# lucas-t-t/FACT-CLIP

Measured on AMD Instinct MI355X. Metric: frames/sec FACT_CLIP fwd+bwd, T=4096 D=2048 Nact=32, at 1/2/4/8 GPUs, higher is better.
Workload: dtype fp32; 1 GPU; FACT_CLIP HAViD-holdout dims, seg10 synthetic, T=4096; model=FACT_CLIP, T=4096, D=2048, Nact=32, C=75, videos_per_rank=2, global_batch=2, seq_len=4096, parallelism=dp1, weights=fixed (no optimizer update in the timed steps)

## Files before the change

### fact-clip_amd/csrc/decoder.cpp

```cpp
#include <algorithm>
#include <cmath>
#include <vector>

#include "fx_common.h"
#include "ops.h"
#include "tokdec.h"

namespace fx {
namespace {

constexpr int MAXL = 16;
constexpr int kSmallTok = 64;

struct PackKV {
  const float* src[2 * MAXL];
  const float* bsrc[2 * MAXL];
  float* dst;
  float* bdst;
  int A, Hm, L;
};

__global__ void pack_kv_kernel(PackKV p) {
  const int blk = blockIdx.y;
  const long long n = (long long)p.A * p.Hm;
// ... 6 lines not shown
}

struct UnpackKV {
  float* dst[2 * MAXL];
  float* bdst[2 * MAXL];
  const float* src;
  const float* bsrc;
  int A, Hm, L;
};

__global__ void unpack_kv_acc_kernel(UnpackKV p) {
  const int blk = blockIdx.y;
  const long long n = (long long)p.A * p.Hm;
  const float* src = p.src + (long long)blk * n;
  float* dst = p.dst[blk];
  for (long long i = (long long)blockIdx.x * blockDim.x + threadIdx.x; i < n; i += (long long)gridDim.x * blockDim.x)
    dst[i] += src[i];
  if (blockIdx.x == 0 && p.bdst[blk])
    for (int i = threadIdx.x; i < p.A; i += blockDim.x) p.bdst[blk][i] += p.bsrc[blk * p.A + i];
}

int linear_fwd_res(const float* x, long long ldx, int M, int K, const float* w, long long ldw, const float* b,
                   const float* resid, long long ldr, float* y, long long ldy, int N, hipStream_t s) {
  fx_gemm_desc d = gemm_desc(M, N, K, op_rows(x, ldx), op_rows(w, ldw), y, ldy);
  d.bias = b;
  d.resid = resid;
  d.ld_resid = ldr;
  return launch_gemm(d, s);
}

fx_gemm_desc dx_res_desc(const float* dy, long long lddy, const float* w, long long ldw, int M, int K, int N,
                         const float* resid, long long ldr, float* dx, long long lddx, float* ws) {
  fx_gemm_desc d = gemm_desc(M, K, N, op_rows(dy, lddy), op_cols(w, ldw), dx, lddx);
  d.resid = resid;
  d.ld_resid = ldr;
  d.split_k = pick_split(M, K, N);
  d.workspace = ws;
  return d;
}

int linear_dx_res(const float* dy, long long lddy, const float* w, long long ldw, int M, int K, int N,
                  const float* resid, long long ldr, float* dx, long long lddx, float* ws, hipStream_t s) {
  fx_gemm_desc d = gemm_desc(M, K, N, op_rows(dy, lddy), op_cols(w, ldw), dx, lddx);
  d.resid = resid;
  d.ld_resid = ldr;
  d.split_k = pick_split(M, K, N);
  d.workspace = ws;
  return launch_gemm(d, s);
}

struct DecLayout {
  long long xq, qkv, psa, osa, xh1, rs1, t1, t1q, qc, pca, oca, xh2, rs2, t2, f1, xh3, rs3, t3, per_layer;
  long long layers, fxh, frs, fo, kv, mpos, total_saved;
  long long wkv, bkv, wsp, total_ws_fwd;
  long long dkv, dwkv, dbkv, dT, dS, dU, dF, dQKV, dO, dq, lnws, core, dmask, split, gdu, gdf, gdq, gdqkv,
      gdy, total_ws_bwd;
};

long long dec_split_ws(const fx_decoder_params* p, int R, int T) {
  const int A = p->A, FF = p->FF;
  long long sp = 0;
  sp = std::max(sp, dwdb_ws(R, A, 3 * A));
  sp = std::max(sp, dwdb_ws(R, A, 2 * A));
  sp = std::max(sp, dwdb_ws(R, A, A));
  sp = std::max(sp, dwdb_ws(R, A, FF));
  sp = std::max(sp, dwdb_ws(R, FF, A));
  sp = std::max(sp, split_ws(R, A, 3 * A));
  sp = std::max(sp, split_ws(R, A, FF));
  sp = std::max(sp, split_ws(R, FF, A));
  sp = std::max(sp, dwdb_ws(R, A, p->out_dim));
  sp = std::max(sp, split_ws(R, A, p->out_dim));
  if (p->cross) {
    const long long AL2 = 2LL * A * p->num_layers;
    sp = std::max(sp, split_ws(T, (int)AL2, p->Hm));
    sp = std::max(sp, dwdb_ws(T, p->Hm, (int)AL2));
    sp = std::max(sp, split_ws(T, p->Hm, (int)AL2));
    sp = std::max(sp, dwdb_ws(T, p->Hm, (int)(AL2 / 2)));
    sp = std::max(sp, (long long)defer_split(T) * AL2 * (p->Hm + 1));
    sp = std::max(sp, split_ws(T, p->Hm, (int)(AL2 / 2)));
  }
  return sp;
}

int dec_tmax(const fx_decoder_params* p, int T, int nvid) {
  if (!p->cross) return 0;
  if (!p->mem_off) return T / nvid;
  int m = 0;
  for (int v = 0; v < nvid; ++v) m = std::max(m, p->mem_off[v + 1] - p->mem_off[v]);
  return m;
}

int dec_qmax(const fx_decoder_params* p, int R, int nvid) {
  if (!p->tok_off) return R / nvid;
  int m = 0;
  for (int v = 0; v < nvid; ++v) m = std::max(m, p->tok_off[v + 1] - p->tok_off[v]);
  return m;
}

long long dec_attn_ws(const fx_decoder_params* p, int nvid, int Qv, int Tv) {
  const int hd = p->A / p->nhead;
  long long w = p->cross ? tattn_ws_floats(nvid, Qv, Tv, hd, p->nhead) : 0;
  if (Qv > kSmallTok) w = std::max(w, tattn_ws_floats(nvid, Qv, Qv, hd, p->nhead));
  return w;
}

DecLayout dec_layout(const fx_decoder_params* p, int R, int T, int has_qpos, int has_mpos, int nvid) {
  DecLayout L{};
  const long long A = p->A, FF = p->FF, h = p->nhead, RA = (long long)R * A;
  const long long Qv = dec_qmax(p, R, nvid), Tv = dec_tmax(p, T, nvid);
  long long o = 0;
  L.xq = o; o += al64(has_qpos ? RA : 0);
  L.qkv = o; o += al64(3 * RA);
  L.psa = o; o += al64(nvid * h * Qv * Qv);
  L.osa = o; o += al64(RA);
  L.xh1 = o; o += al64(RA);
  L.rs1 = o; o += al64(R);
  L.t1 = o; o += al64(RA);
  if (p->cross) {
    L.t1q = o; o += al64(has_qpos ? RA : 0);
    L.qc = o; o += al64(RA);
    L.pca = o; o += al64(nvid * h * Qv);
    L.oca = o; o += al64(RA);
    L.xh2 = o; o += al64(RA);
    L.rs2 = o; o += al64(R);
    L.t2 = o; o += al64(RA);
  }
  L.f1 = o; o += al64((long long)R * FF);
  L.xh3 = o; o += al64(RA);
  L.rs3 = o; o += al64(R);
  L.t3 = o; o += al64(RA);
  L.per_layer = o;
  L.layers = 0;
  o = L.layers + L.per_layer * p->num_layers;
  L.fxh = o; o += al64(p->final_norm ? RA : 0);
  L.frs = o; o += al64(p->final_norm ? R : 0);
  L.fo = o; o += al64(p->final_norm ? RA : 0);
  const long long AL2 = 2 * A * p->num_layers;
  L.kv = o; o += al64(p->cross ? (long long)T * AL2 : 0);
  L.mpos = o; o += al64((p->cross && has_mpos) ? (long long)T * p->Hm : 0);
  L.total_saved = o;
  const long long sp = dec_split_ws(p, R, T);
  o = 0;
  L.wkv = o; o += al64(p->cross ? AL2 * p->Hm : 0);
  L.bkv = o; o += al64(p->cross ? AL2 : 0);
  const long long att = dec_attn_ws(p, nvid, (int)Qv, (int)Tv);
  L.wsp = o; o += al64(std::max(sp, att) + RA);
  L.total_ws_fwd = o;
  o = 0;
  L.dkv = o; o += al64(p->cross ? (long long)T * AL2 : 0);
  L.dwkv = o; o += al64(p->cross ? AL2 * p->Hm : 0);
  L.dbkv = o; o += al64(p->cross ? AL2 : 0);
  L.dT = o; o += al64(RA);
  L.dS = o; o += al64(RA);
  L.dU = o; o += al64(RA);
  L.dF = o; o += al64((long long)R * FF);
  L.dQKV = o; o += al64(3 * RA);
  L.dO = o; o += al64(RA);
  L.dq = o; o += al64(RA);
  L.lnws = o; o += al64(layernorm_bwd_ws_floats(R, (int)A));
  L.core = o; o += al64(att);
  L.dmask = o; o += al64((p->dropout > 0.f) ? RA : 0);
  L.split = o; o += al64(sp);
  L.gdu = o; o += al64(3LL * p->num_layers * RA);
  L.gdf = o; o += al64((long long)p->num_layers * R * FF);
  L.gdq = o; o += al64((long long)p->num_layers * RA);
  L.gdqkv = o; o += al64(3LL * p->num_layers * RA);
  L.gdy = o; o += al64(3LL * p->num_layers * RA);
  L.total_ws_bwd = o;
  (void)FF;
  return L;
}

int dec_check(const fx_decoder_params* p, int R, int T, int nvid) {
  FX_REQUIRE(p && p->num_layers >= 1 && p->num_layers <= MAXL, "decoder: 1..16 layers");
  FX_REQUIRE(nvid >= 1 && nvid <= 32, "decoder: 1..32 videos");
  if (p->tok_off) {
    FX_REQUIRE(p->tok_off[0] == 0 && p->tok_off[nvid] == R, "decoder: token offsets must span [0, R]");
    for (int v = 0; v < nvid; ++v) FX_REQUIRE(p->tok_off[v + 1] > p->tok_off[v], "decoder: >= 1 token per video, offsets increasing");
  } else {
    FX_REQUIRE(R % nvid == 0, "decoder: token rows split evenly (or tok_off)");
  }
  if (p->cross) {
    if (p->mem_off) {
      FX_REQUIRE(p->mem_off[0] == 0 && p->mem_off[nvid] == T, "decoder: memory offsets must span [0, T]");
      for (int v = 0; v < nvid; ++v) FX_REQUIRE(p->mem_off[v + 1] > p->mem_off[v], "decoder: empty video memory");
    } else {
      FX_REQUIRE(T % nvid == 0 && T >= nvid, "decoder: memory rows must split evenly over the videos");
    }
    FX_REQUIRE(p->Hm > 0, "decoder: cross attention needs memory rows");
  }
  R /= nvid;
  FX_REQUIRE(p->nhead > 0 && p->A % p->nhead == 0, "decoder: A must be divisible by nhead");
  FX_REQUIRE(R >= 1, "decoder: >= 1 token per video");
  FX_REQUIRE(p->A / p->nhead <= 64, "decoder: head dim must be <= 64");
  FX_REQUIRE(p->A <= 1024, "decoder: A <= 1024 (LayerNorm row kernel)");
  FX_REQUIRE(p->dropout >= 0.f && p->dropout < 1.f && p->attn_dropout >= 0.f && p->attn_dropout < 1.f,
             "decoder: dropout p in [0, 1)");
// ... 385 lines not shown
  if (amode == TOK_A_LN) {
    P->ln.w = ln_w;
    P->ln.b = ln_b;
    P->ln.eps = 1e-5f;
  }
  return tb.flush();
}

long long fx_decoder_saved_floats(const fx_decoder_params* p, int R, int T, int nvid, int has_qpos, int has_mpos) {
  return dec_layout(p, R, T, has_qpos, has_mpos, std::max(nvid, 1)).total_saved;
}

long long fx_decoder_workspace_floats(const fx_decoder_params* p, int R, int T, int nvid, int has_qpos,
                                      int has_mpos) {
  const DecLayout L = dec_layout(p, R, T, has_qpos, has_mpos, std::max(nvid, 1));
  return std::max(L.total_ws_fwd, L.total_ws_bwd);
}

int fx_decoder_fwd(const fx_decoder_params* p, const float* tgt, long long ldt, int R, const float* qpos,
                   long long ldqp, const float* mem, long long ldm, int T, int nvid, const float* mpos, long long ldmp,
                   float* out, long long ldo, float* saved, float* workspace, void* stream) {
  FX_TRY(dec_check(p, R, T, nvid));
  const int Qv = dec_qmax(p, R, nvid), Tv = dec_tmax(p, T, nvid);
  hipStream_t s = (hipStream_t)stream;
  const int A = p->A, FF = p->FF, h = p->nhead, hd = A / h, NL = p->num_layers;
  const long long RA = (long long)R * A;
  const float eps = p->eps > 0.f ? p->eps : 1e-5f;
  const float pd = p->dropout, pa = p->attn_dropout;
  const float scale = 1.0f / std::sqrt((float)hd);
  const DecLayout L = dec_layout(p, R, T, qpos != nullptr, mpos != nullptr, nvid);
  FX_REQUIRE(!qpos || ldqp == A, "decoder: query_pos must be dense (R, A)");
  float* spl = workspace + L.wsp;
  WsBound wb(spl, L.total_ws_fwd - L.wsp);
  const int AL2 = 2 * A * NL;
  float* kv = saved + L.kv;
  if (p->cross) {
    PackKV pk{};
    for (int l = 0; l < NL; ++l) {
      pk.src[l] = p->ca_k_w[l];
      pk.src[NL + l] = p->ca_v_w[l];
      pk.bsrc[l] = p->ca_in_b[l] + A;
      pk.bsrc[NL + l] = p->ca_in_b[l] + 2 * A;
    }
    pk.dst = workspace + L.wkv;
    pk.bdst = workspace + L.bkv;
    pk.A = A;
    pk.Hm = p->Hm;
    pk.L = NL;
    fx_launch(pack_kv_kernel, dim3(std::min(cdiv((long long)A * p->Hm, 256), 256), 2 * NL), dim3(256), 0, s,
                       pk);
    FX_CHECK_HIP(hipGetLastError());
    prof_begin(9, s);
    if (!mpos) {
      FX_TRY(linear_fwd(mem, ldm, T, p->Hm, workspace + L.wkv, workspace + L.bkv, kv, AL2, AL2, 0, s));
      prof_end(9, s, 2.0 * T * AL2 * p->Hm, 4.0 * ((double)T * p->Hm + (double)AL2 * p->Hm + (double)T * AL2));
    } else {
      const int AL = A * NL;
      FX_TRY(linear_fwd(mem, ldm, T, p->Hm, workspace + L.wkv, workspace + L.bkv, kv, AL2, AL, 0, s, -1, mpos, ldmp,
                        p->Hm));
      FX_TRY(linear_fwd(mem, ldm, T, p->Hm, workspace + L.wkv + (long long)AL * p->Hm, workspace + L.bkv + AL,
                        kv + AL, AL2, AL, 0, s));
      prof_end(9, s, 2.0 * T * AL2 * p->Hm, 4.0 * (2.0 * T * p->Hm + (double)AL2 * p->Hm + (double)T * AL2), 2);
      FX_TRY(add2(mem, ldm, mpos, ldmp, T, p->Hm, saved + L.mpos, p->Hm, 0, s));
    }
  }
  {
    const void* ptrs[3] = {tgt, qpos, out};
    const long long lds_[2] = {ldt, ldo};
    if (dec_tok_ok(p, R, nvid, ptrs, 3, lds_, 2)) {
      float* u = spl + (std::max(L.total_ws_fwd - L.wsp, RA) - RA);
      return dec_fwd_tok(p, tgt, ldt, R, qpos, nvid, Qv, Tv, kv, out, ldo, saved, L, u, spl, s);
    }
  }
  const float* x = tgt;
  long long ldx = ldt;
  for (int l = 0; l < NL; ++l) {
    float* b = saved + L.layers + l * L.per_layer;
    const float* xq = x;
    long long ldxq = ldx;
    if (qpos) {
      if (l == 0) FX_TRY(add2(x, ldx, qpos, A, R, A, b + L.xq, A, 0, s));
      xq = b + L.xq;
      ldxq = A;
    }
    float* qkv = b + L.qkv;
    if (!qpos) {
      FX_TRY(linear_fwd(x, ldx, R, A, p->sa_in_w[l], p->sa_in_b[l], qkv, 3 * A, 3 * A, 0, s));
    } else {
      fx_gemm_desc d2[2];
      d2[0] = gemm_desc(R, 2 * A, A, op_rows(xq, ldxq), op_rows(p->sa_in_w[l], A), qkv, 3 * A);
      d2[0].bias = p->sa_in_b[l];
      d2[1] = gemm_desc(R, A, A, op_rows(x, ldx), op_rows(p->sa_in_w[l] + 2LL * A * A, A), qkv + 2 * A, 3 * A);
      d2[1].bias = p->sa_in_b[l] + 2 * A;
      FX_TRY(launch_gemm_group(d2, 2, s));
    }
    if (Qv <= kSmallTok) {
      FX_TRY(launch_mha_small_fwd(qkv, 3 * A, qkv + A, 3 * A, qkv + 2 * A, 3 * A, Qv, Qv, hd, h, scale, b + L.psa,
                                  b + L.osa, A, s, nvid, pa, dec_seed(p, l, 0), p->tok_off));
    } else {
      TAttnOpts o;
      o.koff = o.qoff = p->tok_off;
      o.drop_p = pa;
      o.drop_seed = dec_seed(p, l, 0);
      FX_TRY(launch_tattn_fwd(qkv, 3 * A, qkv + A, 3 * A, qkv + 2 * A, 3 * A, nvid, Qv, Qv, hd, h, scale, b + L.osa, A,
                              b + L.psa, spl, s, &o));
    }
    float* u = spl + (std::max(L.total_ws_fwd - L.wsp, RA) - RA);
// ... 302 lines not shown
```

### fact-clip_amd/csrc/fx_common.h

```cpp
#pragma once
#include <hip/hip_runtime.h>
#include <hip/hip_ext.h>
#include <cstdint>
#include <cstdio>
#include <string>

#include "../../include/factmx.h"

namespace fx {

void set_error(const std::string& msg);

#define FX_CHECK_HIP(expr)                                                        \
  do {                                                                            \
    hipError_t _e = (expr);                                                       \
    if (_e != hipSuccess) {                                                       \
      ::fx::set_error(std::string("HIP error ") + hipGetErrorString(_e) + " at " + \
                      __FILE__ + ":" + std::to_string(__LINE__));                 \
      return FX_ERR_HIP;                                                          \
    }                                                                             \
  } while (0)

#define FX_REQUIRE(cond, msg)                 \
  do {                                        \
// ... 27 lines not shown
int aux_join_into(hipStream_t s, hipStream_t a);
int defer_split(int rows);
long long gemm_workspace_floats(const fx_gemm_desc& d);

fx_operand op_rows(const float* p, long long ld);
fx_operand op_cols(const float* p, long long ld);
fx_gemm_desc gemm_desc(int M, int N, int K, fx_operand a, fx_operand b, float* c, long long ldc);

int launch_colsum_batched(const float* x, long long ld, long long x_bs, int M, int N, int nb, float* out,
                          long long out_bs, int accumulate, float* ws, hipStream_t s);
int launch_colsum(const float* x, long long ld, int M, int N, float* out, int accumulate,
                  float* ws, hipStream_t s);

constexpr long long kArrivalCounters = 1 << 16;
unsigned* arrival_counters(hipStream_t s);

__host__ __device__ inline unsigned fx_drop_bits(unsigned long long seed, unsigned long long idx) {
  unsigned long long z = seed + (idx + 1ull) * 0x9E3779B97F4A7C15ull;
  z = (z ^ (z >> 30)) * 0xBF58476D1CE4E5B9ull;
  z = (z ^ (z >> 27)) * 0x94D049BB133111EBull;
  z ^= z >> 31;
  return (unsigned)(z >> 32);
}
inline unsigned fx_drop_thresh(float p) {
  const double t = (double)p * 4294967296.0;
  return t >= 4294967295.0 ? 4294967295u : (unsigned)t;
}
inline unsigned long long fx_drop_subseed(unsigned long long seed, int i) {
  return seed + 0xD1B54A32D192ED03ull * (unsigned long long)(i + 1);
}
int launch_dropout(const float* x, long long ldx, int rows, int cols, long long idx_ld, long long idx_col0, float p,
                   unsigned long long seed, float* y, long long ldy, hipStream_t s);

struct Knobs {
  int gemm_path = 0;
  int gemm_wide = -1;
  bool gemm_xcd_planes = true;
  bool gemm_persist = true;
  bool gemm_group_m = true;
  bool gemm_row_perm = true;
  bool frl_pair = true;
  int frl_min_fill = 80;
  int frl2_min_fill = 55;
  bool aux_stream = true;
  bool x2y_a2f_dw = true;
  bool tattn_fold = true;
  bool tattn_rr = true;
  bool gru_poll2 = true;
  int gru_store_wave = 2;
  int frl_xcd = 2;
  bool gemm_group = true;
  bool gemm_ktail = true;
  bool dec_tok = true;
  int tok_spin = 0;
  bool side_stream = true;
  bool mstcn_defer = true;
  bool x2y_fused = true;
  bool x2y_f2a_one = true;
  int x2y_f2a_bwd = 2;
};
const Knobs& knobs();

void prof_begin(int kind, hipStream_t s);
void prof_end(int kind, hipStream_t s, double flops, double bytes, int launches = 1);
extern thread_local int g_prof_open;
bool prof_kernel_events(hipStream_t s, hipEvent_t* e0, hipEvent_t* e1);

template <typename... Args, typename F = void (*)(Args...)>
inline void fx_launch(F kernel, const dim3& grid, const dim3& block, std::uint32_t shm, hipStream_t s, Args... args) {
  hipEvent_t e0, e1;
  if (g_prof_open >= 0 && prof_kernel_events(s, &e0, &e1))
    hipExtLaunchKernelGGL(kernel, grid, block, shm, s, e0, e1, 0u, args...);
  else
    hipLaunchKernelGGL(kernel, grid, block, shm, s, args...);
}

unsigned tok_spin_max();
unsigned x2y_spin_max();
int coresident_blocks(const void* kernel, int threads, size_t lds);

}
```

### fact-clip_amd/csrc/gemm.cpp

```cpp
#include <algorithm>
#include <atomic>
#include <cstdio>
#include <map>
#include <mutex>
#include <utility>
#include <vector>

#include "gemm_plan.h"

namespace fx {

unsigned* arrival_counters(hipStream_t s) {
  static std::mutex mu;
  static std::map<std::pair<int, hipStream_t>, unsigned*> pool;
  int dev = 0;
  if (hipGetDevice(&dev) != hipSuccess) return nullptr;
  std::lock_guard<std::mutex> lk(mu);
  const auto key = std::make_pair(dev, s);
  auto it = pool.find(key);
  if (it != pool.end()) return it->second;
  unsigned* p = nullptr;
  if (hipMalloc(&p, kArrivalCounters * sizeof(unsigned)) != hipSuccess) return nullptr;
  if (hipMemsetAsync(p, 0, kArrivalCounters * sizeof(unsigned), s) != hipSuccess) {
    (void)hipFree(p);
    return nullptr;
  }
  pool[key] = p;
  return p;
}

thread_local const float* t_ws_lo = nullptr;
thread_local const float* t_ws_hi = nullptr;

WsBound::WsBound(const float* base, long long floats) : prev_lo(t_ws_lo), prev_hi(t_ws_hi) {
  t_ws_lo = base;
  t_ws_hi = base ? base + std::max(floats, 0LL) : nullptr;
}
WsBound::~WsBound() {
  t_ws_lo = prev_lo;
  t_ws_hi = prev_hi;
}

fx_operand op_rows(const float* p, long long ld) {
  fx_operand o{};
  o.ptr = p;
  o.ld = ld;
  o.conv_dir = 1;
  return o;
}

fx_operand op_cols(const float* p, long long ld) {
  fx_operand o = op_rows(p, ld);
  o.trans = 1;
  return o;
}

fx_gemm_desc gemm_desc(int M, int N, int K, fx_operand a, fx_operand b, float* c, long long ldc) {
  fx_gemm_desc d{};
  d.M = M;
  d.N = N;
  d.K = K;
  d.batch = 1;
  d.a = a;
  d.b = b;
  d.c = c;
  d.ldc = ldc;
  d.alpha = 1.f;
  d.split_k = 1;
  return d;
}

long long gemm_workspace_floats(const fx_gemm_desc& d) {
  if (d.split_k <= 1) return 0;
  return (long long)d.batch * d.split_k * d.M * d.N;
}

std::mutex g_prec_mu;
std::vector<std::pair<hipStream_t, int>> g_prec;
std::atomic<int> g_prec_any{0};
std::atomic<int> g_prec_default{FX_PREC_F32};

int stream_precision(hipStream_t s) {
  if (!g_prec_any.load(std::memory_order_acquire)) return g_prec_default.load(std::memory_order_relaxed);
  std::lock_guard<std::mutex> lk(g_prec_mu);
  for (const auto& e : g_prec)
    if (e.first == s) return e.second;
  return g_prec_default.load(std::memory_order_relaxed);
}

bool valid_precision(int prec) {
  return prec == FX_PREC_F32 || prec == FX_PREC_BF16 || prec == FX_PREC_F32S || prec == FX_PREC_F32S2;
}

namespace {

int plan_on_stream(const fx_gemm_desc& d, hipStream_t s, long long cnt_base, GemmPlan& P) {
  FX_TRY(plan_gemm(d, stream_precision(s), knobs(), cnt_base, P));
  GemmDev& g = P.g;
  const bool direct = P.family == FAM_DIRECT;
  const int cap = d.split_k > 1 ? d.split_k : 1;
  if (g.split > 1 && t_ws_hi && !(g.ws >= t_ws_lo && g.ws + (long long)g.split * d.M * d.N * d.batch <= t_ws_hi))
    std::fprintf(stderr, "factmx: gemm M %d N %d K %d batch %d split %d (cap %d, %s) needs %lld floats at +%lld of a %lld-float reservation\n",
                 d.M, d.N, d.K, d.batch, g.split, cap, direct ? "direct" : "tiled",
                 (long long)g.split * d.M * d.N * d.batch, (long long)(g.ws - t_ws_lo), (long long)(t_ws_hi - t_ws_lo));
  FX_REQUIRE(g.split <= 1 || !t_ws_hi ||
                 (g.ws >= t_ws_lo && g.ws + (long long)g.split * d.M * d.N * d.batch <= t_ws_hi),
             "gemm: split-K slabs would overrun the entry point's workspace reservation");
  if (P.counters) {
    unsigned* pool = arrival_counters(s);
    g.tile_cnt = pool ? pool + P.cnt_base : nullptr;
  }
  return FX_OK;
}

void census(const fx_gemm_desc& d, const GemmPlan& P, hipStream_t s) {
#ifdef FX_GEMM_CENSUS
  std::fprintf(stderr, "GEMM %p %d %d %d %d %d %d %d %d %d %d %d\n", (void*)s, d.M, d.N, d.K, d.batch, P.ak, P.bk,
               P.g.split, P.family == FAM_DIRECT ? 1 : P.family == FAM_TILED ? 0 : 2, P.g.persist, d.a.conv_taps,
               (int)(P.g.split > 1 && !P.g.tile_cnt));
#endif
}

int launch_family(const GemmPlan& P, hipStream_t s) {
  switch (P.family) {
    case FAM_TILED: return launch_tiled(P, s);
    case FAM_WIDE8: return launch_wide8(P, s);
    case FAM_BF16: return launch_bf16(P, s);
    case FAM_SPLIT: return launch_split(P, s);
    case FAM_DIRECT: return launch_direct(P, s);
    default: break;
  }
  set_error("gemm: unknown kernel family");
  return FX_ERR_UNSUPPORTED;
}

}

int launch_gemm(const fx_gemm_desc& d, hipStream_t s) {
  FX_REQUIRE(d.M >= 0 && d.N >= 0 && d.K >= 0 && d.batch >= 1, "gemm: bad sizes");
  if (d.M == 0 || d.N == 0) return FX_OK;
  GemmPlan P;
  FX_TRY(plan_on_stream(d, s, 0, P));
  census(d, P, s);
  FX_TRY(launch_family(P, s));
  FX_CHECK_HIP(hipGetLastError());
  return launch_reduce(P, s);
}

int launch_gemm_group(const fx_gemm_desc* d, int n, hipStream_t s) {
  const bool on = knobs().gemm_group;
  FX_REQUIRE(n >= 0 && n <= GMAX, "gemm group: 0..4 members");
  int live = 0, nsplit = 0;
  bool all_direct = on;
  GemmPlan P[GMAX];
  long long cnt_base = 0;
  for (int i = 0; i < n && all_direct; ++i) {
    FX_REQUIRE(d[i].M >= 0 && d[i].N >= 0 && d[i].K >= 0 && d[i].batch >= 1, "gemm: bad sizes");
    if (d[i].M == 0 || d[i].N == 0) continue;
    FX_TRY(plan_on_stream(d[i], s, cnt_base, P[i]));
    if (P[i].g.tile_cnt) cnt_base += P[i].counters;
    all_direct = all_direct && P[i].family == FAM_DIRECT;
    nsplit += P[i].g.split > 1 ? 1 : 0;
    ++live;
  }
  bool ws_ok = true;
  if (all_direct && nsplit > 1) {
    const float* base = nullptr;
    long long off = 0;
    for (int i = 0; i < n && ws_ok; ++i) {
      if (d[i].M == 0 || d[i].N == 0 || P[i].g.split <= 1) continue;
      if (!base) base = d[i].workspace;
      ws_ok = d[i].workspace == base && t_ws_hi != nullptr;
      P[i].g.ws = d[i].workspace + off;
      off += (long long)P[i].g.split * d[i].M * d[i].N * d[i].batch;
      ws_ok = ws_ok && P[i].g.ws >= t_ws_lo && P[i].g.ws + (long long)P[i].g.split * d[i].M * d[i].N * d[i].batch <= t_ws_hi;
    }
  }
  if (!all_direct || live < 2 || !ws_ok) {
    for (int i = 0; i < n; ++i) FX_TRY(launch_gemm(d[i], s));
    return FX_OK;
  }
  bool done[GMAX] = {};
  for (int i0 = 0; i0 < n; ++i0) {
    if (done[i0] || d[i0].M == 0 || d[i0].N == 0) continue;
    const unsigned nw = P[i0].block.x;
    GemmGroup G{};
    int m = 0;
    G.start[0] = 0;
    for (int i = i0; i < n; ++i) {
      if (done[i] || d[i].M == 0 || d[i].N == 0 || P[i].block.x != nw) continue;
      done[i] = true;
      G.g[m] = P[i].g;
      G.kinds[m] = gen_kind(P[i].ak) * 8 + P[i].bk;
      G.start[m + 1] = G.start[m] + (int)(P[i].grid.x * P[i].grid.y * P[i].grid.z);
      ++m;
    }
    for (int i = m + 1; i <= GMAX; ++i) G.start[i] = G.start[m];
    G.n = m;
    if (m == 1) {
      census(d[i0], P[i0], s);
      FX_TRY(launch_direct(P[i0], s));
    } else {
      launch_direct_group(G, G.start[m], nw, s);
    }
    FX_CHECK_HIP(hipGetLastError());
  }
  for (int i = 0; i < n; ++i)
    if (d[i].M != 0 && d[i].N != 0) FX_TRY(launch_reduce(P[i], s));
  return FX_OK;
}

}

extern "C" {

int fx_set_stream_precision(void* stream, int prec) {
  FX_REQUIRE(prec == FX_PREC_DEFAULT || fx::valid_precision(prec),
             "gemm precision: FX_PREC_DEFAULT, FX_PREC_F32, FX_PREC_BF16, FX_PREC_F32S or FX_PREC_F32S2");
  std::lock_guard<std::mutex> lk(fx::g_prec_mu);
  const hipStream_t s = (hipStream_t)stream;
  auto& v = fx::g_prec;
  for (auto it = v.begin(); it != v.end(); ++it)
    if (it->first == s) {
      v.erase(it);
      break;
    }
  if (prec != FX_PREC_DEFAULT) v.emplace_back(s, prec);
  fx::g_prec_any.store(v.empty() ? 0 : 1, std::memory_order_release);
  return FX_OK;
}

int fx_get_stream_precision(void* stream) { return fx::stream_precision((hipStream_t)stream); }

int fx_stream_precision_explicit(void* stream) {
  std::lock_guard<std::mutex> lk(fx::g_prec_mu);
  for (const auto& e : fx::g_prec)
    if (e.first == (hipStream_t)stream) return e.second;
  return FX_PREC_DEFAULT;
}

int fx_set_default_precision(int prec) {
  FX_REQUIRE(fx::valid_precision(prec), "default gemm precision: FX_PREC_F32, FX_PREC_BF16, FX_PREC_F32S or FX_PREC_F32S2");
  fx::g_prec_default.store(prec, std::memory_order_relaxed);
  return FX_OK;
}

int fx_get_default_precision(void) { return fx::g_prec_default.load(std::memory_order_relaxed); }

}
```

### fact-clip_amd/csrc/gemm_dev.h

```cpp
#pragma once
#include "fx_common.h"

namespace fx {

constexpr int BM = 64, BN = 64, BK = 64, NTHREADS = 256;
constexpr int RS = 68;
constexpr int CS = 65;
constexpr int IMG = BM * RS;
constexpr int NSLOT = 3;
typedef float f32x16 __attribute__((ext_vector_type(16)));
constexpr int WBM = 128;
constexpr int W8T = 512;
constexpr int DCH = 32, DMAXW = 8;
#define FX_INLINE __attribute__((always_inline))

constexpr int kMaxSeq = 16;

enum Kind { ROWS = 0, ROWS_CONV = 1, ROWS_GEN = 2, COLS = 3, COLS_CONV = 4, ROWS_CAT = 5, COLS_CONVR = 6, COLS_KT = 7 };

struct GemmDev {
  int M, N, K;
  fx_operand a, b;
  float* c;
  long long ldc, c_bs;
  float alpha, beta;
  const float* bias;
  const float* resid;
  long long ld_resid, resid_bs;
  const float* gate;
  long long ld_gate;
  int relu, split, kt_per_split, a_vec, b_vec, c_tap_cin;
  float* ws;
  float* c_last;
  int tiles_x, tiles_y;
  long long* stamps;
  unsigned* tile_cnt;
  unsigned drop_thr;
  float drop_scale;
  unsigned long long drop_seed;
  long long c_last_bs;
  int b_dil_growth;
  int xcd_planes;
  int row_perm;
  int group_m;
  int persist;
  int a_dil_b1;
  long long bias_bs;
  int nsoff;
  int soff[kMaxSeq + 1];
};

namespace {

typedef int SeqOff[kMaxSeq + 1];

__device__ __forceinline__ void seq_pos(int seq_len, const SeqOff& soff, int nsoff, int r, int& pos, int& len) {
  if (nsoff > 0) {
    int start = 0, end = 0x7fffffff;
#pragma unroll
    for (int i = 1; i <= kMaxSeq; ++i) {
      if (i <= nsoff) {
        const int o = soff[i];
        if (o <= r) start = o;
        else end = min(end, o);
      }
    }
    pos = r - start;
    len = end - start;
  } else {
    pos = r % seq_len;
    len = seq_len;
  }
}

#ifdef FX_STAMPS
#define FX_STAMP(g, slot)                                                                          \
  do {                                                                                            \
    if ((g).stamps && threadIdx.x == 0) {                                                         \
      const long long _b = (long long)blockIdx.z * gridDim.x * gridDim.y + blockIdx.y * gridDim.x + \
                           blockIdx.x;                                                            \
      (g).stamps[(_b * 2) * 10 + 2 * (slot)] = __builtin_amdgcn_s_memtime();                       \
      (g).stamps[(_b * 2) * 10 + 2 * (slot) + 1] = __builtin_amdgcn_s_memrealtime();               \
    }                                                                                             \
  } while (0)
#else
#define FX_STAMP(g, slot) \
  do {                    \
  } while (0)
#endif

__device__ __forceinline__ int conv_shift(const fx_operand& o, int tap) {
  return (tap - (o.conv_taps - 1) / 2) * o.conv_dil * o.conv_dir;
}

__device__ __forceinline__ fx_operand batch_op_a(const fx_operand& a, int dil_b1, int bidx) {
  fx_operand o = a;
  if (dil_b1 > 0 && bidx == 1) o.conv_dil = dil_b1;
  return o;
}

__device__ __forceinline__ fx_operand batch_op_b(const fx_operand& b, int growth, int bidx) {
  fx_operand o = b;
// ... 385 lines not shown
```

### fact-clip_amd/csrc/gemm_plan.cpp

```cpp
#include <algorithm>

#include "gemm_plan.h"

namespace fx {
namespace {

bool aligned16(const void* p) { return (reinterpret_cast<uintptr_t>(p) & 15) == 0; }

bool use_direct(const fx_gemm_desc& d, int ak, int bk, const Knobs& kn) {
  const int force = kn.gemm_path;
  auto fits = [&](const fx_operand& o, int kind, int R) {
    const double k = (double)d.K + 2 * DMAXW * DCH + 64, ld = (double)o.ld;
    const double bytes = kind == ROWS ? ((double)R * ld + k) * 4 : kind == COLS ? (k * ld + R) * 4 : 0;
    return bytes < 4294967296.0;
  };
  const bool ok = d.K > 0 && direct_pair(gen_kind(ak), bk) && fits(d.a, ak, d.M) && fits(d.b, bk, d.N);
  if (!ok || force == 1) return false;
  if (force == 2) return true;
  const int lim = (ak == ROWS_GEN || ak == ROWS_CAT) ? 32 : 64;
  if (d.M <= lim || d.N <= lim || d.K <= 64 || (d.K <= 512 && d.K % 64 != 0)) return true;
  const long long t32 = (long long)cdiv(d.M, 32) * cdiv(d.N, 32) * d.batch;
  return (ak == ROWS || ak == COLS) && t32 <= 512 && d.K <= 2048;
}

bool use_wide(const GemmDev& g, int ak, int bk, int batch, const Knobs& kn) {
  const int force = kn.gemm_wide;
  const bool fast = g.a_vec && g.b_vec && ((g.K % BK) == 0 || ak == COLS_KT);
  const bool ok = fast && wide8_pair(ak, bk);
  if (!ok || force == 0) return false;
  if (force == 1) return true;
  return (long long)cdiv(g.M, WBM) * g.tiles_x * batch * g.split >= 192;
}

}

bool operand_vec_ok(const fx_operand& o) {
  if (!aligned16(o.ptr) || (o.ld & 3)) return false;
  if (o.batch_stride & 3) return false;
  if (o.conv_taps && (o.conv_cin & 7)) return false;
  if (!o.trans && o.ptr1 && (!aligned16(o.ptr1) || (o.ld1 & 3) || (o.k_split & 7))) return false;
  return true;
}

int kind_of(const fx_operand& o, bool vec) {
  if (o.trans) return o.conv_taps ? (o.nseq > 0 ? COLS_CONVR : COLS_CONV) : COLS;
  if (o.conv_taps) return (vec && o.conv_cin % BK == 0) ? ROWS_CONV : ROWS_GEN;
  if (o.pos) return ROWS_GEN;
  if (o.ptr1 || o.rows0 || o.rows1) return (vec && (!o.ptr1 || o.k_split % BK == 0)) ? ROWS_CAT : ROWS_GEN;
  return ROWS;
}

int plan_gemm(const fx_gemm_desc& d, int prec, const Knobs& kn, long long tile_cnt_base, GemmPlan& P) {
  FX_REQUIRE(d.M >= 0 && d.N >= 0 && d.K >= 0 && d.batch >= 1, "gemm: bad sizes");
  FX_REQUIRE(d.a.ptr && d.b.ptr && d.c, "gemm: null operand");
  FX_REQUIRE(!(d.a.conv_taps && d.a.seq_len <= 0 && d.a.nseq <= 0) &&
                 !(d.b.conv_taps && d.b.seq_len <= 0 && d.b.nseq <= 0),
             "gemm: conv operand needs seq_len or seq_off");
  FX_REQUIRE(d.a.nseq <= 0 || !d.a.trans, "gemm: ragged conv offsets on a row-major A or a column-major B operand");
  FX_REQUIRE(d.b.nseq <= 0 || (d.b.trans && d.b.conv_taps && d.a.nseq <= 0),
             "gemm: ragged column-major conv B needs a plain A operand");
  FX_REQUIRE(!(d.a.conv_taps && d.K != d.a.conv_taps * d.a.conv_cin), "gemm: conv A needs K == taps*cin");
  FX_REQUIRE(!(d.b.conv_taps && d.b.trans && d.N != d.b.conv_taps * d.b.conv_cin + (d.b.ones_col ? 1 : 0)),
             "gemm: conv B needs N == taps*cin (+1 with a ones column)");
  FX_REQUIRE(!(d.a.ones_col && !d.a.trans) && !(d.b.ones_col && !d.b.trans), "gemm: ones_col needs trans==1");
  FX_REQUIRE(!(d.b.conv_taps && !d.b.trans), "gemm: row-major conv B operand is not supported");
  P = GemmPlan{};
  GemmDev& g = P.g;
  g.M = d.M;
  g.N = d.N;
  g.K = d.K;
  g.a = d.a;
  g.b = d.b;
  {
    const fx_operand& o = d.a;
    if (o.nseq > 0) {
      FX_REQUIRE(o.conv_taps && o.seq_off && o.nseq <= kMaxSeq, "gemm: seq_off needs a conv operand, <= 16 videos");
      const int rows = d.M;
      FX_REQUIRE(o.seq_off[0] == 0 && o.seq_off[o.nseq] == rows, "gemm: seq_off must span the operand's rows");
      for (int v = 0; v <= o.nseq; ++v) {
        FX_REQUIRE(v == 0 || o.seq_off[v] > o.seq_off[v - 1], "gemm: seq_off must increase");
        g.soff[v] = o.seq_off[v];
      }
      g.nsoff = o.nseq;
    }
  }
  {
    const fx_operand& o = d.b;
    if (o.nseq > 0) {
      FX_REQUIRE(o.seq_off && o.nseq <= kMaxSeq && o.seq_off[0] == 0 && o.seq_off[o.nseq] <= d.K,
                 "gemm: ragged B offsets must start at 0 and end within K, <= 16 videos");
      FX_REQUIRE(operand_vec_ok(d.a) && operand_vec_ok(d.b) && d.K % BK == 0,
                 "gemm: ragged B needs 16-B operands and K a multiple of 64 (pad the frames)");
      for (int v = 0; v <= kMaxSeq; ++v) {
        FX_REQUIRE(v == 0 || v > o.nseq || o.seq_off[v] > o.seq_off[v - 1], "gemm: seq_off must increase");
        g.soff[v] = v <= o.nseq ? o.seq_off[v] : 0x7fffffff;
      }
      g.nsoff = o.nseq;
    }
  }
  g.c = d.c;
  g.ldc = d.ldc;
  g.c_bs = d.c_batch_stride;
  g.alpha = d.alpha;
  g.beta = d.beta;
  g.bias = d.bias;
  g.resid = d.resid;
  g.ld_resid = d.ld_resid;
  g.resid_bs = d.resid_batch_stride;
  g.gate = d.gate;
  g.ld_gate = d.ld_gate;
  g.relu = d.relu;
  g.c_tap_cin = d.c_tap_cin;
  g.c_last = d.c_last_col;
  g.c_last_bs = d.c_last_batch_stride ? d.c_last_batch_stride : d.M;
  g.b_dil_growth = d.b_dil_growth;
  g.a_dil_b1 = d.a_dil_b1;
  g.bias_bs = d.bias_batch_stride;
  FX_REQUIRE(d.a_dil_b1 <= 0 || (d.a.conv_taps && !d.a.trans), "gemm: a_dil_b1 needs a row-major conv A");
  FX_REQUIRE(d.b_dil_growth <= 1 || (d.b.conv_taps && d.b.trans), "gemm: b_dil_growth needs a column-major conv B");
  g.stamps = d.dbg_stamps;
  FX_REQUIRE(d.drop_p >= 0.f && d.drop_p < 1.f, "gemm: dropout p must be in [0, 1)");
  FX_REQUIRE(d.drop_p == 0.f || (!d.c_last_col && !d.c_tap_cin && !d.gate && d.beta == 0.f &&
                                 !(d.relu == 1 && d.resid)),
             "gemm: dropout only on plain outputs (before the residual add)");
  g.drop_thr = d.drop_p > 0.f ? std::max(fx_drop_thresh(d.drop_p), 1u) : 0u;
  g.drop_scale = 1.f / (1.f - d.drop_p);
  g.drop_seed = d.drop_seed;
  g.a_vec = operand_vec_ok(d.a);
  g.b_vec = operand_vec_ok(d.b);
  g.ws = d.workspace;
  int ak = kind_of(d.a, g.a_vec), bk = kind_of(d.b, g.b_vec);
  const bool direct = d.b_dil_growth <= 1 && d.a_dil_b1 <= 0 && use_direct(d, ak, bk, kn);
  if (!direct && ak == COLS && bk == COLS && g.a_vec && g.b_vec && d.K % BK != 0 && kn.gemm_ktail) ak = bk = COLS_KT;
  P.ak = ak;
  P.bk = bk;
  P.batch = d.batch;
  bool wide = false;
  const int cap = (d.split_k > 1 && d.workspace) ? d.split_k : 1;
  FX_REQUIRE(!(d.split_k > 1 && !d.workspace), "gemm: split-K needs a workspace");
  if (direct) {
    const int nch = cdiv(d.K, DCH);
    const long long t32 = (long long)cdiv(d.M, 32) * cdiv(d.N, 32) * d.batch;
    const int cpw = 1;
    const int nw = std::min(DMAXW, std::max(1, nch / cpw));
    int split = 1;
    if (cap > 1 && t32 < 64) {
      const long long want = std::min<long long>(nch / (cpw * nw), cdiv(2048, t32 * nw));
      split = (int)std::max<long long>(1, std::min<long long>(cap, want));
    }
    g.kt_per_split = nch > 0 ? cdiv(nch, split) : 0;
    g.split = g.kt_per_split > 0 ? cdiv(nch, g.kt_per_split) : 1;
    g.tiles_x = cdiv(d.N, 32);
    g.tiles_y = cdiv(d.M, 32);
    P.block = dim3(nw * 64);
  } else {
    const int nkt = cdiv(d.K, BK);
    int split = std::min(cap, std::max(nkt, 1));
    g.kt_per_split = nkt > 0 ? cdiv(nkt, split) : 0;
    g.split = g.kt_per_split > 0 ? cdiv(nkt, g.kt_per_split) : 1;
    g.tiles_x = cdiv(d.N, BN);
    wide = use_wide(g, ak, bk, d.batch, kn);
    g.tiles_y = cdiv(d.M, wide ? WBM : BM);
    P.block = dim3(wide ? W8T : NTHREADS);
  }
  P.grid = dim3(g.tiles_x, g.tiles_y, d.batch * g.split);
  const bool lowp = wide && bf16_pair(ak, bk);
  P.np = !lowp ? 0 : prec == FX_PREC_F32S ? 3 : prec == FX_PREC_F32S2 ? 2 : 0;
  P.family = direct ? FAM_DIRECT
           : !wide ? FAM_TILED
           : P.np ? (split_pair(ak, bk) ? FAM_SPLIT : FAM_WIDE8)
           : (lowp && prec == FX_PREC_BF16) ? FAM_BF16
                                            : FAM_WIDE8;
  P.fast = P.family == FAM_TILED && g.a_vec && g.b_vec && ((g.K % BK) == 0 || ak == COLS_KT) && ak != ROWS_GEN &&
           gen_kind(bk) != ROWS_GEN;
  const bool runs = P.family == FAM_DIRECT  ? direct_pair(gen_kind(ak), bk)
                    : P.family == FAM_TILED ? tiled_pair(ak, gen_kind(bk), P.fast)
                    : P.family == FAM_BF16  ? bf16_pair(ak, bk)
                    : P.family == FAM_SPLIT ? split_pair(ak, bk)
                    : P.np                  ? wide8_split_pair(ak, bk)
                                            : wide8_pair(ak, bk);
  if (!runs) {
    set_error("gemm: unsupported operand kinds");
    return FX_ERR_UNSUPPORTED;
  }
// ... 29 lines not shown
```

### fact-clip_amd/csrc/gemm_plan.h

```cpp
#pragma once
#include <type_traits>
#include <utility>

#include "gemm_dev.h"

namespace fx {

enum Family { FAM_TILED = 0, FAM_WIDE8, FAM_BF16, FAM_SPLIT, FAM_DIRECT };

constexpr int gen_kind(int k) { return k == ROWS_CAT ? ROWS_GEN : k; }

constexpr bool rowmajor_a(int ak) { return ak == ROWS || ak == ROWS_CONV || ak == ROWS_CAT; }

constexpr bool tiled_pair(int ak, int bk, bool fast) {
  const bool a = rowmajor_a(ak) || ak == COLS || ak == COLS_KT || (ak == ROWS_GEN && !fast);
  const bool b = bk == ROWS || bk == COLS || bk == COLS_CONV || (bk == ROWS_GEN && !fast) ||
                 (fast && ((bk == COLS_CONVR && ak == COLS) || (bk == COLS_KT && ak == COLS_KT)));
  return a && b;
}
constexpr bool tiled_fast_pair(int ak, int bk) { return tiled_pair(ak, bk, true); }
constexpr bool tiled_generic_pair(int ak, int bk) { return tiled_pair(ak, bk, false); }

constexpr bool wide8_pair(int ak, int bk) { return tiled_pair(ak, bk, true); }

constexpr bool bf16_pair(int ak, int bk) { return rowmajor_a(ak) && (bk == ROWS || bk == COLS); }
constexpr bool wide8_split_pair(int ak, int bk) { return rowmajor_a(ak) && bk == ROWS; }
constexpr bool split_pair(int ak, int bk) { return rowmajor_a(ak) && bk == COLS; }

constexpr bool direct_pair(int ak, int bk) {
  return (ak == ROWS || ak == ROWS_GEN || ak == COLS) && (bk == ROWS || bk == COLS);
}

struct GemmPlan {
  GemmDev g;
  dim3 grid, block;
  int ak, bk;
  int family;
  bool fast;
  int np;
  int batch;
  long long cnt_base, counters;
};

bool operand_vec_ok(const fx_operand& o);
int kind_of(const fx_operand& o, bool vec);

int plan_gemm(const fx_gemm_desc& d, int prec, const Knobs& k, long long tile_cnt_base, GemmPlan& P);

int launch_tiled(const GemmPlan& P, hipStream_t s);
int launch_wide8(const GemmPlan& P, hipStream_t s);
int launch_bf16(const GemmPlan& P, hipStream_t s);
int launch_split(const GemmPlan& P, hipStream_t s);
int launch_direct(const GemmPlan& P, hipStream_t s);
void launch_direct_group(const GemmGroup& G, int blocks, unsigned threads, hipStream_t s);
int launch_reduce(const GemmPlan& P, hipStream_t s);

template <class F, int... Ks>
void with_kind(int k, F&& f, std::integer_sequence<int, Ks...>) {
  ((k == Ks ? f(std::integral_constant<int, Ks>{}) : void()), ...);
}
using AllKinds = std::integer_sequence<int, ROWS, ROWS_CONV, ROWS_GEN, COLS, COLS_CONV, ROWS_CAT, COLS_CONVR, COLS_KT>;

template <bool (*Pair)(int, int), class F>
int dispatch_pair(int ak, int bk, const char* family, F&& launch) {
  bool done = false;
  with_kind(ak, [&](auto A) {
    with_kind(bk, [&](auto B) {
      if constexpr (Pair(decltype(A)::value, decltype(B)::value)) {
        launch(A, B);
        done = true;
      }
    }, AllKinds{});
  }, AllKinds{});
  if (done) return FX_OK;
  set_error(std::string("gemm(") + family + "): unsupported operand kinds");
  return FX_ERR_UNSUPPORTED;
}

}
```

### fact-clip_amd/csrc/linear.cpp

```cpp
#include <algorithm>
#include <vector>

#include "fx_common.h"
#include "ops.h"

namespace fx {
namespace {

__global__ void relu_bwd_kernel(const float* dy, long long lddy, const float* y, long long ldy, int rows, int cols,
                                float* dz, long long lddz) {
  const long long total = (long long)rows * cols;
  for (long long i = (long long)blockIdx.x * blockDim.x + threadIdx.x; i < total; i += (long long)gridDim.x * blockDim.x) {
    const long long r = i / cols, c = i % cols;
    dz[r * lddz + c] = y[r * ldy + c] > 0.f ? dy[r * lddy + c] : 0.f;
  }
}

__global__ void add2_kernel(const float* a, long long lda, const float* b, long long ldb, int rows, int cols,
                            float* o, long long ldo, int accumulate, int bcols) {
  const long long total = (long long)rows * cols;
  for (long long i = (long long)blockIdx.x * blockDim.x + threadIdx.x; i < total; i += (long long)gridDim.x * blockDim.x) {
    const long long r = i / cols, c = i % cols;
    const float v = a[r * lda + c] + (b && c < bcols ? b[r * ldb + c] : 0.f);
    o[r * ldo + c] = accumulate ? o[r * ldo + c] + v : v;
  }
}

}

int ew_grid(long long total) { return (int)std::min<long long>(std::max<long long>(cdiv(total, 256), 1), 4096); }

int relu_bwd(const float* dy, long long lddy, const float* y, long long ldy, int rows, int cols, float* dz,
             long long lddz, hipStream_t s) {
  if ((long long)rows * cols == 0) return FX_OK;
  fx_launch(relu_bwd_kernel, dim3(ew_grid((long long)rows * cols)), dim3(256), 0, s, dy, lddy, y, ldy, rows,
                     cols, dz, lddz);
  FX_CHECK_HIP(hipGetLastError());
  return FX_OK;
}

int add2(const float* a, long long lda, const float* b, long long ldb, int rows, int cols, float* o, long long ldo,
         int accumulate, hipStream_t s, int bcols) {
  if ((long long)rows * cols == 0) return FX_OK;
  fx_launch(add2_kernel, dim3(ew_grid((long long)rows * cols)), dim3(256), 0, s, a, lda, b, ldb, rows, cols,
                     o, ldo, accumulate, bcols < 0 ? cols : bcols);
  FX_CHECK_HIP(hipGetLastError());
  return FX_OK;
}

int pick_split(int M, int N, int K, int batch) {
  const int nkt = cdiv(K, 64);
  if (nkt < 4) return 1;
  const bool wide = M >= 128 && K % 64 == 0;
  const long long tiles = (long long)cdiv(M, wide ? 128 : 64) * cdiv(N, 64) * batch;
  if (tiles >= 160) return 1;
  int sp = (int)std::min<long long>(nkt / 2, 256 / tiles);
  return std::max(sp, 1);
}

long long split_ws(int M, int N, int K, int batch) {
  const int sp = pick_split(M, N, K, batch);
  return sp > 1 ? (long long)sp * M * N * batch : 0;
}

int linear_fwd(const float* x, long long ldx, int M, int K, const float* w, const float* b, float* y, long long ldy,
               int N, int relu, hipStream_t s, long long ldw, const float* pos, long long ldpos, int pos_cols) {
  fx_gemm_desc d = gemm_desc(M, N, K, op_rows(x, ldx), op_rows(w, ldw < 0 ? K : ldw), y, ldy);
  d.a.pos = pos;
  d.a.ld_pos = ldpos;
  d.a.pos_cols = pos ? pos_cols : 0;
  d.bias = b;
  d.relu = relu;
  return launch_gemm(d, s);
}

fx_gemm_desc desc_linear_dx(const float* dy, long long lddy, const float* w, int M, int K, int N, float* dx,
                            long long lddx, int accumulate, const float* gate, long long ld_gate, float* ws,
                            long long ldw) {
  fx_gemm_desc d = gemm_desc(M, K, N, op_rows(dy, lddy), op_cols(w, ldw < 0 ? K : ldw), dx, lddx);
  d.beta = accumulate ? 1.f : 0.f;
  d.gate = gate;
  d.ld_gate = ld_gate;
  d.split_k = pick_split(M, K, N);
  d.workspace = ws;
  return d;
}

int linear_dx(const float* dy, long long lddy, const float* w, int M, int K, int N, float* dx, long long lddx,
              int accumulate, const float* gate, long long ld_gate, float* ws, hipStream_t s, long long ldw) {
  return launch_gemm(desc_linear_dx(dy, lddy, w, M, K, N, dx, lddx, accumulate, gate, ld_gate, ws, ldw), s);
}

fx_gemm_desc desc_linear_dwdb(const float* dy, long long lddy, const float* x, long long ldx, int M, int K, int N,
                              float* dw, float* db, int accumulate, float* ws, long long lddw) {
  if (!dw) {
    fx_gemm_desc e{};
    e.batch = 1;
    e.c_last_col = db;
    return e;
  }
  fx_operand b = op_cols(x, ldx);
  const int Kc = K + (db ? 1 : 0);
  if (db) b.ones_col = K + 1;
  fx_gemm_desc d = gemm_desc(N, Kc, M, op_cols(dy, lddy), b, dw, lddw < 0 ? K : lddw);
  d.c_last_col = db;
  d.beta = accumulate ? 1.f : 0.f;
  d.split_k = pick_split(N, K + 1, M);
  d.workspace = ws;
  return d;
}

int linear_dwdb(const float* dy, long long lddy, const float* x, long long ldx, int M, int K, int N, float* dw,
                float* db, int accumulate, float* ws, hipStream_t s, long long lddw) {
  if (!dw && !db) return FX_OK;
  FX_REQUIRE(dw, "linear_dwdb: bias-only gradient needs dw");
  return launch_gemm(desc_linear_dwdb(dy, lddy, x, ldx, M, K, N, dw, db, accumulate, ws, lddw), s);
}

int linear_bwd_pair(const fx_gemm_desc& dwdb, const fx_gemm_desc& dx, hipStream_t s) {
  FX_REQUIRE(!(dwdb.c_last_col && !dwdb.c), "linear_dwdb: bias-only gradient needs dw");
  const fx_gemm_desc pr[2] = {dwdb, dx};
  return launch_gemm_group(pr, 2, s);
}

int linear_dw(const float* dy, long long lddy, const float* x, long long ldx, int M, int K, int N, float* dw,
              int accumulate, float* ws, hipStream_t s, long long lddw) {
  return linear_dwdb(dy, lddy, x, ldx, M, K, N, dw, nullptr, accumulate, ws, s, lddw);
}

long long dwdb_ws(int M, int K, int N) { return split_ws(N, K + 1, M); }

#ifndef FX_DEFER_SPLIT_BUILD
#define FX_DEFER_SPLIT_BUILD 16
#endif
int defer_split(int rows) { return std::max(1, std::min(FX_DEFER_SPLIT_BUILD, rows / 512)); }

}

using namespace fx;

extern "C" {

int fx_dropout(const float* x, long long ldx, int rows, int cols, long long idx_ld, long long idx_col0, float p,
// ... 258 lines not shown
```

### fact-clip_amd/csrc/mstcn.cpp

```cpp
#include <algorithm>
#include <vector>

#include "fx_common.h"
#include "ops.h"
#include "frames.h"

namespace fx {
namespace {

struct PackArgs {
  const float* w[32];
  float* wf[32];
  float* wb[32];
  const float* wpw[32];
  float* wpt[32];
  int F;
};

__global__ __launch_bounds__(256) void pack_conv_kernel(PackArgs p) {
  const int l = blockIdx.z, F = p.F;
  const int c0 = blockIdx.x * 32, n0 = blockIdx.y * 32;
  const int tx = threadIdx.x & 31, ty = threadIdx.x >> 5;
  __shared__ float t[3][32][33];
  const float* w = p.w[l];
  for (int r = ty; r < 32; r += 8) {
    const int n = n0 + r;
    for (int e = tx; e < 96; e += 32) {
      const int cl = e / 3, j = e - cl * 3;
      t[j][r][cl] = (n < F && c0 + cl < F) ? w[(long long)n * 3 * F + (long long)(c0 + cl) * 3 + j] : 0.f;
    }
  }
  __syncthreads();
  for (int r = ty; r < 32; r += 8) {
    const int n = n0 + r, c = c0 + r;
    if (n < F && c0 + tx < F)
#pragma unroll
      for (int j = 0; j < 3; ++j) p.wf[l][(long long)n * 3 * F + j * F + c0 + tx] = t[j][r][tx];
    if (c < F && n0 + tx < F)
#pragma unroll
      for (int j = 0; j < 3; ++j) p.wb[l][(long long)c * 3 * F + j * F + n0 + tx] = t[j][tx][r];
  }
  if (p.wpt[l]) {
    __syncthreads();
    for (int r = ty; r < 32; r += 8) {
      const int o = n0 + r;
      t[0][r][tx] = (o < F && c0 + tx < F) ? p.wpw[l][(long long)o * F + c0 + tx] : 0.f;
    }
    __syncthreads();
    for (int r = ty; r < 32; r += 8) {
      const int c = c0 + r;
      if (c < F && n0 + tx < F) p.wpt[l][(long long)c * F + n0 + tx] = t[0][tx][r];
    }
  }
}

struct MstcnLayout {
  long long rows_pad;
  long long rowsF;
  long long h, z, xh, rs, wbs, wpts, wk1b, wk2b, total_saved;
  long long wf, wk1, wk2, buf0, buf1, buf2, buf3, buf4, buf5, split, split2, colsum, dzall, dhall, dball, csb, bsl,
      total_ws;
};

MstcnLayout mstcn_layout(const fx_mstcn_params* p, int rows) {
  MstcnLayout L{};
  const long long F = p->F;
  const int NL = p->num_layers;
  L.rows_pad = (long long)cdiv(rows, 64) * 64;
  L.rowsF = L.rows_pad * F;
  L.h = 0;
  L.z = L.h + (NL + 1) * L.rowsF;
  L.xh = L.z + NL * L.rowsF;
  L.rs = L.xh + (p->layernorm ? NL * L.rowsF : 0);
  L.wbs = L.rs + (p->layernorm ? (long long)NL * rows : 0);
  const int ng = mstcn_groups(p->ngroup, p->F);
  const bool fl = p->fused_layers && ng == 1;
  const long long wsz = 3 * F * (F / ng);
  L.wpts = L.wbs + NL * wsz;
  L.wk1b = L.wpts + NL * F * F;
  L.wk2b = L.wk1b + (fl ? NL * wsz : 0);
  L.total_saved = L.wk2b + (fl ? NL * F * F : 0);
  L.wf = 0;
  L.wk1 = L.wf + NL * wsz;
  L.wk2 = L.wk1 + (fl ? NL * wsz : 0);
  L.buf0 = L.wk2 + (fl ? NL * F * F : 0);
  L.buf1 = L.buf0 + L.rowsF;
  L.buf2 = L.buf1 + L.rowsF;
  L.buf3 = L.buf2 + L.rowsF;
  L.buf4 = L.buf3 + L.rowsF;
  L.buf5 = L.buf4 + L.rowsF;
  L.split = L.buf5 + L.rowsF;
  long long sp = 0;
  sp = std::max(sp, split_ws(p->F, 3 * p->F + 1, rows));
  sp = std::max(sp, dwdb_ws(rows, p->F, p->F));
  sp = std::max(sp, split_ws(rows, p->F, p->F));
  sp = std::max(sp, dwdb_ws(rows, p->F, p->cout));
  if (p->in_map) sp = std::max(sp, dwdb_ws(rows, p->cin, p->F));
  sp = std::max(sp, split_ws(rows, p->F, p->cout));
  if (p->in_map) sp = std::max(sp, split_ws(rows, p->cin, p->F));
  sp = std::max(sp, layernorm_bwd_ws_floats(rows, p->F));
  if (ng > 1) sp = std::max(sp, gconv_dw_ws_floats(rows, p->F, ng));
  L.split2 = L.split + sp;
  L.colsum = L.split2 + sp;
  long long cs = colsum_workspace_floats(rows, std::max(std::max(p->F, p->cout), p->cin));
  L.dzall = L.colsum + cs;
  L.dhall = L.dzall + NL * L.rowsF;
  L.dball = L.dhall + NL * L.rowsF;
  L.csb = L.dball + (p->dropout > 0.f ? NL * L.rowsF : 0);
  L.bsl = L.csb + (long long)NL * colsum_workspace_floats(rows, p->F);
  const int dsp = defer_split(rows);
  L.total_ws = L.bsl + std::max(split_ws(p->F, p->F + 1, rows, std::max(NL, 1)),
                                dsp > 1 ? (long long)dsp * std::max(NL, 1) * p->F * (3LL * p->F) : 0LL);
  return L;
}

void frag_layer_jobs(std::vector<FragJob>& J, int NL, int F, const float* w1, long long w1_stride,
                     const float* const* w2list, const float* w2, long long w2_stride, float* dst1, float* dst2) {
  for (int l = 0; l < NL; ++l) {
    J.push_back({w1 + (long long)l * w1_stride, dst1 + (long long)l * frl_packed_floats(3 * F), 3 * F, 3 * F});
    J.push_back({w2list ? w2list[l] : w2 + (long long)l * w2_stride, dst2 + (long long)l * frl_packed_floats(F), F, F});
  }
}

int launch_frag_jobs(const std::vector<FragJob>& J, hipStream_t s) {
  for (size_t i = 0; i < J.size(); i += FRAG_JOBS)
    FX_TRY(launch_pack_frag(J.data() + i, (int)std::min<size_t>(FRAG_JOBS, J.size() - i), s));
  return FX_OK;
}

int layer_dilation(const fx_mstcn_params* p, int i) {
  long long d = p->dil0 > 0 ? p->dil0 : 1;
  const int f = p->dil_factor > 0 ? p->dil_factor : 2;
  for (int k = 0; k < i; ++k) d *= f;
  return (int)d;
}

bool mstcn_fused_ok(const fx_mstcn_params* p, const Seqs& q, const float* buf) {
  return p->fused_layers && p->ngroup <= 1 && !p->layernorm && frl_supported(p->F, buf, p->F, p->F) &&
         (!q.off || q.nvid <= 16) && (p->fused_layers == 2 || frl_fills_device(q.rows()));
}

bool mstcn_defer_ok(const fx_mstcn_params* p, const fx_mstcn_grads* g) {
  const int NL = p->num_layers;
  return knobs().mstcn_defer && uniform_stride(g->w_dil, NL) && uniform_stride(g->b_dil, NL) &&
         uniform_stride(g->w_pw, NL) && uniform_stride(g->b_pw, NL);
}

enum class BwdSchedule {
  FusedDeferred,
  GemmDeferred,
  FusedPerLayer,
  PerLayer,
};

struct MstcnBwd {
  const fx_mstcn_params* p;
  const fx_mstcn_grads* g;
  Seqs q;
  MstcnLayout L;
  const float* saved;
  float* ws;
  float* dx;
  long long lddx;
  hipStream_t s;
  SideLane lane;
  float *spl, *spm;
  const float *wk1, *wk2;
  int rows, F, NL, ng;
  bool drop;
  float *Hb[3], *Zb[3];
  const float* h(int i) const { return saved + L.h + i * L.rowsF; }
  const float* z(int i) const { return saved + L.z + i * L.rowsF; }
  float* dZall(int i) const { return ws + L.dzall + i * L.rowsF; }
  float* dHall(int i) const { return ws + L.dhall + i * L.rowsF; }
  float* dBall(int i) const { return drop ? ws + L.dball + i * L.rowsF : dHall(i); }
  int dil(int i) const { return layer_dilation(p, i); }
  int wait_side(int i) const { return i < NL ? lane.wait(i) : FX_OK; }
  int mask_dB(int i) const {
    if (!drop) return FX_OK;
    return launch_dropout(dHall(i), F, rows, F, F, 0, p->dropout, fx_drop_subseed(p->seed, i), dBall(i), F, s);
  }
  int pw_dx(const float* gB, int i, float* dZ) const {
    fx_gemm_desc d = gemm_desc(rows, F, F, op_rows(gB, F), op_rows(saved + L.wpts + (long long)i * F * F, F), dZ, F);
    d.gate = z(i);
    d.ld_gate = F;
    d.split_k = pick_split(rows, F, F);
    d.workspace = spm;
    return launch_gemm(d, s);
  }
  int pw_dw(const float* gB, int i) const {
    return linear_dwdb(gB, F, z(i), F, rows, F, F, g->w_pw[i], g->b_pw[i], 1, spl, lane.side);
  }
  int conv_dw(int i, const float* dZi) const {
    if (ng > 1)
      return launch_gconv_dw(dZi, F, h(i), F, rows, q.T, q.nvid, q.off, F, ng, dil(i), g->w_dil[i], g->b_dil[i], spl,
                             lane.side);
    return per_video(q, [&](int r0, int nr, const Seqs& qv) -> int {
      fx_operand b = conv_operand(h(i) + (long long)r0 * F, F, F, dil(i), 1, qv, true);
      b.ones_col = 3 * F + 1;
      fx_gemm_desc d = gemm_desc(F, 3 * F + 1, nr, op_cols(dZi + (long long)r0 * F, F), b, g->w_dil[i], 3 * F);
      d.c_tap_cin = F;
      d.c_last_col = g->b_dil[i];
      d.beta = 1.f;
      d.split_k = pick_split(F, 3 * F + 1, nr);
      d.workspace = spl;
      return launch_gemm(d, lane.side);
    });
  }
  int conv_dx(int i, const float* dZ, const float* gU, float* out, long long ldo) const {
    prof_begin(0, s);
    if (ng > 1) {
      FX_TRY(launch_gconv(dZ, F, rows, q.T, q.nvid, q.off, F, ng, dil(i), -1,
                          saved + L.wbs + i * gconv_packed_floats(F, ng), nullptr, 0, gU, F, 0, out, ldo, s));
    } else {
      fx_gemm_desc d = gemm_desc(rows, F, 3 * F, conv_operand(dZ, F, F, dil(i), -1, q, false),
                                 op_rows(saved + L.wbs + (long long)i * 3 * F * F, 3 * F), out, ldo);
      d.resid = gU;
      d.ld_resid = F;
      FX_TRY(launch_gemm(d, s));
    }
    prof_end(0, s, 2.0 * rows * F * 3.0 * (F / ng), 4.0 * (3.0 * rows * F + 3.0 * F * (F / ng)));
    return FX_OK;
  }
  int frl_dx(int i, const float* dZi, const float* gU, float* dHi, float* dZn, float* dBn) const {
    return launch_frl(dZi, F, rows, q.T, dil(i), -1, q.off, q.nvid, wk1 + (long long)i * 3 * F * F, nullptr, 0, gU, F,
                      dHi, F, wk2 + (long long)(i - 1) * F * F, nullptr, nullptr, 0, z(i - 1), F, dZn, F, 0.f, 0, s,
                      dBn ? p->dropout : 0.f, dBn ? fx_drop_subseed(p->seed, i - 1) : 0, dBn, dBn ? F : 0);
  }
  int deferred_conv_dx(int i, const float** dH0) const {
    const bool to_dx = i == 0 && !p->in_map && dx;
    if (i == 0) *dH0 = to_dx ? nullptr : Hb[0];
    return conv_dx(i, dZall(i), dHall(i), i > 0 ? dHall(i - 1) : (to_dx ? dx : Hb[0]), to_dx ? lddx : F);
  }
  int batched_dw() const;
};

int MstcnBwd::batched_dw() const {
  const int Kp = (int)L.rows_pad;
// ... 11 lines not shown
    d.c_last_col = g->b_pw[0];
    d.c_last_batch_stride = NL > 1 ? g->b_pw[1] - g->b_pw[0] : 0;
    d.beta = 1.f;
    d.split_k = std::max(pick_split(F, F + 1, rows, NL), defer_split(rows));
    d.workspace = ws + L.bsl;
    FX_TRY(launch_gemm(d, lane.side));
  }
  {
    fx_operand b = conv_operand(h(0), F, F, dil(0), 1, q, true);
    b.batch_stride = L.rowsF;
    fx_operand a = op_cols(dZall(0), F);
    a.batch_stride = L.rowsF;
    fx_gemm_desc d = gemm_desc(F, 3 * F, Kp, a, b, g->w_dil[0], 3 * F);
    d.batch = NL;
    d.c_batch_stride = NL > 1 ? g->w_dil[1] - g->w_dil[0] : 0;
    d.b_dil_growth = p->dil_factor > 0 ? p->dil_factor : 2;
    d.c_tap_cin = F;
    d.beta = 1.f;
    d.split_k = defer_split(rows);
    d.workspace = ws + L.bsl;
    FX_TRY(launch_gemm(d, lane.side));
  }
  return launch_colsum_batched(dZall(0), F, L.rowsF, rows, F, NL, g->b_dil[0], NL > 1 ? g->b_dil[1] - g->b_dil[0] : 0,
                               1, ws + L.csb, lane.side);
}

int bwd_fused_deferred(const MstcnBwd& c, const float** dH0) {
  const int NL = c.NL, F = c.F, rows = c.rows;
  FX_TRY(c.mask_dB(NL - 1));
  FX_TRY(c.pw_dx(c.dBall(NL - 1), NL - 1, c.dZall(NL - 1)));
  if (NL > 1) prof_begin(7, c.s);
  for (int i = NL - 1; i >= 1; --i)
    FX_TRY(c.frl_dx(i, c.dZall(i), c.dHall(i), c.dHall(i - 1), c.dZall(i - 1), c.drop ? c.dBall(i - 1) : nullptr));
  if (NL > 1)
    prof_end(7, c.s, (NL - 1) * 2.0 * rows * F * 4.0 * F, (NL - 1) * 4.0 * (4.0 * rows * F + 4.0 * F * F), NL - 1);
  FX_TRY(c.deferred_conv_dx(0, dH0));
  return c.batched_dw();
}

int bwd_gemm_deferred(const MstcnBwd& c, const float** dH0) {
  for (int i = c.NL - 1; i >= 0; --i) {
    FX_TRY(c.mask_dB(i));
    FX_TRY(c.pw_dx(c.dBall(i), i, c.dZall(i)));
    FX_TRY(c.deferred_conv_dx(i, dH0));
  }
  return c.batched_dw();
}

int bwd_fused_per_layer(const MstcnBwd& c, const float** dH0) {
  const int NL = c.NL, F = c.F, rows = c.rows;
  const int top = NL - 1;
  FX_TRY(c.lane.fork(1));
  FX_TRY(c.pw_dw(c.Hb[0], top));
  FX_TRY(linear_dx(c.Hb[0], F, c.p->w_pw[top], rows, F, F, c.Zb[0], F, 0, c.z(top), F, c.spm, c.s));
  FX_TRY(c.lane.fork(2));
  FX_TRY(c.conv_dw(top, c.Zb[0]));
  FX_TRY(c.lane.done(top));
  for (int i = NL - 1; i >= 0; --i) {
    const float* gU = c.Hb[(NL - 1 - i) % 3];
    const float* dZi = c.Zb[(NL - 1 - i) % 3];
    float* dHi = c.Hb[(NL - i) % 3];
    FX_TRY(c.wait_side(i + 2));
    if (i == 0) {
      FX_TRY(c.conv_dx(0, dZi, gU, dHi, F));
    } else {
      float* dZn = c.Zb[(NL - i) % 3];
      prof_begin(7, c.s);
      FX_TRY(c.frl_dx(i, dZi, gU, dHi, dZn, nullptr));
      prof_end(7, c.s, 2.0 * rows * F * 4.0 * F, 4.0 * (4.0 * rows * F + 4.0 * F * F));
      FX_TRY(c.lane.fork(1));
      FX_TRY(c.pw_dw(dHi, i - 1));
      FX_TRY(c.conv_dw(i - 1, dZn));
      FX_TRY(c.lane.done(i - 1));
    }
    *dH0 = dHi;
  }
  return FX_OK;
}

int bwd_per_layer(const MstcnBwd& c, const float** dH0) {
  const fx_mstcn_params* p = c.p;
  const int NL = c.NL, F = c.F, rows = c.rows;
  float* dH = c.Hb[0];
  float* dU = c.ws + c.L.buf1;
  for (int i = NL - 1; i >= 0; --i) {
    const int step = NL - 1 - i;
    const float* gU = dH;
    if (p->layernorm) {
      FX_TRY(launch_layernorm_bwd(dH, F, nullptr, 0, c.saved + c.L.xh + i * c.L.rowsF, F, p->ln_w[i],
                                  c.saved + c.L.rs + (long long)i * rows, rows, F, 0, dU, F, c.g->ln_w[i],
                                  c.g->ln_b[i], c.spm, c.s));
      gU = dU;
    }
    const float* gB = gU;
    if (c.drop) {
      float* gm = c.ws + c.L.buf4;
      FX_TRY(launch_dropout(gU, F, rows, F, F, 0, p->dropout, fx_drop_subseed(p->seed, i), gm, F, c.s));
      gB = gm;
    }
    FX_TRY(c.lane.fork(1));
    FX_TRY(c.pw_dw(gB, i));
    float* dZ = c.lane.ss ? c.Zb[step & 1] : c.Zb[0];
    FX_TRY(c.wait_side(i + 2));
    FX_TRY(c.pw_dx(gB, i, dZ));
    FX_TRY(c.lane.fork(2));
    FX_TRY(c.conv_dw(i, dZ));
    FX_TRY(c.lane.done(i));
// ... 8 lines not shown

}

int pack_conv_set(const float* const* w, int NL, int F, int ng, float* wf, float* wb, const float* const* wpw,
                  float* wpt, hipStream_t s) {
  if (ng > 1) {
    const long long gsz = gconv_packed_floats(F, ng);
    std::vector<GPackJob> J;
    for (int l = 0; l < NL; ++l)
      J.push_back({w[l], wf + l * gsz, wb + l * gsz, wpw ? wpw[l] : nullptr, wpt ? wpt + (long long)l * F * F : nullptr});
    return J.empty() ? FX_OK : launch_gconv_pack(J.data(), NL, F, ng, s);
  }
  PackArgs a{};
  a.F = F;
  const long long wsz = 3LL * F * F;
  for (int l = 0; l < NL; ++l) {
    a.w[l] = w[l];
    a.wf[l] = wf + l * wsz;
    a.wb[l] = wb + l * wsz;
    a.wpw[l] = wpw ? wpw[l] : nullptr;
    a.wpt[l] = wpt ? wpt + (long long)l * F * F : nullptr;
  }
  fx_launch(pack_conv_kernel, dim3(cdiv(F, 32), cdiv(F, 32), NL), dim3(256), 0, s, a);
  FX_CHECK_HIP(hipGetLastError());
  return FX_OK;
}

}

using namespace fx;

extern "C" {

long long fx_mstcn_saved_floats(const fx_mstcn_params* p, int rows) { return mstcn_layout(p, rows).total_saved; }
long long fx_mstcn_workspace_floats(const fx_mstcn_params* p, int rows) { return mstcn_layout(p, rows).total_ws; }

int fx_mstcn_fwd(const fx_mstcn_params* p, const float* x, long long ldx, int T, int nvid, float* y, long long ldy,
                 float* saved, float* workspace, void* stream) {
  hipStream_t s = (hipStream_t)stream;
  FX_REQUIRE(p && p->num_layers >= 0 && p->num_layers <= 32, "mstcn: 0..32 layers");
  FX_REQUIRE(p->in_map || p->cin == p->F, "mstcn: in_map=0 needs cin == F");
  FX_TRY(gconv_check(p->F, p->ngroup, "mstcn"));
  const Seqs q{T, nvid, p->seq_off};
  FX_TRY(check_seqs(q));
  const int rows = q.rows();
  const int F = p->F;
  const int ng = mstcn_groups(p->ngroup, F);
  const MstcnLayout L = mstcn_layout(p, rows);
  FX_TRY(pack_conv_set(p->w_dil, p->num_layers, F, ng, workspace + L.wf, saved + L.wbs, p->w_pw, saved + L.wpts, s));
  if (L.rows_pad > rows && p->num_layers > 0)
    FX_CHECK_HIP(hipMemset2DAsync(saved + L.h + (long long)rows * F, L.rowsF * sizeof(float), 0,
                                  (L.rows_pad - rows) * F * sizeof(float), 2 * p->num_layers + 1, s));
  float* h0 = saved + L.h;
  if (p->in_map) {
    FX_TRY(linear_fwd(x, ldx, rows, p->cin, p->w_in, p->b_in, h0, F, F, 0, s));
  } else {
    FX_CHECK_HIP(hipMemcpy2DAsync(h0, F * sizeof(float), x, ldx * sizeof(float), F * sizeof(float), rows,
                                  hipMemcpyDeviceToDevice, s));
  }
  const bool fused = mstcn_fused_ok(p, q, saved);
  if (fused && p->num_layers > 0) {
    std::vector<FragJob> J;
    frag_layer_jobs(J, p->num_layers, F, workspace + L.wf, 3LL * F * F, p->w_pw, nullptr, 0, workspace + L.wk1,
                    workspace + L.wk2);
    frag_layer_jobs(J, p->num_layers, F, saved + L.wbs, 3LL * F * F, nullptr, saved + L.wpts, (long long)F * F,
                    saved + L.wk1b, saved + L.wk2b);
    FX_TRY(launch_frag_jobs(J, s));
  }
  for (int i = 0; i < p->num_layers; ++i) {
    const float* hi = saved + L.h + i * L.rowsF;
    float* hn = saved + L.h + (i + 1) * L.rowsF;
    float* zi = saved + L.z + i * L.rowsF;
    if (fused) {
      if (i == 0) prof_begin(7, s);
      FX_TRY(launch_frl(hi, F, rows, T, layer_dilation(p, i), 1, q.off, q.nvid,
                        workspace + L.wk1 + (long long)i * 3 * F * F, p->b_dil[i], 1, nullptr, 0, zi, F,
                        workspace + L.wk2 + (long long)i * F * F, p->b_pw[i], hi, F, nullptr, 0, hn, F, p->dropout,
                        fx_drop_subseed(p->seed, i), s));
      if (i == p->num_layers - 1)
        prof_end(7, s, p->num_layers * 2.0 * rows * F * 4.0 * F, p->num_layers * 4.0 * (3.0 * rows * F + 4.0 * F * F),
                 p->num_layers);
      continue;
    }
    if (ng > 1) {
      prof_begin(0, s);
      FX_TRY(launch_gconv(hi, F, rows, T, q.nvid, q.off, F, ng, layer_dilation(p, i), 1,
                          workspace + L.wf + i * gconv_packed_floats(F, ng), p->b_dil[i], 1, nullptr, 0, 0, zi, F, s));
      prof_end(0, s, 2.0 * rows * F * 3.0 * (F / ng), 4.0 * (2.0 * rows * F + 3.0 * F * (F / ng)));
    } else {
      fx_gemm_desc d = gemm_desc(rows, F, 3 * F, conv_operand(hi, F, F, layer_dilation(p, i), 1, q, false),
                                 op_rows(workspace + L.wf + (long long)i * 3 * F * F, 3 * F), zi, F);
      d.bias = p->b_dil[i];
      d.relu = 1;
      prof_begin(0, s);
      FX_TRY(launch_gemm(d, s));
      prof_end(0, s, 2.0 * rows * F * 3.0 * F, 4.0 * (2.0 * rows * F + 3.0 * F * F));
    }
    float* u = p->layernorm ? workspace + L.buf0 : hn;
    fx_gemm_desc e = gemm_desc(rows, F, F, op_rows(zi, F), op_rows(p->w_pw[i], F), u, F);
    e.bias = p->b_pw[i];
    e.resid = hi;
    e.ld_resid = F;
    e.drop_p = p->dropout;
    e.drop_seed = fx_drop_subseed(p->seed, i);
    FX_TRY(launch_gemm(e, s));
    if (p->layernorm)
      FX_TRY(launch_layernorm_fwd(u, F, nullptr, 0, p->ln_w[i], p->ln_b[i], 1e-5f, rows, F, 0, hn, F, nullptr,
                                  saved + L.rs + (long long)i * rows, saved + L.xh + i * L.rowsF, F, s));
  }
  const float* hL = saved + L.h + p->num_layers * L.rowsF;
  return linear_fwd(hL, F, rows, F, p->w_out, p->b_out, y, ldy, p->cout, 0, s);
}

int fx_mstcn_bwd(const fx_mstcn_params* p, const fx_mstcn_grads* g, const float* x, long long ldx, int T, int nvid,
                 const float* dy, long long lddy, float* dx, long long lddx, const float* saved, float* ws,
                 void* stream) {
  hipStream_t s = (hipStream_t)stream;
  const Seqs q{T, nvid, p->seq_off};
  FX_TRY(check_seqs(q));
  const int rows = q.rows(), F = p->F, NL = p->num_layers;
  const MstcnLayout L = mstcn_layout(p, rows);
  FX_REQUIRE(p->dropout >= 0.f && p->dropout < 1.f, "mstcn: dropout must be in [0, 1)");
  FX_TRY(gconv_check(F, p->ngroup, "mstcn"));
  const int ng = mstcn_groups(p->ngroup, F);
  const bool drop = p->dropout > 0.f;
  const bool defer = !p->layernorm && NL > 0 && ng == 1 && mstcn_defer_ok(p, g);
  const bool drop_chain_ok = !drop || defer;
  const bool fchain = NL > 0 && drop_chain_ok && mstcn_fused_ok(p, q, ws + L.buf0);
  const BwdSchedule sched = fchain ? (defer ? BwdSchedule::FusedDeferred : BwdSchedule::FusedPerLayer)
                                   : (defer ? BwdSchedule::GemmDeferred : BwdSchedule::PerLayer);
  MstcnBwd c{p, g, q, L, saved, ws, dx, lddx, s, side_lane(s, !p->layernorm && drop_chain_ok), ws + L.split,
             ws + L.split2, saved + L.wk1b, saved + L.wk2b, rows, F, NL, ng, drop,
             {ws + L.buf0, ws + L.buf1, ws + L.buf3}, {ws + L.buf2, ws + L.buf4, ws + L.buf5}};
  if (fchain && !mstcn_fused_ok(p, q, saved)) {
    std::vector<FragJob> J;
    frag_layer_jobs(J, NL, F, saved + L.wbs, 3LL * F * F, nullptr, saved + L.wpts, (long long)F * F, ws + L.wk1,
                    ws + L.wk2);
    FX_TRY(launch_frag_jobs(J, s));
    c.wk1 = ws + L.wk1;
    c.wk2 = ws + L.wk2;
  }
  WsBound wb(c.spl, L.colsum - L.split);
  if (defer && L.rows_pad > rows)
    FX_CHECK_HIP(hipMemset2DAsync(ws + L.dzall + (long long)rows * F, L.rowsF * sizeof(float), 0,
                                  (L.rows_pad - rows) * F * sizeof(float), (drop ? 3 : 2) * NL, s));
  FX_TRY(c.lane.fork(0));
  FX_TRY(linear_dwdb(dy, lddy, c.h(NL), F, rows, F, p->cout, g->w_out, g->b_out, 1, c.spl, c.lane.side));
  float* dHtop = defer ? c.dHall(NL - 1) : c.Hb[0];
  FX_TRY(linear_dx(dy, lddy, p->w_out, rows, F, p->cout, dHtop, F, 0, nullptr, 0, c.spm, s));
  const float* dH = c.Hb[0];
  switch (sched) {
    case BwdSchedule::FusedDeferred: FX_TRY(bwd_fused_deferred(c, &dH)); break;
    case BwdSchedule::GemmDeferred: FX_TRY(bwd_gemm_deferred(c, &dH)); break;
    case BwdSchedule::FusedPerLayer: FX_TRY(bwd_fused_per_layer(c, &dH)); break;
    case BwdSchedule::PerLayer: FX_TRY(bwd_per_layer(c, &dH)); break;
  }
  if (p->in_map) {
    if (g->w_in) {
      FX_TRY(c.lane.fork(0));
      FX_TRY(linear_dwdb(dH, F, x, ldx, rows, p->cin, F, g->w_in, g->b_in, 1, c.spl, c.lane.side));
    }
    if (dx) FX_TRY(linear_dx(dH, F, p->w_in, rows, p->cin, F, dx, lddx, 0, nullptr, 0, c.spm, s));
  } else if (dx && dH) {
    FX_CHECK_HIP(hipMemcpy2DAsync(dx, lddx * sizeof(float), dH, F * sizeof(float), F * sizeof(float), rows,
                                  hipMemcpyDeviceToDevice, s));
  }
  return c.lane.join(p->side_defer);
}

}
```

### fact-clip_amd/csrc/mstcn_fused.hip

```cpp
#include <cstdlib>
#include <map>
#include <mutex>

#include "frl_dev.h"
#include "fx_common.h"
#include "ops.h"

namespace fx {
namespace {

using namespace frl_dev;

constexpr int VS = FN + 4;
constexpr int LDS_FLOATS = NSL * A_IMG + FR * VS;
constexpr int LDS_FLOATS_PAIR = 2 * NSL * A_IMG + FR * VS;

struct FrlArgs {
  const float* x;
  long long ldx;
  int dil, dir, T, M;
  int xcd_runs;
  int row_perm;
  int nsoff;
  int soff[kMaxSeqF + 1];
// ... 184 lines not shown
      }
      V[row * VS + col] = v;
      acc[q] = 0.f;
    }
  }
  auto load_res = [&]() {
#pragma unroll
    for (int q = 0; q < 16; ++q) {
      res[q] = g.resid2 ? g.resid2[(long long)erow(q) * g.ldr2 + ecol] : 0.f;
      gat[q] = g.gate2 ? g.gate2[(long long)erow(q) * g.ldg2 + ecol] : 1.f;
    }
  };
  load_res();
  FRL_ST(4);
  __syncthreads();
  FRL_ST(5);
  if constexpr (PAIR) {
    float4 fv[2][4];
    lds_frag(V, VS, li, lh, fv[0]);
#pragma unroll
    for (int j = 0; j < n2; ++j) {
      if (j + 1 < n2) lds_frag(V + (j + 1) * FBK, VS, li, lh, fv[(j + 1) & 1]);
      __builtin_amdgcn_sched_barrier(0);
      mma_frag(fv[j & 1], pb[(n1 + j) % NB], acc);
      __builtin_amdgcn_sched_barrier(0);
      load_w(n1 + j + PD);
      __builtin_amdgcn_sched_barrier(0);
    }
  } else {
#pragma unroll
    for (int j = 0; j < n2; ++j) step(n1 + j, V + j * FBK, VS);
  }
  FRL_ST(6);
  const int col = ecol;
  const float bv = g.bias2 ? g.bias2[col] : 0.f;
#pragma unroll
  for (int q = 0; q < 16; ++q) {
    const int gr = m0 + (q & 3) + 8 * (q >> 2) + 4 * lh;
    float v = acc[q] + bv;
    if (g.drop_thr)
      v = fx_drop_bits(g.drop_seed, (unsigned long long)gr * FN + col) >= g.drop_thr ? v * g.drop_scale : 0.f;
    v += res[q];
    if (!(gat[q] > 0.f)) v = 0.f;
    if (gr < g.M) g.out2[(long long)gr * g.ldo2 + col] = v;
  }
  FRL_ST(7);
}

struct PackFragArgs {
  const float* src[FRAG_JOBS];
  float* dst[FRAG_JOBS];
  int ld[FRAG_JOBS];
  int K[FRAG_JOBS];
  unsigned long long trans;
};

__global__ __launch_bounds__(256) void pack_frag_kernel(PackFragArgs a) {
  const int st = blockIdx.x, w = blockIdx.y, m = blockIdx.z;
  if (st * FBK >= a.K[m]) return;
  const int q = threadIdx.x >> 6, lane = threadIdx.x & 63;
  const int n = w * 32 + (lane & 31), k = st * FBK + 16 * (lane >> 5) + 4 * q;
  float4 v;
  if ((a.trans >> m) & 1ull) {
    const float* c = a.src[m] + (long long)k * a.ld[m] + n;
    v = make_float4(c[0], c[a.ld[m]], c[2ll * a.ld[m]], c[3ll * a.ld[m]]);
  } else {
    v = ld4(a.src[m] + (long long)n * a.ld[m] + k);
  }
  st4(a.dst[m] + ((long long)((st * 8 + w) * 4 + q) * 64 + lane) * 4, v);
}

}

#ifdef FRL_STAMPS
extern "C" int fx_debug_frl_stamps(unsigned long long* out) {
  return hipMemcpyFromSymbol(out, HIP_SYMBOL(g_frl_st), sizeof(g_frl_st)) == hipSuccess ? 0 : -1;
}
#endif

bool frl_fills_device(long long rows, int min_fill_pct) {
  static std::mutex mu;
  static std::map<int, int> cus;
  int dev = 0;
  if (hipGetDevice(&dev) != hipSuccess) return false;
  int n = 0;
  {
    std::lock_guard<std::mutex> lk(mu);
    auto it = cus.find(dev);
    if (it == cus.end()) {
      if (hipDeviceGetAttribute(&n, hipDeviceAttributeMultiprocessorCount, dev) != hipSuccess) n = 256;
      cus[dev] = n;
    } else {
      n = it->second;
    }
  }
  return (rows + FR - 1) / FR >= (long long)n * (min_fill_pct >= 0 ? min_fill_pct : knobs().frl_min_fill) / 100;
}

bool frl_supported(int F, const void* x, long long ldx, long long ld_other) {
  return F == FN && ldx % 4 == 0 && ((uintptr_t)x & 15) == 0 && ld_other % 4 == 0;
}

long long frl_packed_floats(int K) { return (long long)FN * K; }

int launch_pack_frag(const FragJob* jobs, int n, hipStream_t s) {
  FX_REQUIRE(n >= 1 && n <= FRAG_JOBS, "pack_frag: 1..48 matrices per launch");
  PackFragArgs a{};
  int kmax = 0;
  for (int i = 0; i < n; ++i) {
    FX_REQUIRE(jobs[i].K % FBK == 0 && jobs[i].ld % 4 == 0 && jobs[i].ld >= (jobs[i].trans ? FN : jobs[i].K),
               "pack_frag: K % 32 == 0");
    a.src[i] = jobs[i].src;
    a.dst[i] = jobs[i].dst;
    a.ld[i] = jobs[i].ld;
    a.K[i] = jobs[i].K;
    if (jobs[i].trans) a.trans |= 1ull << i;
    kmax = std::max(kmax, jobs[i].K);
  }
  fx_launch(pack_frag_kernel, dim3(kmax / FBK, FN / 32, n), dim3(256), 0, s, a);
  FX_CHECK_HIP(hipGetLastError());
  return FX_OK;
}

int launch_frl(const float* x, long long ldx, int M, int T, int dil, int dir, const int* seq_off, int nseq,
               const float* w1p, const float* bias1, int relu1, const float* resid1, long long ldr1, float* out1,
               long long ldo1, const float* w2p, const float* bias2, const float* resid2, long long ldr2,
               const float* gate2, long long ldg2, float* out2, long long ldo2, float drop_p,
               unsigned long long drop_seed, hipStream_t s, float vdrop_p, unsigned long long vdrop_seed, float* out3,
               long long ldo3) {
  FX_REQUIRE(M > 0 && dil > 0 && (dir == 1 || dir == -1), "frl: bad shape");
  FX_REQUIRE(seq_off ? (nseq >= 1 && nseq <= kMaxSeqF && seq_off[0] == 0 && seq_off[nseq] == M) : T > 0,
             "frl: uniform videos of T rows, or ragged offsets spanning [0, M) (<= 16 videos)");
  FX_REQUIRE(frl_supported(FN, x, ldx, ldo1) && ((uintptr_t)w1p & 15) == 0 && ((uintptr_t)w2p & 15) == 0,
             "frl: needs F = 256 and 16-byte aligned rows");
  FX_REQUIRE(drop_p >= 0.f && drop_p < 1.f && vdrop_p >= 0.f && vdrop_p < 1.f, "frl: dropout must be in [0, 1)");
  FX_REQUIRE(!out3 || (vdrop_p > 0.f && ldo3 % 4 == 0), "frl: out3 holds the masked tile of a dropout layer");
  static const bool attr = [] {
    return hipFuncSetAttribute((const void*)frl_kernel<false, 3>, hipFuncAttributeMaxDynamicSharedMemorySize,
                               LDS_FLOATS * (int)sizeof(float)) == hipSuccess &&
           hipFuncSetAttribute((const void*)frl_kernel<true, 3>, hipFuncAttributeMaxDynamicSharedMemorySize,
                               LDS_FLOATS_PAIR * (int)sizeof(float)) == hipSuccess;
  }();
  FX_REQUIRE(attr, "frl: cannot raise the LDS limit");
  FrlArgs a{};
  a.x = x;
  a.ldx = ldx;
  a.dil = dil;
  a.dir = dir;
  a.T = T > 0 ? T : 1;
  a.M = M;
  const int nt = cdiv(M, FR), sh = dil / FR;
  a.xcd_runs = knobs().frl_xcd >= 1 && nt >= 16;
  a.row_perm = (knobs().frl_xcd >= 2 && dil % FR == 0 && sh > 1 && nt % sh == 0) ? sh : 1;
  a.nsoff = seq_off ? nseq : 0;
  if (seq_off)
    for (int v = 0; v <= nseq; ++v) a.soff[v] = seq_off[v];
  a.w1p = w1p;
  a.bias1 = bias1;
  a.relu1 = relu1;
  a.resid1 = resid1;
  a.ldr1 = ldr1;
  a.out1 = out1;
  a.ldo1 = ldo1;
  a.w2p = w2p;
  a.bias2 = bias2;
  a.resid2 = resid2;
  a.ldr2 = ldr2;
  a.gate2 = gate2;
  a.ldg2 = ldg2;
  a.out2 = out2;
  a.ldo2 = ldo2;
  a.drop_thr = drop_p > 0.f ? std::max(fx_drop_thresh(drop_p), 1u) : 0u;
// ... 17 lines not shown
```

### fact-clip_amd/csrc/ops.h

```cpp
#pragma once
#include "fx_common.h"

namespace fx {

long long colsum_workspace_floats(int M, int N);
int launch_layernorm_fwd(const float* x, long long ldx, const float* r, long long ldr, const float* w,
                         const float* b, float eps, int rows, int cols, int relu, float* y, long long ldy,
                         float* mean, float* rstd, float* xhat, long long ldxh, hipStream_t s);
int launch_layernorm_fwd_pos(const float* x, long long ldx, const float* r, long long ldr, const float* w,
                             const float* b, float eps, int rows, int cols, int relu, float* y, long long ldy,
                             float* mean, float* rstd, float* xhat, long long ldxh, const float* pos, long long ldp,
                             float* y2, long long ldy2, hipStream_t s);
long long layernorm_bwd_ws_floats(int rows, int cols);
struct LnGradJob {
  const float* dy;
  const float* xhat;
  float* dw;
  float* db;
};
int launch_ln_param_grads(const LnGradJob* jobs, int n, int rows, int cols, long long lddy, long long ldxh,
                          hipStream_t s);
int launch_layernorm_bwd(const float* dy, long long lddy, const float* y, long long ldy, const float* xhat,
                         long long ldxh, const float* w, const float* rstd, int rows, int cols, int relu,
                         float* dx, long long lddx, float* dw, float* db, float* ws, hipStream_t s);
int launch_softmax_rows(const float* x, long long ldx, int rows, int cols, float scale, float* p, long long ldp,
                        hipStream_t s);
int launch_softmax_rows_bwd(const float* p, long long ldp, const float* dp, long long lddp, const float* extra,
                            long long lde, int rows, int cols, float scale, float* dl, long long ldd,
                            hipStream_t s);
int launch_pf_fwd(const float* x, long long ldx, int rows, int cols, int n, float* out, long long ldo, float* clogit,
                  long long ldc,
                  hipStream_t s);
int launch_pf_bwd(const float* out, long long ldo, const float* dout, long long lddo, const float* dcl,
                  long long lddc, int rows, int cols, int n, float* dx, long long lddx, hipStream_t s);
int launch_l2n_fwd(const float* x, long long ldx, int rows, int cols, float* y, long long ldy, float* nrm,
                   hipStream_t s);
int launch_l2n_bwd(const float* y, long long ldy, const float* nrm, const float* dy, long long lddy, int rows,
                   int cols, float* dx, long long lddx, hipStream_t s);
int launch_segments(const float* x, long long ldx, int col0, int ncls, int T, int nvid, const int* row_off,
                    int32_t* pred, int32_t* seg_id, int32_t* seg_start, int32_t* seg_end, int32_t* num_seg,
                    hipStream_t s);
int segments_check_rows(int T, int nvid, const int* row_off, int* rows);
int launch_boundary_scan(const int32_t* pred, int T, int nvid, const int* row_off, int32_t* seg_id,
                         int32_t* seg_start, int32_t* seg_end, int32_t* num_seg, hipStream_t s);
int launch_pf2_fwd(const float* x, long long ldx, int rows, int cols, int n1, int n2, float* out, long long ldo,
                   float* clogit, long long ldc, hipStream_t s);
int launch_pf2_bwd(const float* out, long long ldo, const float* dout, long long lddo, const float* dcl,
                   long long lddc, int rows, int cols, int n1, int n2, float* dx, long long lddx, hipStream_t s);
int launch_vn_logp_fwd(const float* clogit, long long ldc, int rows, int n1, int n2, const int32_t* vids,
                       const int32_t* nids, int A, int null, float* logp, long long ldl, float* lse, hipStream_t s);
int launch_vn_logp_bwd(const float* clogit, long long ldc, const float* lse, const float* dlogp, long long ldg,
                       int rows, int n1, int n2, int A, int null, const int32_t* voff, const int32_t* vlist,
                       const int32_t* noff, const int32_t* nlist, float* dclogit, long long lddc, hipStream_t s);
// ... 15 lines not shown
                   const float* const bhh[2], float* out, long long ldo, int relu_out, float* saved, float* ws,
                   unsigned* status, int spin_max, hipStream_t s);
long long gru_sync_floats(int Hh, int nseq);
int launch_gru_bwd(const float* dout, long long lddo, const float* relu_y, long long ldy, int nseq, const int* seq_off,
                   int Hh, const float* const whh[2], const float* saved, float* dgi, long long lddgi, float* dgh,
                   float* sync_ws, unsigned* status, int spin_max, hipStream_t s);

constexpr int FX_X2Y_MAXTOK = 320;
enum { FX_X2Y_CORE_NONE = 0, FX_X2Y_CORE_A2F = 1, FX_X2Y_CORE_F2A = 2, FX_X2Y_CORE_A2F_WIDE = 3, FX_X2Y_CORE_F2A_WIDE = 4 };
int x2y_core_pick(int nvid, const int* xoff, const int* yoff, int Hd);
bool x2y_a2f_fusable(int nvid, const int* xoff, int Hd);
int launch_x2y_a2f_fwd(const float* yq, const float* xk, const float* xv, int Hd, float scale, int nvid,
                       const int* yoff, const int* xoff, const long long* aoff, float* logit, float* attn,
                       float* feat, hipStream_t s);
bool x2y_f2a_fusable(int nvid, const int* xoff, const int* yoff, int Hd);
long long x2y_f2a_chunks(int nvid, const int* xoff);
long long x2y_f2a_ws_floats(int nvid, const int* xoff, const int* yoff, int Hd);
int launch_x2y_f2a_fwd(const float* yq, const float* xk, const float* xv, int Hd, float scale, int nvid,
                       const int* yoff, const int* xoff, const long long* aoff, float* logit, float* attn,
                       float* feat, float* ws, hipStream_t s);
int launch_x2y_f2a_bwd(const float* dfeat, long long ldf, const float* xv, const float* xk, const float* yq,
                       const float* attn, const float* dattn, const float* dlogit_in, int Hd, float scale, int nvid,
                       const int* yoff, const int* xoff, const long long* aoff, float* dlogit, float* dxv, float* dxk,
                       float* dyq, float* ws, unsigned* status, hipStream_t s);
long long x2y_a2f_dw_ws_floats(int nvid, int Hd, const int* xoff);
bool x2y_a2f_dw_ok(int nvid, const int* yoff);
int launch_x2y_a2f_dw(const float* attn, const float* dl, const float* dfeat, long long ldf, const float* yq, int Hd,
                      float scale, int nvid, const int* yoff, const int* xoff, const long long* aoff, float* dxv,
                      float* dxk, float* ws, hipStream_t s);
int launch_x2y_a2f_bwd(const float* dfeat, long long ldf, const float* xv, const float* xk, const float* attn,
                       const float* dattn, const float* dlogit_in, int Hd, float scale, int nvid, const int* yoff,
                       const int* xoff, const long long* aoff, float* dlogit, float* dyq, hipStream_t s);

struct SideStream;
struct SideLane {
  hipStream_t main, side;
  SideStream* ss;
  int fork(int e) const;
  int done(int i) const;
  int wait(int i) const;
  int join(bool deferred) const;
};
SideLane side_lane(hipStream_t main, bool on = true);

int ew_grid(long long total);
int relu_bwd(const float* dy, long long lddy, const float* y, long long ldy, int rows, int cols, float* dz,
             long long lddz, hipStream_t s);
int add2(const float* a, long long lda, const float* b, long long ldb, int rows, int cols, float* o, long long ldo,
         int accumulate, hipStream_t s, int bcols = -1);
int pick_split(int M, int N, int K, int batch = 1);
long long split_ws(int M, int N, int K, int batch = 1);
int linear_fwd(const float* x, long long ldx, int M, int K, const float* w, const float* b, float* y, long long ldy,
               int N, int relu, hipStream_t s, long long ldw = -1, const float* pos = nullptr, long long ldpos = 0,
               int pos_cols = 0);
int linear_dx(const float* dy, long long lddy, const float* w, int M, int K, int N, float* dx, long long lddx,
              int accumulate, const float* gate, long long ld_gate, float* ws, hipStream_t s, long long ldw = -1);
int linear_dwdb(const float* dy, long long lddy, const float* x, long long ldx, int M, int K, int N, float* dw,
                float* db, int accumulate, float* ws, hipStream_t s, long long lddw = -1);
int linear_dw(const float* dy, long long lddy, const float* x, long long ldx, int M, int K, int N, float* dw,
              int accumulate, float* ws, hipStream_t s, long long lddw = -1);
long long dwdb_ws(int M, int K, int N);
fx_gemm_desc desc_linear_dx(const float* dy, long long lddy, const float* w, int M, int K, int N, float* dx,
                            long long lddx, int accumulate, const float* gate, long long ld_gate, float* ws,
                            long long ldw = -1);
fx_gemm_desc desc_linear_dwdb(const float* dy, long long lddy, const float* x, long long ldx, int M, int K, int N,
                              float* dw, float* db, int accumulate, float* ws, long long lddw = -1);
int linear_bwd_pair(const fx_gemm_desc& dwdb, const fx_gemm_desc& dx, hipStream_t s);

int launch_mha_small_fwd(const float* q, long long ldq, const float* k, long long ldk, const float* v,
                         long long ldv, int Lq, int Lk, int hd, int nhead, float scale, float* probs, float* o,
                         long long ldo, hipStream_t s, int nvid = 1, float drop_p = 0.f,
                         unsigned long long seed = 0, const int* off = nullptr);
int launch_mha_small_bwd(const float* q, long long ldq, const float* k, long long ldk, const float* v,
                         long long ldv, const float* probs, const float* dout, long long lddo, int Lq, int Lk, int hd,
                         int nhead, float scale, float* dq, long long lddq, float* dk, long long lddk, float* dv,
                         long long lddv, hipStream_t s, int nvid = 1, float drop_p = 0.f, unsigned long long seed = 0,
                         const int* off = nullptr);

struct TAttnOpts {
  const int* koff = nullptr;
  const int* qoff = nullptr;
  float drop_p = 0.f;
  unsigned long long drop_seed = 0;
  int acc_kv = 0;
};
long long tattn_ws_floats(int nvid, int Qv, int Tv, int hd, int nhead);
int launch_tattn_fwd(const float* q, long long ldq, const float* k, long long ldk, const float* v, long long ldv,
                     int nvid, int Qv, int Tv, int hd, int nhead, float scale, float* o, long long ldo, float* lse,
                     float* ws, hipStream_t s, const TAttnOpts* opt = nullptr);
int launch_tattn_bwd(const float* q, long long ldq, const float* k, long long ldk, const float* v, long long ldv,
                     const float* o, long long ldo, const float* dout, long long lddo, const float* lse, int nvid,
                     int Qv, int Tv, int hd, int nhead, float scale, float* dq, long long lddq, float* dk,
                     long long lddk, float* dv, long long lddv, float* ws, hipStream_t s,
                     const TAttnOpts* opt = nullptr);

bool frl_supported(int F, const void* x, long long ldx, long long ld_other);
bool frl_fills_device(long long rows, int min_fill_pct = -1);
long long frl_packed_floats(int K);
struct FragJob {
  const float* src;
  float* dst;
  int ld, K;
  int trans = 0;
};
constexpr int FRAG_JOBS = 48;
int launch_pack_frag(const FragJob* jobs, int n, hipStream_t s);
int launch_frl(const float* x, long long ldx, int M, int T, int dil, int dir, const int* seq_off, int nseq,
               const float* w1p, const float* bias1, int relu1, const float* resid1, long long ldr1, float* out1,
               long long ldo1, const float* w2p, const float* bias2, const float* resid2, long long ldr2,
               const float* gate2, long long ldg2, float* out2, long long ldo2, float drop_p,
               unsigned long long drop_seed, hipStream_t s, float vdrop_p = 0.f, unsigned long long vdrop_seed = 0,
               float* out3 = nullptr, long long ldo3 = 0);

struct Frl2Layer {
  int M, T;
  int dil1, dil2;
  const int* seq_off;
  int nseq;
  float drop_p;
  unsigned long long drop_seed;
};
int launch_frl2_fwd(const Frl2Layer& y, const float* f, const float* w1p, const float* w2p, const float* b1,
                    const float* b2, float* cat, const float* wfup, const float* bfu, float* r, float* fnext,
                    hipStream_t s);
int launch_frl2_bwd(const Frl2Layer& y, const float* dcat, const float* wb1p, const float* wb2p, const float* gnext,
                    float* gout, const float* rprev, float* du, const float* wfutp, float* dcat_prev, hipStream_t s);

int gconv_check(int F, int ngroup, const char* who);
long long gconv_packed_floats(int F, int ngroup);
struct GPackJob {
  const float* w;
  float* wf;
  float* wb;
  const float* wpw;
  float* wpt;
};
int launch_gconv_pack(const GPackJob* jobs, int n, int F, int ngroup, hipStream_t s);
int launch_gconv(const float* x, long long ldx, int rows, int T, int nvid, const int* seq_off, int F, int ngroup,
                 int dil, int dir, const float* wp, const float* bias, int relu, const float* resid, long long ldr,
                 int accumulate, float* y, long long ldy, hipStream_t s);
long long gconv_dw_ws_floats(int rows, int F, int ngroup);
int launch_gconv_dw(const float* dz, long long lddz, const float* x, long long ldx, int rows, int T, int nvid,
                    const int* seq_off, int F, int ngroup, int dil, float* dw, float* db, float* ws, hipStream_t s);

}
```

### fact-clip_amd/csrc/runtime.cpp

```cpp
#include <algorithm>
#include <atomic>
#include <cstdlib>
#include <map>
#include <mutex>
#include <tuple>
#include <vector>

#include "fx_common.h"
#include "ops.h"

namespace fx {

static thread_local std::string g_last_error;
void set_error(const std::string& msg) { g_last_error = msg; }

namespace {
struct ProfState {
  int max_events = 0;
  std::vector<hipEvent_t> ev;
  std::vector<double> flops, bytes;
  std::vector<int> launches;
  int used = 0;
  std::vector<hipEvent_t> kev;
  int kused = 0;
// ... 43 lines not shown
  if (kind < 0 || kind >= kProfKinds) return false;
  ProfState& p = g_prof[kind];
  if (s != p.open_stream) return false;
  if (2 * (size_t)(p.kused + 1) > p.kev.size()) {
    p.kdropped++;
    return false;
  }
  *e0 = p.kev[2 * p.kused];
  *e1 = p.kev[2 * p.kused + 1];
  p.kused++;
  return true;
}

unsigned tok_spin_max() {
  const int o = g_spin_override[0].load(std::memory_order_relaxed);
  if (o > 0) return (unsigned)o;
  return knobs().tok_spin > 0 ? (unsigned)knobs().tok_spin : (1u << 20);
}

unsigned x2y_spin_max() {
  const int o = g_spin_override[1].load(std::memory_order_relaxed);
  return o > 0 ? (unsigned)o : (1u << 22);
}

int coresident_blocks(const void* kernel, int threads, size_t lds) {
  static std::mutex mu;
  static std::map<std::tuple<int, const void*, int, size_t>, int> cache;
  int dev = 0;
  if (hipGetDevice(&dev) != hipSuccess) return 0;
  std::lock_guard<std::mutex> lk(mu);
  const auto key = std::make_tuple(dev, kernel, threads, lds);
  auto it = cache.find(key);
  if (it != cache.end()) return it->second;
  int per_cu = 0, cus = 0;
  if (hipOccupancyMaxActiveBlocksPerMultiprocessor(&per_cu, kernel, threads, lds) != hipSuccess ||
      hipDeviceGetAttribute(&cus, hipDeviceAttributeMultiprocessorCount, dev) != hipSuccess)
    return 0;
  const int n = std::max(per_cu, 0) * std::max(cus, 0);
  cache[key] = n;
  return n;
}

const Knobs& knobs() {
  static Knobs k;
  static std::once_flag once;
  std::call_once(once, [] {
    auto env = [](const char* n) -> const char* { return std::getenv(n); };
    if (const char* p = env("FX_GEMM_PATH")) k.gemm_path = std::string(p) == "tiled" ? 1 : std::string(p) == "direct" ? 2 : 0;
    if (const char* p = env("FX_GEMM_WIDE")) k.gemm_wide = p[0] == '1' ? 1 : 0;
    if (const char* p = env("FX_GEMM_XCDPLANES")) k.gemm_xcd_planes = p[0] != '0';
    if (const char* p = env("FX_GEMM_GROUP")) k.gemm_group = p[0] != '0';
    if (const char* p = env("FX_GEMM_KTAIL")) k.gemm_ktail = p[0] != '0';
    if (const char* p = env("FX_DEC_TOK")) k.dec_tok = p[0] != '0';
    if (const char* p = env("FX_TOK_SPIN")) k.tok_spin = std::max(0, std::atoi(p));
    if (const char* p = env("FX_SIDE_STREAM")) k.side_stream = p[0] != '0';
    if (const char* p = env("FX_MSTCN_DEFER")) k.mstcn_defer = p[0] != '0';
    if (const char* p = env("FX_GEMM_ROWPERM")) k.gemm_row_perm = p[0] != '0';
    if (const char* p = env("FX_GEMM_GROUPM")) k.gemm_group_m = p[0] != '0';
    if (const char* p = env("FX_GEMM_PERSIST")) k.gemm_persist = p[0] != '0';
    if (const char* p = env("FX_FRL_XCD")) k.frl_xcd = std::atoi(p);
    if (const char* p = env("FX_FRL_PAIR")) k.frl_pair = p[0] != '0';
    if (const char* p = env("FX_FRL_MIN_FILL")) k.frl_min_fill = std::atoi(p);
    if (const char* p = env("FX_FRL2_MIN_FILL")) k.frl2_min_fill = std::atoi(p);
    if (const char* p = env("FX_AUX_STREAM")) k.aux_stream = p[0] != '0';
    if (const char* p = env("FX_GRU_POLL2")) k.gru_poll2 = p[0] != '0';
    if (const char* p = env("FX_GRU_STORE_WAVE")) k.gru_store_wave = std::max(0, std::min(2, std::atoi(p)));
    if (const char* p = env("FX_TATTN_RR")) k.tattn_rr = p[0] != '0';
    if (const char* p = env("FX_X2Y_A2F_DW")) k.x2y_a2f_dw = p[0] != '0';
    if (const char* p = env("FX_TATTN_FOLD")) k.tattn_fold = p[0] != '0';
    if (const char* p = env("FX_X2Y_FUSED")) k.x2y_fused = p[0] != '0';
    if (const char* p = env("FX_X2Y_F2A_BWD")) k.x2y_f2a_bwd = std::atoi(p);
    if (const char* p = env("FX_X2Y_F2A_ONE")) k.x2y_f2a_one = p[0] != '0';
  });
  return k;
}

struct SideStream {
  hipStream_t s = nullptr;
  hipEvent_t to_side[3] = {};
  hipEvent_t layer_done[4] = {};
  hipEvent_t join = nullptr;
  hipStream_t aux = nullptr;
  hipEvent_t aux_fork = nullptr, aux_done = nullptr;
};

static SideStream* side_stream() {
  if (!knobs().side_stream) return nullptr;
  static std::mutex mu;
  static std::map<int, SideStream*> pool;
  int dev = 0;
  if (hipGetDevice(&dev) != hipSuccess) return nullptr;
  std::lock_guard<std::mutex> lk(mu);
  auto it = pool.find(dev);
  if (it != pool.end()) return it->second;
  SideStream* ss = new SideStream();
#ifndef FX_SIDE_PRIO_BUILD
#define FX_SIDE_PRIO_BUILD 0
#endif
  int prio = 0, least = 0, greatest = 0;
  if (FX_SIDE_PRIO_BUILD != 0 && hipDeviceGetStreamPriorityRange(&least, &greatest) == hipSuccess)
    prio = FX_SIDE_PRIO_BUILD < 0 ? least : greatest;
  bool ok = hipStreamCreateWithPriority(&ss->s, hipStreamNonBlocking, prio) == hipSuccess;
  for (auto& e : ss->to_side) ok = ok && hipEventCreateWithFlags(&e, hipEventDisableTiming) == hipSuccess;
  for (auto& e : ss->layer_done) ok = ok && hipEventCreateWithFlags(&e, hipEventDisableTiming) == hipSuccess;
  ok = ok && hipEventCreateWithFlags(&ss->join, hipEventDisableTiming) == hipSuccess;
  ok = ok && hipStreamCreateWithPriority(&ss->aux, hipStreamNonBlocking, prio) == hipSuccess;
// ... 168 lines not shown
```

### fact-clip_amd/csrc/x2y.cpp

```cpp
#include <algorithm>
#include <cmath>
#include <vector>

#include "fx_common.h"
#include "ops.h"

using namespace fx;

namespace {
constexpr int GMAX_GROUP = 4;
struct X2YLayout {
  long long xin, yin, xk, xv, yq, feat, total;
};
X2YLayout x2y_layout(int Nx, int xdim, int Ny, int ydim, int Hd) {
  X2YLayout L{};
  L.xin = 0;
  L.yin = L.xin + al64((long long)Nx * xdim);
  L.xk = L.yin + al64((long long)Ny * ydim);
  L.xv = L.xk + al64((long long)Nx * Hd);
  L.yq = L.xv + al64((long long)Nx * Hd);
  L.feat = L.yq + al64((long long)Ny * Hd);
  L.total = L.feat + al64((long long)Ny * Hd);
  return L;
}
struct VidRows {
  int n;
  std::vector<int> x, y;
  std::vector<long long> a;
};
VidRows vid_rows(int Nx, int Ny, int nvid, const int* x_off, const int* y_off) {
  VidRows v;
  v.n = std::max(nvid, 1);
  if (v.n == 1 || !x_off || !y_off) {
    v.n = 1;
    v.x = {0, Nx};
    v.y = {0, Ny};
  } else {
    v.x.assign(x_off, x_off + v.n + 1);
    v.y.assign(y_off, y_off + v.n + 1);
  }
  v.a.assign(v.n + 1, 0);
  for (int i = 0; i < v.n; ++i)
    v.a[i + 1] = v.a[i] + (long long)(v.y[i + 1] - v.y[i]) * (v.x[i + 1] - v.x[i]);
  return v;
}
long long x2y_split_ws1(int Nx, int xdim, int Ny, int ydim, int Hd, int outdim) {
  long long sp = 0;
  sp = std::max(sp, split_ws(Ny, Nx, Hd));
  sp = std::max(sp, split_ws(Ny, Hd, Nx));
  sp = std::max(sp, split_ws(Nx, Hd, Ny));
  sp = std::max(sp, split_ws(Ny, ydim + Hd, outdim));
  sp = std::max(sp, dwdb_ws(Ny, ydim, outdim));
  sp = std::max(sp, dwdb_ws(Ny, Hd, outdim));
  sp = std::max(sp, dwdb_ws(Nx, xdim, Hd));
  sp = std::max(sp, dwdb_ws(Ny, ydim, Hd));
  sp = std::max(sp, split_ws(Nx, xdim, Hd));
  sp = std::max(sp, split_ws(Ny, ydim, Hd));
  return sp;
}
long long x2y_split_ws(const VidRows& v, int xdim, int ydim, int Hd, int outdim) {
  long long sp = x2y_split_ws1(v.x[v.n], xdim, v.y[v.n], ydim, Hd, outdim);
  if (Hd % 32 == 0) sp = std::max(sp, x2y_a2f_dw_ws_floats(v.n, Hd, v.x.data()));
  for (int i = 0; i < v.n; ++i)
    sp = std::max(sp, x2y_split_ws1(v.x[i + 1] - v.x[i], xdim, v.y[i + 1] - v.y[i], ydim, Hd, outdim));
  return sp;
}
long long x2y_side_ws(int Nx, int xdim, int Ny, int ydim, int Hd, int outdim) {
  auto one = [](int rows, int M, int N) {
    const int sp = std::max(pick_split(M, N, rows), defer_split(rows));
    return sp > 1 ? (long long)sp * M * N : 0LL;
  };
  long long w = std::max(one(Ny, outdim, ydim + Hd + 1), one(Nx, Hd, xdim + 1));
  w = std::max(w, std::max(one(Ny, outdim, ydim + 1), one(Ny, outdim, Hd + 1)));
  return std::max(w, one(Ny, Hd, ydim + 1));
}
// ... 31 lines not shown
  return x2y_ws_layout(Nx, xdim, Ny, ydim, Hd, outdim, vid_rows(Nx, Ny, nvid, x_off, y_off)).total;
}

int fx_x2y_core(int Hd, int nvid, const int* x_off, const int* y_off, int Nx, int Ny) {
  if (Hd <= 0 || Nx < 0 || Ny < 0) return 0;
  const VidRows v = vid_rows(Nx, Ny, nvid, x_off, y_off);
  switch (x2y_core_pick(v.n, v.x.data(), v.y.data(), Hd)) {
    case FX_X2Y_CORE_A2F:
    case FX_X2Y_CORE_A2F_WIDE: return 1;
    case FX_X2Y_CORE_F2A:
    case FX_X2Y_CORE_F2A_WIDE: return 2;
    default: return 0;
  }
}

static int x2y_drop_cat(const float* Y, long long ldy, const float* feat, int Ny, int ydim, int Hd, float p,
                        unsigned long long seed, float* catd, hipStream_t s) {
  const int cw = ydim + Hd;
  FX_TRY(launch_dropout(Y, ldy, Ny, ydim, cw, 0, p, seed, catd, cw, s));
  return launch_dropout(feat, Hd, Ny, Hd, cw, ydim, p, seed, catd + ydim, cw, s);
}

int fx_x2y_fwd(const float* X, long long ldx, int Nx, int xdim, const float* Xpos, long long ldxp, int xpos_cols,
               const float* Y, long long ldy, int Ny, int ydim, const float* Ypos, long long ldyp, int ypos_cols,
               const float* wk, const float* bk, const float* wv, const float* bv, const float* wq, const float* bq,
               const float* wy, const float* by, int Hd, int outdim, int nvid, const int* x_off, const int* y_off,
               float drop_p, unsigned long long seed, float* out, long long ldo, float* logit, float* attn,
               float* saved, float* workspace, void* stream) {
  hipStream_t s = (hipStream_t)stream;
  const VidRows V = vid_rows(Nx, Ny, nvid, x_off, y_off);
  FX_REQUIRE(drop_p >= 0.f && drop_p < 1.f, "x2y: dropout must be in [0, 1)");
  FX_REQUIRE(V.x[V.n] == Nx && V.y[V.n] == Ny, "x2y: offsets must end at Nx / Ny");
  const X2YLayout L = x2y_layout(Nx, xdim, Ny, ydim, Hd);
  const X2YWs W = x2y_ws_layout(Nx, xdim, Ny, ydim, Hd, outdim, V);
  WsBound wb(workspace, W.split_floats);
  float* xk = saved + L.xk;
  float* xv = saved + L.xv;
  float* yq = saved + L.yq;
  float* feat = saved + L.feat;
  const float* xin = X;
  long long ldxin = ldx;
  if (Xpos) {
    FX_TRY(add2(X, ldx, Xpos, ldxp, Nx, xdim, saved + L.xin, xdim, 0, s, xpos_cols));
    xin = saved + L.xin;
    ldxin = xdim;
  }
  const float* yin = Y;
  long long ldyin = ldy;
  if (Ypos) {
    FX_TRY(add2(Y, ldy, Ypos, ldyp, Ny, ydim, saved + L.yin, ydim, 0, s, ypos_cols));
    yin = saved + L.yin;
    ldyin = ydim;
  }
  prof_begin(10, s);
  FX_TRY(linear_fwd(xin, ldxin, Nx, xdim, wk, bk, xk, Hd, Hd, 0, s));
  FX_TRY(linear_fwd(X, ldx, Nx, xdim, wv, bv, xv, Hd, Hd, 0, s));
  FX_TRY(linear_fwd(yin, ldyin, Ny, ydim, wq, bq, yq, Hd, Hd, 0, s));
  prof_end(10, s, 2.0 * Hd * (2.0 * Nx * xdim + (double)Ny * ydim),
           4.0 * (2.0 * Nx * xdim + (double)Ny * ydim + Hd * (2.0 * xdim + ydim) + Hd * (2.0 * Nx + Ny)), 3);
  const float scale = 1.0f / std::sqrt((float)Hd);
  const bool al16 =
      ((reinterpret_cast<uintptr_t>(yq) | reinterpret_cast<uintptr_t>(xk) | reinterpret_cast<uintptr_t>(xv)) & 15) == 0;
  const double na = (double)V.a[V.n];
  const double core_bytes = 4.0 * ((double)Ny * Hd + 2.0 * Nx * Hd + 2.0 * na + (double)Ny * Hd);
  const int kseg = std::max(Nx, Ny) >= 1024 ? 0 : 8;
  const int core = knobs().x2y_fused && al16 ? x2y_core_pick(V.n, V.x.data(), V.y.data(), Hd) : FX_X2Y_CORE_NONE;
  if (core == FX_X2Y_CORE_A2F || core == FX_X2Y_CORE_A2F_WIDE) {
    prof_begin(3 + kseg, s);
    FX_TRY(launch_x2y_a2f_fwd(yq, xk, xv, Hd, scale, V.n, V.y.data(), V.x.data(), V.a.data(), logit, attn, feat, s));
    prof_end(3 + kseg, s, 4.0 * na * Hd, core_bytes);
  } else if (core == FX_X2Y_CORE_F2A || core == FX_X2Y_CORE_F2A_WIDE) {
    prof_begin(5 + kseg, s);
    FX_TRY(launch_x2y_f2a_fwd(yq, xk, xv, Hd, scale, V.n, V.y.data(), V.x.data(), V.a.data(), logit, attn, feat,
                              workspace + W.f2a, s));
    prof_end(5 + kseg, s, 4.0 * na * Hd, core_bytes);
  } else
  for (int v0 = 0; v0 < V.n; v0 += 2) {
    fx_gemm_desc g1[2], g2[2];
    int n1 = 0, n2 = 0;
    for (int v = v0; v < std::min(V.n, v0 + 2); ++v) {
      const int nx = V.x[v + 1] - V.x[v], ny = V.y[v + 1] - V.y[v];
      if (nx == 0 || ny == 0) continue;
      fx_gemm_desc d = gemm_desc(ny, nx, Hd, op_rows(yq + (long long)V.y[v] * Hd, Hd),
                                 op_rows(xk + (long long)V.x[v] * Hd, Hd), logit + V.a[v], nx);
      d.alpha = scale;
      d.split_k = pick_split(ny, nx, Hd);
      d.workspace = workspace;
      g1[n1++] = d;
      d = gemm_desc(ny, Hd, nx, op_rows(attn + V.a[v], nx), op_cols(xv + (long long)V.x[v] * Hd, Hd),
                    feat + (long long)V.y[v] * Hd, Hd);
      d.split_k = pick_split(ny, Hd, nx);
      d.workspace = workspace;
      g2[n2++] = d;
    }
    FX_TRY(launch_gemm_group(g1, n1, s));
    for (int v = v0; v < std::min(V.n, v0 + 2); ++v) {
      const int nx = V.x[v + 1] - V.x[v], ny = V.y[v + 1] - V.y[v];
      if (nx == 0 || ny == 0) continue;
      FX_TRY(launch_softmax_rows(logit + V.a[v], nx, ny, nx, 1.f, attn + V.a[v], nx, s));
    }
    FX_TRY(launch_gemm_group(g2, n2, s));
  }
  fx_operand a = op_rows(Y, ldy);
  a.ptr1 = feat;
  a.ld1 = Hd;
  a.k_split = ydim;
  if (drop_p > 0.f) {
    float* catd = workspace + W.catd;
    FX_TRY(x2y_drop_cat(Y, ldy, feat, Ny, ydim, Hd, drop_p, seed, catd, s));
    a = op_rows(catd, ydim + Hd);
  }
  fx_gemm_desc d = gemm_desc(Ny, outdim, ydim + Hd, a, op_rows(wy, ydim + Hd), out, ldo);
  d.bias = by;
  return launch_gemm(d, s);
}

int fx_x2y_bwd(const float* X, long long ldx, int Nx, int xdim, int xpos_cols, const float* Y, long long ldy, int Ny,
               int ydim, int ypos_cols, const float* wk, const float* wv, const float* wq, const float* wy, int Hd,
               int outdim, int nvid, const int* x_off, const int* y_off, float drop_p, unsigned long long seed,
               const float* attn, const float* saved,
               const float* dout, long long lddo, const float* dlogit, const float* dattn, float* dX, float* dXpos,
               float* dY, float* dYpos, float* dwk, float* dbk, float* dwv, float* dbv, float* dwq, float* dbq,
               float* dwy, float* dby, int has_xpos, int has_ypos, float* workspace, int side_defer, int32_t* status,
               void* stream) {
  hipStream_t s = (hipStream_t)stream;
  const VidRows V = vid_rows(Nx, Ny, nvid, x_off, y_off);
  FX_REQUIRE(V.x[V.n] == Nx && V.y[V.n] == Ny, "x2y: offsets must end at Nx / Ny");
  const X2YLayout L = x2y_layout(Nx, xdim, Ny, ydim, Hd);
  const float* xk = saved + L.xk;
  const float* xv = saved + L.xv;
  const float* yq = saved + L.yq;
  const float* feat = saved + L.feat;
  const float* xin = has_xpos ? saved + L.xin : X;
  const long long ldxin = has_xpos ? xdim : ldx;
  const float* yin = has_ypos ? saved + L.yin : Y;
  const long long ldyin = has_ypos ? ydim : ldy;
  const int cw = ydim + Hd;
  const X2YWs W = x2y_ws_layout(Nx, xdim, Ny, ydim, Hd, outdim, V);
  float* dcat = workspace + W.dcat;
  float* dL = workspace + W.dL;
  float* dxv = workspace + W.dxv;
  float* dxk = workspace + W.dxk;
  float* dyq = workspace + W.dyq;
  float* dXk = workspace + W.dXk;
  float* dYq = workspace + W.dYq;
  float* spl = workspace + W.split;
  WsBound wb(spl, W.split_floats);
  const float scale = 1.0f / std::sqrt((float)Hd);
  FX_TRY(linear_dx(dout, lddo, wy, Ny, cw, outdim, dcat, cw, 0, nullptr, 0, spl, s));
  const float* catd = nullptr;
  if (drop_p > 0.f) {
    float* cd = workspace + W.catd;
    FX_TRY(x2y_drop_cat(Y, ldy, feat, Ny, ydim, Hd, drop_p, seed, cd, s));
    FX_TRY(launch_dropout(dcat, cw, Ny, cw, cw, 0, drop_p, seed, dcat, cw, s));
    catd = cd;
  }
  const bool al16 = ((reinterpret_cast<uintptr_t>(xk) | reinterpret_cast<uintptr_t>(xv) |
                      reinterpret_cast<uintptr_t>(yq) | reinterpret_cast<uintptr_t>(dcat + ydim)) & 15) == 0;
  const int core = knobs().x2y_fused && (cw & 3) == 0 && al16 ? x2y_core_pick(V.n, V.x.data(), V.y.data(), Hd)
                                                                : FX_X2Y_CORE_NONE;
  const bool fused = core == FX_X2Y_CORE_A2F || core == FX_X2Y_CORE_A2F_WIDE;
  const double na = (double)V.a[V.n];
  const double core_bytes = 4.0 * (2.0 * Ny * Hd + 4.0 * Nx * Hd + 4.0 * na + (double)Ny * Hd);
  const int f2a_mode = knobs().x2y_f2a_bwd;
  const bool f2a_fused = (core == FX_X2Y_CORE_F2A || core == FX_X2Y_CORE_F2A_WIDE) &&
                         (f2a_mode == 1 || (f2a_mode == 2 && core == FX_X2Y_CORE_F2A &&
                                            x2y_f2a_chunks(V.n, V.x.data()) >= 64));
  const int kseg = std::max(Nx, Ny) >= 1024 ? 0 : 8;
  if (fused) prof_begin(4 + kseg, s);
  else if (f2a_fused) prof_begin(6 + kseg, s);
  if (fused) {
    FX_TRY(launch_x2y_a2f_bwd(dcat + ydim, cw, xv, xk, attn, dattn, dlogit, Hd, scale, V.n, V.y.data(), V.x.data(),
                              V.a.data(), dL, dyq, s));
    if (knobs().x2y_a2f_dw && x2y_a2f_dw_ok(V.n, V.y.data())) {
      FX_TRY(launch_x2y_a2f_dw(attn, dL, dcat + ydim, cw, yq, Hd, scale, V.n, V.y.data(), V.x.data(), V.a.data(), dxv,
                               dxk, spl, s));
    } else
    for (int v0 = 0; v0 < V.n; v0 += GMAX_GROUP / 2) {
      fx_gemm_desc g2[GMAX_GROUP];
      int n2 = 0;
      for (int v = v0; v < std::min(V.n, v0 + GMAX_GROUP / 2); ++v) {
        const int nx = V.x[v + 1] - V.x[v], ny = V.y[v + 1] - V.y[v];
        if (nx == 0 || ny == 0) continue;
        const long long xr = (long long)V.x[v] * Hd, yr = (long long)V.y[v] * Hd;
        fx_gemm_desc d = gemm_desc(nx, Hd, ny, op_cols(attn + V.a[v], nx),
                                   op_cols(dcat + (long long)V.y[v] * cw + ydim, cw), dxv + xr, Hd);
        d.split_k = pick_split(nx, Hd, ny);
        d.workspace = spl;
        g2[n2++] = d;
        d = gemm_desc(nx, Hd, ny, op_cols(dL + V.a[v], nx), op_cols(yq + yr, Hd), dxk + xr, Hd);
        d.alpha = scale;
        d.split_k = pick_split(nx, Hd, ny);
        d.workspace = spl;
        g2[n2++] = d;
      }
      FX_TRY(launch_gemm_group(g2, n2, s));
    }
  } else if (f2a_fused) {
    FX_TRY(launch_x2y_f2a_bwd(dcat + ydim, cw, xv, xk, yq, attn, dattn, dlogit, Hd, scale, V.n, V.y.data(), V.x.data(),
                              V.a.data(), dL, dxv, dxk, dyq, workspace + W.f2a, reinterpret_cast<unsigned*>(status), s));
  } else
// ... 13 lines not shown
      d.split_k = pick_split(ny, nx, Hd);
      d.workspace = spl;
      g1[n1++] = d;
      d = gemm_desc(nx, Hd, ny, op_cols(at, nx), op_cols(dfeat, cw), dxv + xr, Hd);
      d.split_k = pick_split(nx, Hd, ny);
      d.workspace = spl;
      g1[n1++] = d;
      d = gemm_desc(ny, Hd, nx, op_rows(dl, nx), op_cols(xk + xr, Hd), dyq + yr, Hd);
      d.alpha = scale;
      d.split_k = pick_split(ny, Hd, nx);
      d.workspace = spl;
      g2[n2++] = d;
      d = gemm_desc(nx, Hd, ny, op_cols(dl, nx), op_cols(yq + yr, Hd), dxk + xr, Hd);
      d.alpha = scale;
      d.split_k = pick_split(nx, Hd, ny);
      d.workspace = spl;
      g2[n2++] = d;
    }
    FX_TRY(launch_gemm_group(g1, n1, s));
    for (int v = v0; v < std::min(V.n, v0 + 2); ++v) {
      const int nx = V.x[v + 1] - V.x[v], ny = V.y[v + 1] - V.y[v];
      if (nx == 0 || ny == 0) continue;
      float* dl = dL + V.a[v];
      FX_TRY(launch_softmax_rows_bwd(attn + V.a[v], nx, dl, nx, dlogit ? dlogit + V.a[v] : nullptr, nx, ny, nx, 1.f,
                                     dl, nx, s));
    }
    FX_TRY(launch_gemm_group(g2, n2, s));
  }
  if (fused) prof_end(4 + kseg, s, 8.0 * na * Hd, core_bytes);
  else if (f2a_fused) prof_end(6 + kseg, s, 8.0 * na * Hd, core_bytes);
  {
    const SideLane lane = side_lane(s);
    FX_TRY(lane.fork(1));
    float* sps = workspace + W.side;
    WsBound wbs(sps, W.side_floats);
    auto dw = [&](const float* dy, long long lddy, const float* x, long long ldx_, int rows, int K, int N, float* w,
                  float* b, long long ldw) -> int {
      fx_gemm_desc d = desc_linear_dwdb(dy, lddy, x, ldx_, rows, K, N, w, b, 1, sps, ldw);
      if (lane.ss) d.split_k = std::max(d.split_k, defer_split(rows));
      return launch_gemm(d, lane.side);
    };
    if (catd) {
      FX_TRY(dw(dout, lddo, catd, cw, Ny, cw, outdim, dwy, dby, cw));
    } else {
      FX_TRY(dw(dout, lddo, Y, ldy, Ny, ydim, outdim, dwy, dby, cw));
      FX_TRY(dw(dout, lddo, feat, Hd, Ny, Hd, outdim, dwy + ydim, nullptr, cw));
    }
    FX_TRY(dw(dxk, Hd, xin, ldxin, Nx, xdim, Hd, dwk, dbk, -1));
    FX_TRY(dw(dxv, Hd, X, ldx, Nx, xdim, Hd, dwv, dbv, -1));
    FX_TRY(dw(dyq, Hd, yin, ldyin, Ny, ydim, Hd, dwq, dbq, -1));
    FX_TRY(lane.join(side_defer));
  }
  if (dX || dXpos) {
    FX_TRY(linear_dx(dxk, Hd, wk, Nx, xdim, Hd, dXk, xdim, 0, nullptr, 0, spl, s));
    if (dXpos) FX_TRY(add2(dXk, xdim, nullptr, 0, Nx, xpos_cols, dXpos, xpos_cols, (has_xpos >> 1) & 1, s));
    if (dX) {
      fx_gemm_desc d = gemm_desc(Nx, xdim, Hd, op_rows(dxv, Hd), op_cols(wv, xdim), dX, xdim);
      d.resid = dXk;
      d.ld_resid = xdim;
      d.split_k = pick_split(Nx, xdim, Hd);
      d.workspace = spl;
      FX_TRY(launch_gemm(d, s));
    }
  }
  if (dY || dYpos) {
    FX_TRY(linear_dx(dyq, Hd, wq, Ny, ydim, Hd, dYq, ydim, 0, nullptr, 0, spl, s));
    if (dYpos) FX_TRY(add2(dYq, ydim, nullptr, 0, Ny, ypos_cols, dYpos, ypos_cols, (has_ypos >> 1) & 1, s));
    if (dY) FX_TRY(add2(dYq, ydim, dcat, cw, Ny, ydim, dY, ydim, 0, s));
  }
  return FX_OK;
}

}
```

### fact-clip_amd/factmx/native.py

```python
import ctypes
import os

import torch

_HERE = os.path.dirname(os.path.abspath(__file__))
LIB_PATH = os.environ.get("FACTMX_LIB", os.path.join(_HERE, "_lib", "libfactmx.so"))
ABI_VERSION = 29

P = ctypes.c_void_p
I = ctypes.c_int
L = ctypes.c_longlong
F = ctypes.c_float
D = ctypes.c_double
U = ctypes.c_ulonglong


class FactmxNativeError(RuntimeError):
    pass


class Operand(ctypes.Structure):
    _fields_ = [("ptr", P), ("ld", L), ("ptr1", P), ("ld1", L), ("k_split", I), ("rows0", P), ("rows1", P),
                ("pos", P), ("ld_pos", L), ("pos_cols", I), ("trans", I), ("conv_taps", I), ("conv_cin", I),
                ("conv_dil", I), ("conv_dir", I), ("seq_len", I), ("batch_stride", L), ("ones_col", I),
                ("seq_off", P), ("nseq", I)]


class GemmDesc(ctypes.Structure):
    _fields_ = [("M", I), ("N", I), ("K", I), ("batch", I), ("a", Operand), ("b", Operand), ("c", P), ("ldc", L),
                ("c_batch_stride", L), ("alpha", F), ("beta", F), ("bias", P), ("resid", P), ("ld_resid", L),
                ("resid_batch_stride", L), ("gate", P), ("ld_gate", L), ("relu", I), ("c_tap_cin", I),
                ("split_k", I), ("workspace", P), ("c_last_col", P), ("dbg_stamps", P), ("drop_p", F),
                ("drop_seed", U), ("c_last_batch_stride", L), ("b_dil_growth", I),
                ("a_dil_b1", I), ("bias_batch_stride", L)]


class MstcnParams(ctypes.Structure):
    _fields_ = [("cin", I), ("F", I), ("cout", I), ("num_layers", I), ("layernorm", I), ("in_map", I),
                ("dil0", I), ("dil_factor", I), ("w_in", P), ("b_in", P), ("w_dil", P), ("b_dil", P), ("w_pw", P), ("b_pw", P),
                ("ln_w", P), ("ln_b", P), ("w_out", P), ("b_out", P), ("dropout", F), ("seed", U),
                ("side_defer", I), ("seq_off", P), ("fused_layers", I), ("ngroup", I)]


class Mstcn2Params(ctypes.Structure):
    _fields_ = [("cin", I), ("F", I), ("cout", I), ("num_layers", I), ("in_map", I), ("dil_factor", I),
                ("w_in", P), ("b_in", P), ("w_d1", P), ("b_d1", P), ("w_d2", P), ("b_d2", P), ("w_fu", P),
                ("b_fu", P), ("w_out", P), ("b_out", P), ("dropout", F), ("seed", U), ("side_defer", I),
                ("seq_off", P), ("ngroup", I), ("fused_layers", I)]


class Mstcn2Grads(ctypes.Structure):
    _fields_ = [("w_in", P), ("b_in", P), ("w_d1", P), ("b_d1", P), ("w_d2", P), ("b_d2", P), ("w_fu", P),
                ("b_fu", P), ("w_out", P), ("b_out", P)]


class MstcnGrads(ctypes.Structure):
    _fields_ = [("w_in", P), ("b_in", P), ("w_dil", P), ("b_dil", P), ("w_pw", P), ("b_pw", P),
                ("ln_w", P), ("ln_b", P), ("w_out", P), ("b_out", P)]


_DEC_PTRS = ["sa_in_w", "sa_in_b", "sa_out_w", "sa_out_b", "ca_q_w", "ca_k_w", "ca_v_w", "ca_in_b", "ca_out_w",
             "ca_out_b", "ff1_w", "ff1_b", "ff2_w", "ff2_b", "ln_sa_w", "ln_sa_b", "ln_ca_w", "ln_ca_b", "ln_ff_w",
             "ln_ff_b"]
DECODER_LAYER_FIELDS = _DEC_PTRS
DECODER_GLOBAL_FIELDS = ["fn_w", "fn_b", "out_w", "out_b"]


class DecoderParams(ctypes.Structure):
    _fields_ = ([("A", I), ("FF", I), ("nhead", I), ("num_layers", I), ("cross", I), ("Hm", I), ("out_dim", I),
                 ("final_norm", I), ("eps", F)] + [(n, P) for n in _DEC_PTRS] + [(n, P) for n in DECODER_GLOBAL_FIELDS]
                + [("side_defer", I), ("dropout", F), ("attn_dropout", F), ("seed", U), ("mem_off", P), ("status", P),
                   ("dqpos_accumulate", I), ("tok_off", P)])


class DecoderGrads(ctypes.Structure):
    _fields_ = [(n, P) for n in _DEC_PTRS] + [(n, P) for n in DECODER_GLOBAL_FIELDS]


STATUS_GRU_TIMEOUT = 1
STATUS_TOK_TIMEOUT = 2
STATUS_X2Y_TIMEOUT = 4
LOSS_MAXK = 512
LOSS_NB = 128
TERM_CLASS, TERM_ATTN, TERM_INFONCE, TERM_VNCLASS = 0, 1, 2, 3
PROF_MSTCN2_FUSED = 15
PREC_DEFAULT, PREC_F32, PREC_BF16, PREC_F32S, PREC_F32S2 = -1, 0, 1, 2, 3


class LossTerm(ctypes.Structure):
    _fields_ = [("kind", I), ("slot", I), ("R", I), ("C", I), ("x", P), ("sr", L), ("sc", L), ("dx", P), ("dsr", L),
                ("dsc", L), ("y", P), ("rs", P), ("re", P), ("gs", P), ("ge", P), ("gl", P), ("G", I), ("axis", I),
                ("K", I), ("D", I), ("w", P), ("c_ce", F), ("c_sm", F), ("inv_temp", F), ("pad0", F), ("lse", P),
                ("lse2", P), ("colz", P), ("emb", P), ("ld_emb", L), ("text", P), ("demb", P), ("ld_demb", L),
                ("ka", P), ("kgs", P), ("kge", P), ("ksw", P), ("vn", P), ("vn_host", P)]


class VnTerm(ctypes.Structure):
    _fields_ = [("n1", I), ("n2", I), ("A", I), ("null", I), ("vids", P), ("nids", P), ("voff", P), ("vlist", P),
                ("noff", P), ("nlist", P)]


class VideoAttn(ctypes.Structure):
    _fields_ = [("Q", I), ("C1", I), ("T", I), ("G", I), ("clogit", P), ("ldc", L), ("attn", P), ("lda", L),
                ("seg_id", P), ("flogit", P), ("ldf", L), ("gs", P), ("ge", P), ("gl", P), ("pred_off", L)]


class VnVideo(ctypes.Structure):
    _fields_ = [("Q", I), ("T", I), ("G", I), ("nattn", I), ("action_clogit", P), ("lda", L), ("frame_clogit", P),
                ("ldf", L), ("attn", P), ("ldattn", L), ("seg_id", P), ("seg_start", P), ("seg_end", P), ("gs", P),
                ("ge", P), ("gl", P), ("pred_off", L)]


ABI_STRUCTS = (GemmDesc, DecoderParams, MstcnParams, LossTerm, VideoAttn, Mstcn2Params, VnTerm, VnVideo)


SIGNATURES = {
    "fx_version": (I, []),
    "fx_last_error": (ctypes.c_char_p, []),
    "fx_struct_size": (L, [I]),
    "fx_gemm": (I, [ctypes.POINTER(GemmDesc), P]),
    "fx_gemm_workspace_floats": (L, [ctypes.POINTER(GemmDesc)]),
    "fx_linear_fwd": (I, [P, L, P, L, I, I, I, P, L, P, P, L, I, I, P]),
    "fx_linear_bwd_workspace_floats": (L, [I, I, I]),
    "fx_linear_bwd": (I, [P, L, P, L, P, L, P, L, I, I, I, P, L, P, L, P, I, I, P, P]),
    "fx_x2y_saved_floats": (L, [I, I, I, I, I]),
    "fx_x2y_workspace_floats": (L, [I, I, I, I, I, I, I, P, P]),
    "fx_x2y_core": (I, [I, I, P, P, I, I]),
    "fx_x2y_fwd": (I, [P, L, I, I, P, L, I, P, L, I, I, P, L, I, P, P, P, P, P, P, P, P, I, I, I, P, P, F, U, P, L, P,
                       P, P, P, P]),
    "fx_x2y_bwd": (I, [P, L, I, I, I, P, L, I, I, I, P, P, P, P, I, I, I, P, P, F, U, P, P, P, L, P, P, P, P, P, P,
                       P, P, P, P, P, P, P, P, I, I, P, I, P, P]),
    "fx_decoder_saved_floats": (L, [ctypes.POINTER(DecoderParams), I, I, I, I, I]),
    "fx_decoder_workspace_floats": (L, [ctypes.POINTER(DecoderParams), I, I, I, I, I]),
    "fx_tok_gemm": (I, [P, L, I, I, I, I, P, P, P, L, I, P, P, L, P, L, P, P]),
    "fx_decoder_fwd": (I, [ctypes.POINTER(DecoderParams), P, L, I, P, L, P, L, I, I, P, L, P, L, P, P, P]),
    "fx_decoder_bwd": (I, [ctypes.POINTER(DecoderParams), ctypes.POINTER(DecoderGrads), P, L, I, P, P, L, I, I, P, L,
                           P, L, P, L, P, P, L, P, L, P, P, P]),
    "fx_mstcn_saved_floats": (L, [ctypes.POINTER(MstcnParams), I]),
    "fx_side_stream": (P, []),
    "fx_side_join": (I, [P]),
    "fx_mstcn_workspace_floats": (L, [ctypes.POINTER(MstcnParams), I]),
    "fx_mstcn_fwd": (I, [ctypes.POINTER(MstcnParams), P, L, I, I, P, L, P, P, P]),
    "fx_mstcn_bwd": (I, [ctypes.POINTER(MstcnParams), ctypes.POINTER(MstcnGrads), P, L, I, I, P, L, P, L, P, P, P]),
    "fx_mstcn2_saved_floats": (L, [ctypes.POINTER(Mstcn2Params), I]),
    "fx_mstcn2_workspace_floats": (L, [ctypes.POINTER(Mstcn2Params), I]),
    "fx_mstcn2_fwd": (I, [ctypes.POINTER(Mstcn2Params), P, L, I, I, P, L, P, P, P]),
    "fx_mstcn2_bwd": (I, [ctypes.POINTER(Mstcn2Params), ctypes.POINTER(Mstcn2Grads), P, L, I, I, P, L, P, L, P, P, P]),
    "fx_conv3g_workspace_floats": (L, [I, I, I]),
    "fx_conv3g_fwd": (I, [P, L, I, I, I, P, I, I, I, P, P, I, P, L, P, P]),
    "fx_conv3g_bwd": (I, [P, L, I, I, I, P, I, I, I, P, P, L, P, L, P, P, P, P]),
    "fx_layernorm_fwd": (I, [P, L, P, L, P, P, F, I, I, I, P, L, P, L, P, P]),
    "fx_layernorm_bwd_workspace_floats": (L, [I, I]),
    "fx_layernorm_bwd": (I, [P, L, P, L, P, L, P, P, I, I, I, P, L, P, P, P, P]),
    "fx_softmax_rows": (I, [P, L, I, I, F, P, L, P]),
    "fx_softmax_rows_bwd": (I, [P, L, P, L, P, L, I, I, F, P, L, P]),
    "fx_process_feature_fwd": (I, [P, L, I, I, I, P, L, P, L, P]),
    "fx_process_feature_bwd": (I, [P, L, P, L, P, L, I, I, I, P, L, P]),
    "fx_process_feature2_fwd": (I, [P, L, I, I, I, I, P, L, P, L, P]),
    "fx_process_feature2_bwd": (I, [P, L, P, L, P, L, I, I, I, I, P, L, P]),
    "fx_vn_logp_fwd": (I, [P, L, I, I, I, P, P, I, I, P, L, P, P]),
    "fx_vn_logp_bwd": (I, [P, L, P, P, L, I, I, I, I, I, P, P, P, P, P, L, P]),
    "fx_segments_from_vn_probs": (I, [P, L, I, I, I, P, P, I, I, I, P, P, P, P, P, P, P]),
    "fx_vn_workspace_floats": (L, [I, I, I, I]),
    "fx_vn_loss_fwd": (I, [P, L, I, I, I, P, P, I, I, P, I, P, P, P, F, F, P, P, P, P]),
    "fx_vn_loss_bwd": (I, [P, L, I, I, I, P, P, I, I, P, I, P, P, P, P, P, P, P, P, F, F, P, P, L, P]),
    "fx_vn_eval_pred": (I, [P, L, I, P, L, I, I, I, P, P, I, P, L, P, I, F, P, P, P]),
    "fx_vn_match_cost": (I, [P, L, I, I, I, P, P, I, P, L, I, P, P, P, P, P, I, I, F, F, P, P]),
    "fx_vn_match_cost_batch": (I, [P, P, I, I, I, P, P, I, F, F, I, P, P]),
    "fx_vn_eval_pred_batch": (I, [P, P, I, I, I, P, P, I, F, P, P, P]),
    "fx_l2norm_fwd": (I, [P, L, I, I, P, L, P, P]),
    "fx_l2norm_bwd": (I, [P, L, P, P, L, I, I, P, L, P]),
    "fx_relu_bwd": (I, [P, L, P, L, I, I, P, L, P]),
    "fx_add": (I, [P, L, P, L, I, I, P, L, I, P]),
    "fx_mha_t_workspace_floats": (L, [I, I, I, I, I]),
# ... 115 lines not shown
```

### include/factmx.h

```cpp
#ifndef FACTMX_H
#define FACTMX_H

#include <stddef.h>
#include <stdint.h>

#ifdef __cplusplus
extern "C" {
#endif

#define FX_ABI_VERSION 29

enum {
  FX_OK = 0,
  FX_ERR_SHAPE = -1,
  FX_ERR_HIP = -2,
  FX_ERR_UNSUPPORTED = -3
};

int fx_version(void);
const char* fx_last_error(void);
long long fx_struct_size(int which);

typedef struct fx_operand {
  const float* ptr;
  long long ld;
  const float* ptr1;
  long long ld1;
  int k_split;
  const int32_t* rows0;
  const int32_t* rows1;
  const float* pos;
  long long ld_pos;
  int pos_cols;
  int trans;
  int conv_taps;
  int conv_cin;
  int conv_dil;
  int conv_dir;
  int seq_len;
  long long batch_stride;
  int ones_col;
  const int* seq_off;
  int nseq;
} fx_operand;

typedef struct fx_gemm_desc {
  int M, N, K, batch;
  fx_operand a, b;
  float* c;
  long long ldc;
  long long c_batch_stride;
  float alpha;
  float beta;
  const float* bias;
  const float* resid;
  long long ld_resid;
  long long resid_batch_stride;
  const float* gate;
  long long ld_gate;
  int relu;
  int c_tap_cin;
  int split_k;
  float* workspace;
  float* c_last_col;
  long long* dbg_stamps;
  float drop_p;
  unsigned long long drop_seed;
  long long c_last_batch_stride;
  int b_dil_growth;
  int a_dil_b1;
  long long bias_batch_stride;
} fx_gemm_desc;

int fx_gemm(const fx_gemm_desc* desc, void* stream);
long long fx_gemm_workspace_floats(const fx_gemm_desc* desc);

int fx_linear_fwd(const float* x, long long ldx, const float* pos, long long ldpos, int pos_cols,
                  int M, int K, const float* w, long long ldw, const float* b, float* y,
                  long long ldy, int N, int relu, void* stream);
long long fx_linear_bwd_workspace_floats(int M, int K, int N);
int fx_linear_bwd(const float* dy, long long lddy, const float* x, long long ldx, const float* w,
                  long long ldw, const float* relu_out, long long ld_relu, int M, int K, int N,
                  float* dx, long long lddx, float* dw, long long lddw, float* db, int accumulate_dx,
                  int accumulate_w, float* workspace, void* stream);

long long fx_x2y_saved_floats(int Nx, int xdim, int Ny, int ydim, int Hd);
long long fx_x2y_workspace_floats(int Nx, int xdim, int Ny, int ydim, int Hd, int outdim, int nvid,
                                  const int* x_off, const int* y_off);
int fx_x2y_core(int Hd, int nvid, const int* x_off, const int* y_off, int Nx, int Ny);
int fx_x2y_fwd(const float* X, long long ldx, int Nx, int xdim, const float* Xpos, long long ldxp,
               int xpos_cols, const float* Y, long long ldy, int Ny, int ydim, const float* Ypos,
               long long ldyp, int ypos_cols, const float* wk, const float* bk, const float* wv,
               const float* bv, const float* wq, const float* bq, const float* wy, const float* by,
               int Hd, int outdim, int nvid, const int* x_off, const int* y_off, float drop_p,
               unsigned long long seed, float* out, long long ldo, float* logit, float* attn,
               float* saved, float* workspace, void* stream);
int fx_x2y_bwd(const float* X, long long ldx, int Nx, int xdim, int xpos_cols, const float* Y,
               long long ldy, int Ny, int ydim, int ypos_cols, const float* wk, const float* wv,
               const float* wq, const float* wy, int Hd, int outdim, int nvid, const int* x_off,
               const int* y_off, float drop_p, unsigned long long seed, const float* attn,
               const float* saved, const float* dout,
               long long lddo, const float* dlogit, const float* dattn, float* dX, float* dXpos,
               float* dY, float* dYpos, float* dwk, float* dbk, float* dwv, float* dbv, float* dwq,
               float* dbq, float* dwy, float* dby, int has_xpos, int has_ypos, float* workspace,
               int side_defer, int32_t* status, void* stream);

typedef struct fx_decoder_params {
  int A, FF, nhead, num_layers, cross, Hm, out_dim, final_norm;
  float eps;
  const float* const* sa_in_w; const float* const* sa_in_b;
  const float* const* sa_out_w; const float* const* sa_out_b;
  const float* const* ca_q_w; const float* const* ca_k_w; const float* const* ca_v_w;
  const float* const* ca_in_b;
  const float* const* ca_out_w; const float* const* ca_out_b;
  const float* const* ff1_w; const float* const* ff1_b;
  const float* const* ff2_w; const float* const* ff2_b;
  const float* const* ln_sa_w; const float* const* ln_sa_b;
  const float* const* ln_ca_w; const float* const* ln_ca_b;
  const float* const* ln_ff_w; const float* const* ln_ff_b;
  const float* fn_w; const float* fn_b;
  const float* out_w; const float* out_b;
  int side_defer;
  float dropout;
  float attn_dropout;
  unsigned long long seed;
  const int* mem_off;
  int* status;
  int dqpos_accumulate;
// ... 355 lines not shown
```

Before: 610,100 frames/s.

## Add row-tile fp32 MFMA GEMM with pre-packed weight fragments for skinny-K linears

```diff
diff --git a/fact-clip_amd/csrc/decoder.cpp b/fact-clip_amd/csrc/decoder.cpp
--- a/fact-clip_amd/csrc/decoder.cpp
+++ b/fact-clip_amd/csrc/decoder.cpp
@@ -82,7 +82,7 @@
 struct DecLayout {
   long long xq, qkv, psa, osa, xh1, rs1, t1, t1q, qc, pca, oca, xh2, rs2, t2, f1, xh3, rs3, t3, per_layer;
   long long layers, fxh, frs, fo, kv, mpos, total_saved;
-  long long wkv, bkv, wsp, total_ws_fwd;
+  long long wkv, bkv, wkvp, wsp, total_ws_fwd;
   long long dkv, dwkv, dbkv, dT, dS, dU, dF, dQKV, dO, dq, lnws, core, dmask, split, gdu, gdf, gdq, gdqkv,
       gdy, total_ws_bwd;
 };
@@ -173,6 +173,7 @@
   o = 0;
   L.wkv = o; o += al64(p->cross ? AL2 * p->Hm : 0);
   L.bkv = o; o += al64(p->cross ? AL2 : 0);
+  L.wkvp = o; o += al64(p->cross ? rowtile_packed_floats((int)AL2, p->Hm) : 0);
   const long long att = dec_attn_ws(p, nvid, (int)Qv, (int)Tv);
   L.wsp = o; o += al64(std::max(sp, att) + RA);
   L.total_ws_fwd = o;
@@ -664,7 +665,15 @@
     FX_CHECK_HIP(hipGetLastError());
     prof_begin(9, s);
     if (!mpos) {
-      FX_TRY(linear_fwd(mem, ldm, T, p->Hm, workspace + L.wkv, workspace + L.bkv, kv, AL2, AL2, 0, s));
+      const float* wkvp = nullptr;
+      if (rowtile_wanted(T, AL2, p->Hm) && ((uintptr_t)workspace & 15) == 0) {
+        std::vector<FragJob> J;
+        rowtile_job(J, workspace + L.wkv, p->Hm, AL2, p->Hm, 0, workspace + L.wkvp);
+        FX_TRY(launch_pack_frag(J.data(), 1, s));
+        wkvp = workspace + L.wkvp;
+      }
+      FX_TRY(linear_fwd(mem, ldm, T, p->Hm, workspace + L.wkv, workspace + L.bkv, kv, AL2, AL2, 0, s, -1, nullptr, 0, 0,
+                        wkvp));
       prof_end(9, s, 2.0 * T * AL2 * p->Hm, 4.0 * ((double)T * p->Hm + (double)AL2 * p->Hm + (double)T * AL2));
     } else {
       const int AL = A * NL;
diff --git a/fact-clip_amd/csrc/fx_common.h b/fact-clip_amd/csrc/fx_common.h
--- a/fact-clip_amd/csrc/fx_common.h
+++ b/fact-clip_amd/csrc/fx_common.h
@@ -103,6 +103,8 @@
   bool gemm_group = true;
   bool gemm_ktail = true;
   bool dec_tok = true;
+  int gemm_rowtile = 1;
+  int rowtile_min_fill = 80;
   int tok_spin = 0;
   bool side_stream = true;
   bool mstcn_defer = true;
diff --git a/fact-clip_amd/csrc/gemm.cpp b/fact-clip_amd/csrc/gemm.cpp
--- a/fact-clip_amd/csrc/gemm.cpp
+++ b/fact-clip_amd/csrc/gemm.cpp
@@ -7,6 +7,7 @@
 #include <vector>
 
 #include "gemm_plan.h"
+#include "ops.h"
 
 namespace fx {
 
@@ -95,7 +96,8 @@
 namespace {
 
 int plan_on_stream(const fx_gemm_desc& d, hipStream_t s, long long cnt_base, GemmPlan& P) {
-  FX_TRY(plan_gemm(d, stream_precision(s), knobs(), cnt_base, P));
+  const bool fills = d.b_frag && knobs().gemm_rowtile == 1 && frl_fills_device(d.M, knobs().rowtile_min_fill);
+  FX_TRY(plan_gemm(d, stream_precision(s), knobs(), cnt_base, P, fills));
   GemmDev& g = P.g;
   const bool direct = P.family == FAM_DIRECT;
   const int cap = d.split_k > 1 ? d.split_k : 1;
@@ -128,6 +130,7 @@
     case FAM_BF16: return launch_bf16(P, s);
     case FAM_SPLIT: return launch_split(P, s);
     case FAM_DIRECT: return launch_direct(P, s);
+    case FAM_ROWTILE: return launch_rowtile(P, s);
     default: break;
   }
   set_error("gemm: unknown kernel family");
@@ -210,9 +213,40 @@
   return FX_OK;
 }
 
+bool rowtile_wanted(long long M, int N, int K) {
+  const int kn = knobs().gemm_rowtile;
+  return kn != 0 && M > 0 && rowtile_dims_ok(N, K) && (kn == 2 || frl_fills_device(M, knobs().rowtile_min_fill));
+}
+
+long long rowtile_packed_floats(int N, int K) { return rowtile_dims_ok(N, K) ? (long long)N * K : 0; }
+
+void rowtile_job(std::vector<FragJob>& J, const float* w, long long ldw, int N, int K, int trans, float* dst) {
+  FragJob j{w, dst, (int)ldw, K, trans};
+  j.N = N;
+  J.push_back(j);
+}
+
 }
 
 extern "C" {
+
+int fx_gemm_rowtile(const fx_gemm_desc* desc, float* packed, void* stream) {
+  FX_REQUIRE(desc, "fx_gemm_rowtile: null descriptor");
+  hipStream_t s = (hipStream_t)stream;
+  fx_gemm_desc d = *desc;
+  d.b_frag = packed;
+  const bool fills = fx::knobs().gemm_rowtile == 1 && fx::frl_fills_device(d.M, fx::knobs().rowtile_min_fill);
+  if (!packed || !d.b.ptr || !fx::use_rowtile(d, fx::stream_precision(s), fx::knobs(), fills) || (d.b.ld & 3)) {
+    d.b_frag = nullptr;
+    return fx::launch_gemm(d, s);
+  }
+  std::vector<fx::FragJob> J;
+  fx::rowtile_job(J, d.b.ptr, d.b.ld, d.N, d.K, d.b.trans, packed);
+  FX_TRY(fx::launch_pack_frag(J.data(), 1, s));
+  return fx::launch_gemm(d, s);
+}
+
+long long fx_gemm_rowtile_packed_floats(int N, int K) { return fx::rowtile_packed_floats(N, K); }
 
 int fx_set_stream_precision(void* stream, int prec) {
   FX_REQUIRE(prec == FX_PREC_DEFAULT || fx::valid_precision(prec),
diff --git a/fact-clip_amd/csrc/gemm_dev.h b/fact-clip_amd/csrc/gemm_dev.h
--- a/fact-clip_amd/csrc/gemm_dev.h
+++ b/fact-clip_amd/csrc/gemm_dev.h
@@ -48,6 +48,7 @@
   long long bias_bs;
   int nsoff;
   int soff[kMaxSeq + 1];
+  const float* b_frag;
 };
 
 namespace {
diff --git a/fact-clip_amd/csrc/gemm_plan.cpp b/fact-clip_amd/csrc/gemm_plan.cpp
--- a/fact-clip_amd/csrc/gemm_plan.cpp
+++ b/fact-clip_amd/csrc/gemm_plan.cpp
@@ -32,6 +32,24 @@
   return (long long)cdiv(g.M, WBM) * g.tiles_x * batch * g.split >= 192;
 }
 
+bool plain_operand(const fx_operand& o) {
+  return !o.conv_taps && !o.pos && !o.ptr1 && !o.rows0 && !o.rows1 && !o.ones_col && o.nseq <= 0 && !o.batch_stride;
+}
+
+}
+
+bool use_rowtile(const fx_gemm_desc& d, int prec, const Knobs& kn, bool fills) {
+  if (kn.gemm_rowtile == 0 || !d.b_frag || prec != FX_PREC_F32) return false;
+  if (kn.gemm_rowtile == 1 && !fills) return false;
+  if (!rowtile_dims_ok(d.N, d.K) || d.M <= 0 || d.batch != 1) return false;
+  if (d.a.trans || !plain_operand(d.a) || !aligned16(d.a.ptr) || (d.a.ld & 3) || d.a.ld < d.K) return false;
+  if (!plain_operand(d.b) || !aligned16(d.b_frag)) return false;
+  auto ld_ok = [&](long long ld) { return ld >= d.N && ld < (1LL << 26); };
+  if (!ld_ok(d.ldc) || (d.resid && !ld_ok(d.ld_resid)) || (d.gate && !ld_ok(d.ld_gate))) return false;
+  if (d.beta != 0.f || d.drop_p != 0.f || d.c_tap_cin || d.c_last_col || d.b_dil_growth > 1 || d.a_dil_b1 > 0 ||
+      d.dbg_stamps)
+    return false;
+  return true;
 }
 
 bool operand_vec_ok(const fx_operand& o) {
@@ -50,7 +68,8 @@
   return ROWS;
 }
 
-int plan_gemm(const fx_gemm_desc& d, int prec, const Knobs& kn, long long tile_cnt_base, GemmPlan& P) {
+int plan_gemm(const fx_gemm_desc& d, int prec, const Knobs& kn, long long tile_cnt_base, GemmPlan& P,
+              bool rowtile_fills) {
   FX_REQUIRE(d.M >= 0 && d.N >= 0 && d.K >= 0 && d.batch >= 1, "gemm: bad sizes");
   FX_REQUIRE(d.a.ptr && d.b.ptr && d.c, "gemm: null operand");
   FX_REQUIRE(!(d.a.conv_taps && d.a.seq_len <= 0 && d.a.nseq <= 0) &&
@@ -130,6 +149,21 @@
   g.b_vec = operand_vec_ok(d.b);
   g.ws = d.workspace;
   int ak = kind_of(d.a, g.a_vec), bk = kind_of(d.b, g.b_vec);
+  if (use_rowtile(d, prec, kn, rowtile_fills) && rowtile_pair(ak, bk)) {
+    g.b_frag = d.b_frag;
+    g.split = 1;
+    g.kt_per_split = d.K / 32;
+    g.tiles_x = 1;
+    g.tiles_y = cdiv(d.M, 32);
+    P.ak = ak;
+    P.bk = bk;
+    P.batch = 1;
+    P.family = FAM_ROWTILE;
+    P.grid = dim3(g.tiles_y);
+    P.block = dim3(W8T);
+    P.cnt_base = tile_cnt_base;
+    return FX_OK;
+  }
   const bool direct = d.b_dil_growth <= 1 && d.a_dil_b1 <= 0 && use_direct(d, ak, bk, kn);
   if (!direct && ak == COLS && bk == COLS && g.a_vec && g.b_vec && d.K % BK != 0 && kn.gemm_ktail) ak = bk = COLS_KT;
   P.ak = ak;
diff --git a/fact-clip_amd/csrc/gemm_plan.h b/fact-clip_amd/csrc/gemm_plan.h
--- a/fact-clip_amd/csrc/gemm_plan.h
+++ b/fact-clip_amd/csrc/gemm_plan.h
@@ -6,7 +6,7 @@
 
 namespace fx {
 
-enum Family { FAM_TILED = 0, FAM_WIDE8, FAM_BF16, FAM_SPLIT, FAM_DIRECT };
+enum Family { FAM_TILED = 0, FAM_WIDE8, FAM_BF16, FAM_SPLIT, FAM_DIRECT, FAM_ROWTILE };
 
 constexpr int gen_kind(int k) { return k == ROWS_CAT ? ROWS_GEN : k; }
 
@@ -31,6 +31,13 @@
   return (ak == ROWS || ak == ROWS_GEN || ak == COLS) && (bk == ROWS || bk == COLS);
 }
 
+constexpr bool rowtile_pair(int ak, int bk) { return ak == ROWS && (bk == ROWS || bk == COLS); }
+constexpr int ROWTILE_KMAX = 768;
+constexpr bool rowtile_dims_ok(int N, int K) {
+  return K >= 32 && K <= ROWTILE_KMAX && K % 32 == 0 && N >= 256 && N % 256 == 0;
+}
+bool use_rowtile(const fx_gemm_desc& d, int prec, const Knobs& k, bool fills);
+
 struct GemmPlan {
   GemmDev g;
   dim3 grid, block;
@@ -45,13 +52,15 @@
 bool operand_vec_ok(const fx_operand& o);
 int kind_of(const fx_operand& o, bool vec);
 
-int plan_gemm(const fx_gemm_desc& d, int prec, const Knobs& k, long long tile_cnt_base, GemmPlan& P);
+int plan_gemm(const fx_gemm_desc& d, int prec, const Knobs& k, long long tile_cnt_base, GemmPlan& P,
+              bool rowtile_fills = false);
 
 int launch_tiled(const GemmPlan& P, hipStream_t s);
 int launch_wide8(const GemmPlan& P, hipStream_t s);
 int launch_bf16(const GemmPlan& P, hipStream_t s);
 int launch_split(const GemmPlan& P, hipStream_t s);
 int launch_direct(const GemmPlan& P, hipStream_t s);
+int launch_rowtile(const GemmPlan& P, hipStream_t s);
 void launch_direct_group(const GemmGroup& G, int blocks, unsigned threads, hipStream_t s);
 int launch_reduce(const GemmPlan& P, hipStream_t s);
 
diff --git a/fact-clip_amd/csrc/gemm_rowtile.hip b/fact-clip_amd/csrc/gemm_rowtile.hip
--- /dev/null
+++ b/fact-clip_amd/csrc/gemm_rowtile.hip
@@ -0,0 +1,165 @@
+#include "frl_dev.h"
+#include "gemm_plan.h"
+#include "ops.h"
+
+namespace fx {
+namespace {
+
+using namespace frl_dev;
+
+constexpr int PD = 3;
+constexpr int NB = PD + 1;
+
+template <bool FAST, bool RES, bool GATE>
+__device__ __forceinline__ void rowtile_main(const GemmDev& g, const float* lds, int m0, float4 (&pb)[NB][4]) {
+  const int tid = threadIdx.x, lane = tid & 63, w = tid >> 6, li = lane & 31, lh = lane >> 5;
+  const int K = g.K, as = K + 4, nst = K / FBK, nch = g.N / FN, S = nch * nst;
+  const float* wp = g.b_frag;
+  f32x16 acc;
+#pragma unroll
+  for (int i = 0; i < 16; ++i) acc[i] = 0.f;
+  float res[16], gat[16];
+#pragma unroll
+  for (int q = 0; q < 16; ++q) {
+    res[q] = 0.f;
+    gat[q] = 1.f;
+  }
+  auto ro = [](int q) { return (q & 3) + 8 * (q >> 2); };
+  const int lrow = m0 + 4 * lh, lcol = w * 32 + li;
+  const unsigned vb_r = 4u * (unsigned)(4 * lh * (int)g.ld_resid + lcol), vb_g = 4u * (unsigned)(4 * lh * (int)g.ld_gate + lcol),
+                 vb_c = 4u * (unsigned)(4 * lh * (int)g.ldc + lcol);
+  auto at = [](const float* base, unsigned byte_off) {
+    return reinterpret_cast<const float*>(reinterpret_cast<const char*>(base) + byte_off);
+  };
+  auto pin = [](unsigned v) {
+    asm volatile("" : "+v"(v));
+    return v;
+  };
+  auto load_res = [&](int chunk) {
+    const unsigned vo_r = pin(vb_r), vo_g = pin(vb_g);
+#pragma unroll
+    for (int q = 0; q < 16; ++q) {
+      const long long r = m0 + ro(q);
+      if (FAST || lrow + ro(q) < g.M) {
+        if constexpr (RES) res[q] = *at(g.resid + r * g.ld_resid + chunk * FN, vo_r);
+        if constexpr (GATE) gat[q] = *at(g.gate + r * g.ld_gate + chunk * FN, vo_g);
+      }
+    }
+  };
+  auto epilogue = [&](int chunk) {
+    const unsigned vo_c = pin(vb_c);
+    const float bv = g.bias ? g.bias[chunk * FN + lcol] : 0.f;
+#pragma unroll
+    for (int q = 0; q < 16; ++q) {
+      float v = g.alpha * acc[q] + bv;
+      if (g.relu == 2) v = fmaxf(v, 0.f);
+      v += res[q];
+      if (!(gat[q] > 0.f)) v = 0.f;
+      if (g.relu == 1) v = fmaxf(v, 0.f);
+      if (FAST || lrow + ro(q) < g.M) *const_cast<float*>(at(g.c + (long long)(m0 + ro(q)) * g.ldc + chunk * FN, vo_c)) = v;
+      acc[q] = 0.f;
+    }
+  };
+  float4 fa[2][4];
+  lds_frag(lds, as, li, lh, fa[0]);
+  int kst = 0;
+  auto stage = [&](int j, int t) {
+    const int kn = kst + 1 == nst ? 0 : kst + 1;
+    lds_frag(lds + kn * FBK, as, li, lh, fa[(j + 1) & 1]);
+    __builtin_amdgcn_sched_barrier(0);
+    mma_frag(fa[j & 1], pb[j], acc);
+    __builtin_amdgcn_sched_barrier(0);
+    load_b(wp, min(t + PD, S - 1), w, lane, pb[(j + PD) % NB]);
+    __builtin_amdgcn_sched_barrier(0);
+    kst = kn;
+  };
+  if constexpr (FAST) {
+    const int ngrp = nst / NB;
+    int t = 0;
+    for (int chunk = 0; chunk < nch; ++chunk) {
+      for (int gi = 0; gi + 1 < ngrp; ++gi, t += NB) {
+#pragma unroll
+        for (int j = 0; j < NB; ++j) stage(j, t + j);
+      }
+      load_res(chunk);
+#pragma unroll
+      for (int j = 0; j < NB; ++j) stage(j, t + j);
+      t += NB;
+      epilogue(chunk);
+    }
+  } else {
+    int chunk = 0;
+    auto stage_end = [&](int j, int t) {
+      const bool last = kst + 1 == nst;
+      if (last) load_res(chunk);
+      stage(j, t);
+      if (last) epilogue(chunk++);
+    };
+    int t0 = 0;
+    for (; t0 + NB <= S; t0 += NB) {
+#pragma unroll
+      for (int j = 0; j < NB; ++j) stage_end(j, t0 + j);
+    }
+#pragma unroll
+    for (int j = 0; j < NB - 1; ++j)
+      if (t0 + j < S) stage_end(j, t0 + j);
+  }
+}
+
+template <bool RES, bool GATE>
+__global__ __launch_bounds__(FT) void gemm_rowtile_kernel(GemmDev g, int xcd_runs) {
+  extern __shared__ float lds[];
+  const int tid = threadIdx.x, lane = tid & 63, w = tid >> 6;
+  const int m0 = frl_tile_id(xcd_runs, 1) * FR;
+  const int K = g.K, as = K + 4, nst = K / FBK, S = (g.N / FN) * nst;
+  const float* wp = g.b_frag;
+  float4 pb[NB][4];
+#pragma unroll
+  for (int t = 0; t < PD; ++t) load_b(wp, min(t, S - 1), w, lane, pb[t]);
+  {
+    const int k4n = K / 4, total = FR * k4n;
+    for (int i0 = tid; i0 < total; i0 += 4 * FT) {
+      float4 v[4];
+#pragma unroll
+      for (int u = 0; u < 4; ++u) {
+        const int i = min(i0 + u * FT, total - 1), r = i / k4n, c = i - r * k4n;
+        v[u] = ld4(g.a.ptr + (long long)min(m0 + r, g.M - 1) * g.a.ld + c * 4);
+      }
+#pragma unroll
+      for (int u = 0; u < 4; ++u) {
+        const int i = i0 + u * FT, r = i / k4n, c = i - r * k4n;
+        if (i < total) st4(lds + r * as + c * 4, m0 + r < g.M ? v[u] : make_float4(0.f, 0.f, 0.f, 0.f));
+      }
+    }
+  }
+  __syncthreads();
+  if (m0 + FR <= g.M && nst % NB == 0) rowtile_main<true, RES, GATE>(g, lds, m0, pb);
+  else rowtile_main<false, RES, GATE>(g, lds, m0, pb);
+}
+
+}
+
+int launch_rowtile(const GemmPlan& P, hipStream_t s) {
+  const GemmDev& g = P.g;
+  FX_REQUIRE(g.b_frag && rowtile_dims_ok(g.N, g.K) && g.M > 0, "gemm(rowtile): needs packed weights, K % 32, N % 256");
+  auto lds_bytes = [](int K) { return FR * (K + 4) * (int)sizeof(float); };
+  using Kernel = void (*)(GemmDev, int);
+  static const Kernel kernels[2][2] = {{gemm_rowtile_kernel<false, false>, gemm_rowtile_kernel<false, true>},
+                                       {gemm_rowtile_kernel<true, false>, gemm_rowtile_kernel<true, true>}};
+  static const bool attr = [&] {
+    bool ok = true;
+    for (const auto& row : kernels)
+      for (Kernel k : row)
+        ok = ok && hipFuncSetAttribute((const void*)k, hipFuncAttributeMaxDynamicSharedMemorySize,
+                                       lds_bytes(ROWTILE_KMAX)) == hipSuccess;
+    return ok;
+  }();
+  FX_REQUIRE(attr, "gemm(rowtile): cannot raise the LDS limit");
+  const int nt = cdiv(g.M, FR);
+  const int xcd_runs = knobs().frl_xcd >= 1 && nt >= 16;
+  fx_launch(kernels[g.resid != nullptr][g.gate != nullptr], dim3(nt), dim3(FT), (std::uint32_t)lds_bytes(g.K), s, g,
+            xcd_runs);
+  return FX_OK;
+}
+
+}
diff --git a/fact-clip_amd/csrc/linear.cpp b/fact-clip_amd/csrc/linear.cpp
--- a/fact-clip_amd/csrc/linear.cpp
+++ b/fact-clip_amd/csrc/linear.cpp
@@ -64,8 +64,10 @@
 }
 
 int linear_fwd(const float* x, long long ldx, int M, int K, const float* w, const float* b, float* y, long long ldy,
-               int N, int relu, hipStream_t s, long long ldw, const float* pos, long long ldpos, int pos_cols) {
+               int N, int relu, hipStream_t s, long long ldw, const float* pos, long long ldpos, int pos_cols,
+               const float* w_frag) {
   fx_gemm_desc d = gemm_desc(M, N, K, op_rows(x, ldx), op_rows(w, ldw < 0 ? K : ldw), y, ldy);
+  d.b_frag = w_frag;
   d.a.pos = pos;
   d.a.ld_pos = ldpos;
   d.a.pos_cols = pos ? pos_cols : 0;
@@ -76,8 +78,9 @@
 
 fx_gemm_desc desc_linear_dx(const float* dy, long long lddy, const float* w, int M, int K, int N, float* dx,
                             long long lddx, int accumulate, const float* gate, long long ld_gate, float* ws,
-                            long long ldw) {
+                            long long ldw, const float* wt_frag) {
   fx_gemm_desc d = gemm_desc(M, K, N, op_rows(dy, lddy), op_cols(w, ldw < 0 ? K : ldw), dx, lddx);
+  d.b_frag = wt_frag;
   d.beta = accumulate ? 1.f : 0.f;
   d.gate = gate;
   d.ld_gate = ld_gate;
@@ -87,8 +90,9 @@
 }
 
 int linear_dx(const float* dy, long long lddy, const float* w, int M, int K, int N, float* dx, long long lddx,
-              int accumulate, const float* gate, long long ld_gate, float* ws, hipStream_t s, long long ldw) {
-  return launch_gemm(desc_linear_dx(dy, lddy, w, M, K, N, dx, lddx, accumulate, gate, ld_gate, ws, ldw), s);
+              int accumulate, const float* gate, long long ld_gate, float* ws, hipStream_t s, long long ldw,
+              const float* wt_frag) {
+  return launch_gemm(desc_linear_dx(dy, lddy, w, M, K, N, dx, lddx, accumulate, gate, ld_gate, ws, ldw, wt_frag), s);
 }
 
 fx_gemm_desc desc_linear_dwdb(const float* dy, long long lddy, const float* x, long long ldx, int M, int K, int N,
diff --git a/fact-clip_amd/csrc/mstcn.cpp b/fact-clip_amd/csrc/mstcn.cpp
--- a/fact-clip_amd/csrc/mstcn.cpp
+++ b/fact-clip_amd/csrc/mstcn.cpp
@@ -57,7 +57,7 @@
 struct MstcnLayout {
   long long rows_pad;
   long long rowsF;
-  long long h, z, xh, rs, wbs, wpts, wk1b, wk2b, total_saved;
+  long long h, z, xh, rs, wbs, wpts, wk1b, wk2b, rt_in, rt_int, rt_out, rt_outt, rt_top, total_saved;
   long long wf, wk1, wk2, buf0, buf1, buf2, buf3, buf4, buf5, split, split2, colsum, dzall, dhall, dball, csb, bsl,
       total_ws;
 };
@@ -79,7 +79,12 @@
   L.wpts = L.wbs + NL * wsz;
   L.wk1b = L.wpts + NL * F * F;
   L.wk2b = L.wk1b + (fl ? NL * wsz : 0);
-  L.total_saved = L.wk2b + (fl ? NL * F * F : 0);
+  L.rt_in = al64(L.wk2b + (fl ? NL * F * F : 0));
+  L.rt_int = L.rt_in + (p->in_map ? rowtile_packed_floats(p->F, p->cin) : 0);
+  L.rt_out = L.rt_int + (p->in_map ? rowtile_packed_floats(p->cin, p->F) : 0);
+  L.rt_outt = L.rt_out + rowtile_packed_floats(p->cout, p->F);
+  L.rt_top = L.rt_outt + rowtile_packed_floats(p->F, p->cout);
+  L.total_saved = L.rt_top + (NL > 0 ? rowtile_packed_floats(p->F, p->F) : 0);
   L.wf = 0;
   L.wk1 = L.wf + NL * wsz;
   L.wk2 = L.wk1 + (fl ? NL * wsz : 0);
@@ -128,6 +133,20 @@
   return FX_OK;
 }
 
+struct MstcnRowtile {
+  bool in, in_dx, out, out_dx, top;
+};
+MstcnRowtile mstcn_rowtile(const fx_mstcn_params* p, int rows, const float* saved) {
+  MstcnRowtile r{};
+  if ((uintptr_t)saved & 15) return r;
+  r.in = p->in_map && rowtile_wanted(rows, p->F, p->cin);
+  r.in_dx = p->in_map && rowtile_wanted(rows, p->cin, p->F);
+  r.out = rowtile_wanted(rows, p->cout, p->F);
+  r.out_dx = rowtile_wanted(rows, p->F, p->cout);
+  r.top = p->num_layers > 0 && rowtile_wanted(rows, p->F, p->F);
+  return r;
+}
+
 int layer_dilation(const fx_mstcn_params* p, int i) {
   long long d = p->dil0 > 0 ? p->dil0 : 1;
   const int f = p->dil_factor > 0 ? p->dil_factor : 2;
@@ -166,6 +185,7 @@
   SideLane lane;
   float *spl, *spm;
   const float *wk1, *wk2;
+  MstcnRowtile rt;
   int rows, F, NL, ng;
   bool drop;
   float *Hb[3], *Zb[3];
@@ -184,6 +204,7 @@
     fx_gemm_desc d = gemm_desc(rows, F, F, op_rows(gB, F), op_rows(saved + L.wpts + (long long)i * F * F, F), dZ, F);
     d.gate = z(i);
     d.ld_gate = F;
+    if (i == NL - 1 && rt.top) d.b_frag = saved + L.rt_top;
     d.split_k = pick_split(rows, F, F);
     d.workspace = spm;
     return launch_gemm(d, s);
@@ -301,7 +322,8 @@
   const int top = NL - 1;
   FX_TRY(c.lane.fork(1));
   FX_TRY(c.pw_dw(c.Hb[0], top));
-  FX_TRY(linear_dx(c.Hb[0], F, c.p->w_pw[top], rows, F, F, c.Zb[0], F, 0, c.z(top), F, c.spm, c.s));
+  FX_TRY(linear_dx(c.Hb[0], F, c.p->w_pw[top], rows, F, F, c.Zb[0], F, 0, c.z(top), F, c.spm, c.s, -1,
+                   c.rt.top ? c.saved + c.L.rt_top : nullptr));
   FX_TRY(c.lane.fork(2));
   FX_TRY(c.conv_dw(top, c.Zb[0]));
   FX_TRY(c.lane.done(top));
@@ -416,20 +438,29 @@
     FX_CHECK_HIP(hipMemset2DAsync(saved + L.h + (long long)rows * F, L.rowsF * sizeof(float), 0,
                                   (L.rows_pad - rows) * F * sizeof(float), 2 * p->num_layers + 1, s));
   float* h0 = saved + L.h;
+  const bool fused = mstcn_fused_ok(p, q, saved);
+  const MstcnRowtile rt = mstcn_rowtile(p, rows, saved);
+  {
+    std::vector<FragJob> J;
+    if (fused && p->num_layers > 0) {
+      frag_layer_jobs(J, p->num_layers, F, workspace + L.wf, 3LL * F * F, p->w_pw, nullptr, 0, workspace + L.wk1,
+                      workspace + L.wk2);
+      frag_layer_jobs(J, p->num_layers, F, saved + L.wbs, 3LL * F * F, nullptr, saved + L.wpts, (long long)F * F,
+                      saved + L.wk1b, saved + L.wk2b);
+    }
+    if (rt.in) rowtile_job(J, p->w_in, p->cin, F, p->cin, 0, saved + L.rt_in);
+    if (rt.in_dx) rowtile_job(J, p->w_in, p->cin, p->cin, F, 1, saved + L.rt_int);
+    if (rt.out) rowtile_job(J, p->w_out, F, p->cout, F, 0, saved + L.rt_out);
+    if (rt.out_dx) rowtile_job(J, p->w_out, F, F, p->cout, 1, saved + L.rt_outt);
+    if (rt.top) rowtile_job(J, p->w_pw[p->num_layers - 1], F, F, F, 1, saved + L.rt_top);
+    if (!J.empty()) FX_TRY(launch_frag_jobs(J, s));
+  }
   if (p->in_map) {
-    FX_TRY(linear_fwd(x, ldx, rows, p->cin, p->w_in, p->b_in, h0, F, F, 0, s));
+    FX_TRY(linear_fwd(x, ldx, rows, p->cin, p->w_in, p->b_in, h0, F, F, 0, s, -1, nullptr, 0, 0,
+                      rt.in ? saved + L.rt_in : nullptr));
   } else {
     FX_CHECK_HIP(hipMemcpy2DAsync(h0, F * sizeof(float), x, ldx * sizeof(float), F * sizeof(float), rows,
                                   hipMemcpyDeviceToDevice, s));
-  }
-  const bool fused = mstcn_fused_ok(p, q, saved);
-  if (fused && p->num_layers > 0) {
-    std::vector<FragJob> J;
-    frag_layer_jobs(J, p->num_layers, F, workspace + L.wf, 3LL * F * F, p->w_pw, nullptr, 0, workspace + L.wk1,
-                    workspace + L.wk2);
-    frag_layer_jobs(J, p->num_layers, F, saved + L.wbs, 3LL * F * F, nullptr, saved + L.wpts, (long long)F * F,
-                    saved + L.wk1b, saved + L.wk2b);
-    FX_TRY(launch_frag_jobs(J, s));
   }
   for (int i = 0; i < p->num_layers; ++i) {
     const float* hi = saved + L.h + i * L.rowsF;
@@ -473,7 +504,8 @@
                                   saved + L.rs + (long long)i * rows, saved + L.xh + i * L.rowsF, F, s));
   }
   const float* hL = saved + L.h + p->num_layers * L.rowsF;
-  return linear_fwd(hL, F, rows, F, p->w_out, p->b_out, y, ldy, p->cout, 0, s);
+  return linear_fwd(hL, F, rows, F, p->w_out, p->b_out, y, ldy, p->cout, 0, s, -1, nullptr, 0, 0,
+                    rt.out ? saved + L.rt_out : nullptr);
 }
 
 int fx_mstcn_bwd(const fx_mstcn_params* p, const fx_mstcn_grads* g, const float* x, long long ldx, int T, int nvid,
@@ -494,7 +526,7 @@
   const BwdSchedule sched = fchain ? (defer ? BwdSchedule::FusedDeferred : BwdSchedule::FusedPerLayer)
                                    : (defer ? BwdSchedule::GemmDeferred : BwdSchedule::PerLayer);
   MstcnBwd c{p, g, q, L, saved, ws, dx, lddx, s, side_lane(s, !p->layernorm && drop_chain_ok), ws + L.split,
-             ws + L.split2, saved + L.wk1b, saved + L.wk2b, rows, F, NL, ng, drop,
+             ws + L.split2, saved + L.wk1b, saved + L.wk2b, mstcn_rowtile(p, rows, saved), rows, F, NL, ng, drop,
              {ws + L.buf0, ws + L.buf1, ws + L.buf3}, {ws + L.buf2, ws + L.buf4, ws + L.buf5}};
   if (fchain && !mstcn_fused_ok(p, q, saved)) {
     std::vector<FragJob> J;
@@ -511,7 +543,8 @@
   FX_TRY(c.lane.fork(0));
   FX_TRY(linear_dwdb(dy, lddy, c.h(NL), F, rows, F, p->cout, g->w_out, g->b_out, 1, c.spl, c.lane.side));
   float* dHtop = defer ? c.dHall(NL - 1) : c.Hb[0];
-  FX_TRY(linear_dx(dy, lddy, p->w_out, rows, F, p->cout, dHtop, F, 0, nullptr, 0, c.spm, s));
+  FX_TRY(linear_dx(dy, lddy, p->w_out, rows, F, p->cout, dHtop, F, 0, nullptr, 0, c.spm, s, -1,
+                   c.rt.out_dx ? saved + L.rt_outt : nullptr));
   const float* dH = c.Hb[0];
   switch (sched) {
     case BwdSchedule::FusedDeferred: FX_TRY(bwd_fused_deferred(c, &dH)); break;
@@ -524,7 +557,9 @@
       FX_TRY(c.lane.fork(0));
       FX_TRY(linear_dwdb(dH, F, x, ldx, rows, p->cin, F, g->w_in, g->b_in, 1, c.spl, c.lane.side));
     }
-    if (dx) FX_TRY(linear_dx(dH, F, p->w_in, rows, p->cin, F, dx, lddx, 0, nullptr, 0, c.spm, s));
+    if (dx)
+      FX_TRY(linear_dx(dH, F, p->w_in, rows, p->cin, F, dx, lddx, 0, nullptr, 0, c.spm, s, -1,
+                       c.rt.in_dx ? saved + L.rt_int : nullptr));
   } else if (dx && dH) {
     FX_CHECK_HIP(hipMemcpy2DAsync(dx, lddx * sizeof(float), dH, F * sizeof(float), F * sizeof(float), rows,
                                   hipMemcpyDeviceToDevice, s));
diff --git a/fact-clip_amd/csrc/mstcn_fused.hip b/fact-clip_amd/csrc/mstcn_fused.hip
--- a/fact-clip_amd/csrc/mstcn_fused.hip
+++ b/fact-clip_amd/csrc/mstcn_fused.hip
@@ -260,14 +260,16 @@
   float* dst[FRAG_JOBS];
   int ld[FRAG_JOBS];
   int K[FRAG_JOBS];
+  int N[FRAG_JOBS];
   unsigned long long trans;
 };
 
 __global__ __launch_bounds__(256) void pack_frag_kernel(PackFragArgs a) {
-  const int st = blockIdx.x, w = blockIdx.y, m = blockIdx.z;
-  if (st * FBK >= a.K[m]) return;
+  const int st = blockIdx.x, m = blockIdx.z;
+  if (st * FBK >= a.K[m] || (int)blockIdx.y * 32 >= a.N[m]) return;
+  const int chunk = blockIdx.y / 8, w = blockIdx.y % 8;
   const int q = threadIdx.x >> 6, lane = threadIdx.x & 63;
-  const int n = w * 32 + (lane & 31), k = st * FBK + 16 * (lane >> 5) + 4 * q;
+  const int n = blockIdx.y * 32 + (lane & 31), k = st * FBK + 16 * (lane >> 5) + 4 * q;
   float4 v;
   if ((a.trans >> m) & 1ull) {
     const float* c = a.src[m] + (long long)k * a.ld[m] + n;
@@ -275,7 +277,7 @@
   } else {
     v = ld4(a.src[m] + (long long)n * a.ld[m] + k);
   }
-  st4(a.dst[m] + ((long long)((st * 8 + w) * 4 + q) * 64 + lane) * 4, v);
+  st4(a.dst[m] + (long long)chunk * FN * a.K[m] + ((long long)((st * 8 + w) * 4 + q) * 64 + lane) * 4, v);
 }
 
 }
@@ -314,10 +316,13 @@
 int launch_pack_frag(const FragJob* jobs, int n, hipStream_t s) {
   FX_REQUIRE(n >= 1 && n <= FRAG_JOBS, "pack_frag: 1..48 matrices per launch");
   PackFragArgs a{};
-  int kmax = 0;
+  int kmax = 0, nmax = 0;
   for (int i = 0; i < n; ++i) {
-    FX_REQUIRE(jobs[i].K % FBK == 0 && jobs[i].ld % 4 == 0 && jobs[i].ld >= (jobs[i].trans ? FN : jobs[i].K),
-               "pack_frag: K % 32 == 0");
+    FX_REQUIRE(jobs[i].K % FBK == 0 && jobs[i].ld % 4 == 0 && jobs[i].N >= FN && jobs[i].N % FN == 0 &&
+                   jobs[i].ld >= (jobs[i].trans ? jobs[i].N : jobs[i].K),
+               "pack_frag: K % 32 == 0, N % 256 == 0");
+    a.N[i] = jobs[i].N;
+    nmax = std::max(nmax, jobs[i].N);
     a.src[i] = jobs[i].src;
     a.dst[i] = jobs[i].dst;
     a.ld[i] = jobs[i].ld;
@@ -325,7 +330,7 @@
     if (jobs[i].trans) a.trans |= 1ull << i;
     kmax = std::max(kmax, jobs[i].K);
   }
-  fx_launch(pack_frag_kernel, dim3(kmax / FBK, FN / 32, n), dim3(256), 0, s, a);
+  fx_launch(pack_frag_kernel, dim3(kmax / FBK, nmax / 32, n), dim3(256), 0, s, a);
   FX_CHECK_HIP(hipGetLastError());
   return FX_OK;
 }
diff --git a/fact-clip_amd/csrc/ops.h b/fact-clip_amd/csrc/ops.h
--- a/fact-clip_amd/csrc/ops.h
+++ b/fact-clip_amd/csrc/ops.h
@@ -1,4 +1,6 @@
 #pragma once
+#include <vector>
+
 #include "fx_common.h"
 
 namespace fx {
@@ -120,9 +122,10 @@
 long long split_ws(int M, int N, int K, int batch = 1);
 int linear_fwd(const float* x, long long ldx, int M, int K, const float* w, const float* b, float* y, long long ldy,
                int N, int relu, hipStream_t s, long long ldw = -1, const float* pos = nullptr, long long ldpos = 0,
-               int pos_cols = 0);
+               int pos_cols = 0, const float* w_frag = nullptr);
 int linear_dx(const float* dy, long long lddy, const float* w, int M, int K, int N, float* dx, long long lddx,
-              int accumulate, const float* gate, long long ld_gate, float* ws, hipStream_t s, long long ldw = -1);
+              int accumulate, const float* gate, long long ld_gate, float* ws, hipStream_t s, long long ldw = -1,
+              const float* wt_frag = nullptr);
 int linear_dwdb(const float* dy, long long lddy, const float* x, long long ldx, int M, int K, int N, float* dw,
                 float* db, int accumulate, float* ws, hipStream_t s, long long lddw = -1);
 int linear_dw(const float* dy, long long lddy, const float* x, long long ldx, int M, int K, int N, float* dw,
@@ -130,7 +133,7 @@
 long long dwdb_ws(int M, int K, int N);
 fx_gemm_desc desc_linear_dx(const float* dy, long long lddy, const float* w, int M, int K, int N, float* dx,
                             long long lddx, int accumulate, const float* gate, long long ld_gate, float* ws,
-                            long long ldw = -1);
+                            long long ldw = -1, const float* wt_frag = nullptr);
 fx_gemm_desc desc_linear_dwdb(const float* dy, long long lddy, const float* x, long long ldx, int M, int K, int N,
                               float* dw, float* db, int accumulate, float* ws, long long lddw = -1);
 int linear_bwd_pair(const fx_gemm_desc& dwdb, const fx_gemm_desc& dx, hipStream_t s);
@@ -170,9 +173,13 @@
   float* dst;
   int ld, K;
   int trans = 0;
+  int N = 256;
 };
 constexpr int FRAG_JOBS = 48;
 int launch_pack_frag(const FragJob* jobs, int n, hipStream_t s);
+bool rowtile_wanted(long long M, int N, int K);
+long long rowtile_packed_floats(int N, int K);
+void rowtile_job(std::vector<FragJob>& J, const float* w, long long ldw, int N, int K, int trans, float* dst);
 int launch_frl(const float* x, long long ldx, int M, int T, int dil, int dir, const int* seq_off, int nseq,
                const float* w1p, const float* bias1, int relu1, const float* resid1, long long ldr1, float* out1,
                long long ldo1, const float* w2p, const float* bias2, const float* resid2, long long ldr2,
diff --git a/fact-clip_amd/csrc/runtime.cpp b/fact-clip_amd/csrc/runtime.cpp
--- a/fact-clip_amd/csrc/runtime.cpp
+++ b/fact-clip_amd/csrc/runtime.cpp
@@ -119,6 +119,8 @@
     if (const char* p = env("FX_GEMM_GROUP")) k.gemm_group = p[0] != '0';
     if (const char* p = env("FX_GEMM_KTAIL")) k.gemm_ktail = p[0] != '0';
     if (const char* p = env("FX_DEC_TOK")) k.dec_tok = p[0] != '0';
+    if (const char* p = env("FX_GEMM_ROWTILE")) k.gemm_rowtile = std::max(0, std::min(2, std::atoi(p)));
+    if (const char* p = env("FX_ROWTILE_MIN_FILL")) k.rowtile_min_fill = std::atoi(p);
     if (const char* p = env("FX_TOK_SPIN")) k.tok_spin = std::max(0, std::atoi(p));
     if (const char* p = env("FX_SIDE_STREAM")) k.side_stream = p[0] != '0';
     if (const char* p = env("FX_MSTCN_DEFER")) k.mstcn_defer = p[0] != '0';
diff --git a/fact-clip_amd/csrc/x2y.cpp b/fact-clip_amd/csrc/x2y.cpp
--- a/fact-clip_amd/csrc/x2y.cpp
+++ b/fact-clip_amd/csrc/x2y.cpp
@@ -10,8 +10,20 @@
 namespace {
 constexpr int GMAX_GROUP = 4;
 struct X2YLayout {
-  long long xin, yin, xk, xv, yq, feat, total;
+  long long xin, yin, xk, xv, yq, feat, pk, pv, pkt, pvt, pq, pqt, total;
 };
+struct X2YRowtile {
+  bool x, xt, y, yt;
+};
+X2YRowtile x2y_rowtile(int Nx, int xdim, int Ny, int ydim, int Hd, const float* saved) {
+  X2YRowtile r{};
+  if ((uintptr_t)saved & 15) return r;
+  r.x = rowtile_wanted(Nx, Hd, xdim);
+  r.xt = rowtile_wanted(Nx, xdim, Hd);
+  r.y = rowtile_wanted(Ny, Hd, ydim);
+  r.yt = rowtile_wanted(Ny, ydim, Hd);
+  return r;
+}
 X2YLayout x2y_layout(int Nx, int xdim, int Ny, int ydim, int Hd) {
   X2YLayout L{};
   L.xin = 0;
@@ -20,7 +32,13 @@
   L.xv = L.xk + al64((long long)Nx * Hd);
   L.yq = L.xv + al64((long long)Nx * Hd);
   L.feat = L.yq + al64((long long)Ny * Hd);
-  L.total = L.feat + al64((long long)Ny * Hd);
+  L.pk = L.feat + al64((long long)Ny * Hd);
+  L.pv = L.pk + rowtile_packed_floats(Hd, xdim);
+  L.pkt = L.pv + rowtile_packed_floats(Hd, xdim);
+  L.pvt = L.pkt + rowtile_packed_floats(xdim, Hd);
+  L.pq = L.pvt + rowtile_packed_floats(xdim, Hd);
+  L.pqt = L.pq + rowtile_packed_floats(Hd, ydim);
+  L.total = L.pqt + rowtile_packed_floats(ydim, Hd);
   return L;
 }
 struct VidRows {
@@ -158,10 +176,21 @@
     yin = saved + L.yin;
     ldyin = ydim;
   }
+  const X2YRowtile rt = x2y_rowtile(Nx, xdim, Ny, ydim, Hd, saved);
+  {
+    std::vector<FragJob> J;
+    if (rt.x) rowtile_job(J, wk, xdim, Hd, xdim, 0, saved + L.pk);
+    if (rt.x) rowtile_job(J, wv, xdim, Hd, xdim, 0, saved + L.pv);
+    if (rt.xt) rowtile_job(J, wk, xdim, xdim, Hd, 1, saved + L.pkt);
+    if (rt.xt) rowtile_job(J, wv, xdim, xdim, Hd, 1, saved + L.pvt);
+    if (rt.y) rowtile_job(J, wq, ydim, Hd, ydim, 0, saved + L.pq);
+    if (rt.yt) rowtile_job(J, wq, ydim, ydim, Hd, 1, saved + L.pqt);
+    if (!J.empty()) FX_TRY(launch_pack_frag(J.data(), (int)J.size(), s));
+  }
   prof_begin(10, s);
-  FX_TRY(linear_fwd(xin, ldxin, Nx, xdim, wk, bk, xk, Hd, Hd, 0, s));
-  FX_TRY(linear_fwd(X, ldx, Nx, xdim, wv, bv, xv, Hd, Hd, 0, s));
-  FX_TRY(linear_fwd(yin, ldyin, Ny, ydim, wq, bq, yq, Hd, Hd, 0, s));
+  FX_TRY(linear_fwd(xin, ldxin, Nx, xdim, wk, bk, xk, Hd, Hd, 0, s, -1, nullptr, 0, 0, rt.x ? saved + L.pk : nullptr));
+  FX_TRY(linear_fwd(X, ldx, Nx, xdim, wv, bv, xv, Hd, Hd, 0, s, -1, nullptr, 0, 0, rt.x ? saved + L.pv : nullptr));
+  FX_TRY(linear_fwd(yin, ldyin, Ny, ydim, wq, bq, yq, Hd, Hd, 0, s, -1, nullptr, 0, 0, rt.y ? saved + L.pq : nullptr));
   prof_end(10, s, 2.0 * Hd * (2.0 * Nx * xdim + (double)Ny * ydim),
            4.0 * (2.0 * Nx * xdim + (double)Ny * ydim + Hd * (2.0 * xdim + ydim) + Hd * (2.0 * Nx + Ny)), 3);
   const float scale = 1.0f / std::sqrt((float)Hd);
@@ -253,6 +282,7 @@
   float* spl = workspace + W.split;
   WsBound wb(spl, W.split_floats);
   const float scale = 1.0f / std::sqrt((float)Hd);
+  const X2YRowtile rt = x2y_rowtile(Nx, xdim, Ny, ydim, Hd, saved);
   FX_TRY(linear_dx(dout, lddo, wy, Ny, cw, outdim, dcat, cw, 0, nullptr, 0, spl, s));
   const float* catd = nullptr;
   if (drop_p > 0.f) {
@@ -372,19 +402,20 @@
     FX_TRY(lane.join(side_defer));
   }
   if (dX || dXpos) {
-    FX_TRY(linear_dx(dxk, Hd, wk, Nx, xdim, Hd, dXk, xdim, 0, nullptr, 0, spl, s));
+    FX_TRY(linear_dx(dxk, Hd, wk, Nx, xdim, Hd, dXk, xdim, 0, nullptr, 0, spl, s, -1, rt.xt ? saved + L.pkt : nullptr));
     if (dXpos) FX_TRY(add2(dXk, xdim, nullptr, 0, Nx, xpos_cols, dXpos, xpos_cols, (has_xpos >> 1) & 1, s));
     if (dX) {
       fx_gemm_desc d = gemm_desc(Nx, xdim, Hd, op_rows(dxv, Hd), op_cols(wv, xdim), dX, xdim);
       d.resid = dXk;
       d.ld_resid = xdim;
+      if (rt.xt) d.b_frag = saved + L.pvt;
       d.split_k = pick_split(Nx, xdim, Hd);
       d.workspace = spl;
       FX_TRY(launch_gemm(d, s));
     }
   }
   if (dY || dYpos) {
-    FX_TRY(linear_dx(dyq, Hd, wq, Ny, ydim, Hd, dYq, ydim, 0, nullptr, 0, spl, s));
+    FX_TRY(linear_dx(dyq, Hd, wq, Ny, ydim, Hd, dYq, ydim, 0, nullptr, 0, spl, s, -1, rt.yt ? saved + L.pqt : nullptr));
     if (dYpos) FX_TRY(add2(dYq, ydim, nullptr, 0, Ny, ypos_cols, dYpos, ypos_cols, (has_ypos >> 1) & 1, s));
     if (dY) FX_TRY(add2(dYq, ydim, dcat, cw, Ny, ydim, dY, ydim, 0, s));
   }
diff --git a/fact-clip_amd/factmx/native.py b/fact-clip_amd/factmx/native.py
--- a/fact-clip_amd/factmx/native.py
+++ b/fact-clip_amd/factmx/native.py
@@ -5,7 +5,7 @@
 
 _HERE = os.path.dirname(os.path.abspath(__file__))
 LIB_PATH = os.environ.get("FACTMX_LIB", os.path.join(_HERE, "_lib", "libfactmx.so"))
-ABI_VERSION = 29
+ABI_VERSION = 30
 
 P = ctypes.c_void_p
 I = ctypes.c_int
@@ -32,7 +32,7 @@
                 ("resid_batch_stride", L), ("gate", P), ("ld_gate", L), ("relu", I), ("c_tap_cin", I),
                 ("split_k", I), ("workspace", P), ("c_last_col", P), ("dbg_stamps", P), ("drop_p", F),
                 ("drop_seed", U), ("c_last_batch_stride", L), ("b_dil_growth", I),
-                ("a_dil_b1", I), ("bias_batch_stride", L)]
+                ("a_dil_b1", I), ("bias_batch_stride", L), ("b_frag", P)]
 
 
 class MstcnParams(ctypes.Structure):
@@ -120,6 +120,8 @@
     "fx_struct_size": (L, [I]),
     "fx_gemm": (I, [ctypes.POINTER(GemmDesc), P]),
     "fx_gemm_workspace_floats": (L, [ctypes.POINTER(GemmDesc)]),
+    "fx_gemm_rowtile": (I, [ctypes.POINTER(GemmDesc), P, P]),
+    "fx_gemm_rowtile_packed_floats": (L, [I, I]),
     "fx_linear_fwd": (I, [P, L, P, L, I, I, I, P, L, P, P, L, I, I, P]),
     "fx_linear_bwd_workspace_floats": (L, [I, I, I]),
     "fx_linear_bwd": (I, [P, L, P, L, P, L, P, L, I, I, I, P, L, P, L, P, I, I, P, P]),
diff --git a/include/factmx.h b/include/factmx.h
--- a/include/factmx.h
+++ b/include/factmx.h
@@ -8,7 +8,7 @@
 extern "C" {
 #endif
 
-#define FX_ABI_VERSION 29
+#define FX_ABI_VERSION 30
 
 enum {
   FX_OK = 0,
@@ -70,10 +70,13 @@
   int b_dil_growth;
   int a_dil_b1;
   long long bias_batch_stride;
+  const float* b_frag;
 } fx_gemm_desc;
 
 int fx_gemm(const fx_gemm_desc* desc, void* stream);
 long long fx_gemm_workspace_floats(const fx_gemm_desc* desc);
+int fx_gemm_rowtile(const fx_gemm_desc* desc, float* packed, void* stream);
+long long fx_gemm_rowtile_packed_floats(int N, int K);
 
 int fx_linear_fwd(const float* x, long long ldx, const float* pos, long long ldpos, int pos_cols,
                   int M, int K, const float* w, long long ldw, const float* b, float* y,
```

Measured after the change: 617,100 frames/s (median of 4 runs). +1.1%, better.
